# lujiarui/Str2Str

Hardware: AMD Instinct MI355X
Metric: sampled conformations/sec (whole node), 256-res chain, 100 denoise steps (higher is better)
Workload: dtype f32 (matrix products on 2-way f16 split MFMA 'f16x3': 3 products per block, fp32 accumulate, fp32-equivalent); 1 GPU; configs[1]: single 256-residue synthetic chain, 128 replicas per GPU x 100 denoise steps (+1 self-conditioning forward), probability-flow ODE, seeded synthetic weights; n_res=256, replicas_per_gpu=128, denoise_steps=100, parallelism=replica-shard x1, arith=f16x3, rng=device

## Files before the change

include/str2str_hip.h:

```cpp
#ifndef STR2STR_HIP_H
#define STR2STR_HIP_H

#ifdef __cplusplus
extern "C" {
#endif

int s2s_abi_version(void);



int s2s_edge_transition(const float* edge, const float* node_ab, const float* node_p, const float* w1_packed,
                        const float* w2_packed, const float* wf_packed, const float* b2, const float* bf,
                        const float* ln_gamma, const float* ln_beta, const float* mask, float* out, int n_samples,
                        int n_res, float ln_eps, const float* proj_w_packed, const float* proj_bias_cat64,
                        float* proj_attn_bias, float* proj_pair_z, void* stream);

int s2s_edge_transition_f16x3(const float* edge, const float* node_ab, const float* node_p, const void* weight_stream,
                              const float* b2, const float* ln_gamma, const float* ln_beta,
                              const float* mask, float* out, int n_samples, int n_res, float ln_eps, int io_layout,
                              const float* proj_bias_cat64, float* proj_attn_bias, float* proj_pair_z, int prescale_exp,
                              int* range_words, void* stream);

int s2s_edge_embed(const float* node_a, const float* node_b, const float* rel_table, const float* bin_table,
                   const float* bin_lower, const long long* residue_idx, const float* ca_xyz, const float* w2_packed,
                   const float* w3_packed, const float* b2, const float* b3, const float* ln_gamma, const float* ln_beta,
                   const float* mask, float* out, int n_samples, int n_res, int rel_offset, int n_rel, int n_bins,
                   float ln_eps, const float* proj_w_packed, const float* proj_bias_cat64, float* proj_attn_bias,
                   float* proj_pair_z, void* stream);

int s2s_edge_embed_f16x3(const float* node_a, const float* node_b, const float* rel_table, const float* bin_table,
                         const float* bin_lower, const long long* residue_idx, const float* ca_xyz,
                         const void* weight_stream, const float* b2, const float* b3, const float* ln_gamma,
                         const float* ln_beta, const float* mask, float* out, int n_samples, int n_res, int rel_offset,
                         int n_rel, int n_bins, float ln_eps, int out_tiled, const float* proj_bias_cat64,
                         float* proj_attn_bias, float* proj_pair_z, int* range_words, void* stream);

int s2s_pair_project(const float* edge, const float* w_packed, const float* bias_cat64, float* attn_bias, float* pair_z,
                     int n_samples, int n_res, void* stream);


int s2s_ipa_prep_points(const float* rigids7, const float* q_pts_lin, const float* kv_pts_lin, float* q_pts, float* k_pts,
                        float* v_pts, long long n_frames, int n_heads, int n_qk_points, int n_v_points, int v_pts_stride,
                        void* stream);

int s2s_ipa_attention(const float* q, const float* kv, const float* q_pts, const float* k_pts, const float* v_pts64,
                      const float* attn_bias, float* logits_out, float* stats_out, const float* mask, const float* rigids7,
                      const float* head_w_scaled, float* out, int n_samples, int n_res, int n_heads, int c_hidden,
                      int n_qk_points, int n_v_points, int c_pair_z, float inf, float eps, void* stream);

int s2s_ipa_prep_points_f16(const float* rigids7, const float* q_pts_lin, const float* kv_pts_lin, const float* head_w_scaled,
                            void* qp_xp, void* kp_xp, void* vp_vf, float* q2, float* k2, int n_samples, int n_res, int n_heads,
                            int n_qk_points, int n_v_points, int c_hidden, const void* s_xp, void* k_shared, void* v_shared,
                            int* range_words, void* stream);
int s2s_ipa_attention_f16w(const void* q_xp, const void* k_xp, const void* v_vf, const void* qp_xp, const void* kp_xp,
                             const void* vp_vf, const float* q2, const float* k2, const float* attn_bias, float* logits_out,
                             float* stats_out, const float* mask, const float* rigids7, float* out, void* out_xp,
                             int out_xp_ksteps, int n_samples, int n_res, int n_heads, int c_hidden, int n_qk_points,
                             int n_v_points, int c_pair_z, float inf, float eps, int n_kv_heads, void* stream);

int s2s_ipa_opair(const float* logits, const float* stats, const float* pair_z, float* out, int n_samples, int n_res,
                  int n_heads, int c_pair_z, int out_row_stride, int out_col_offset, int logits_ld, void* stream);


int s2s_rigid_compose_update(const float* rigids7, const float* update6, const float* mask, float* out7,
                             long long n_frames, int update_ld, void* stream);

int s2s_torsion_head(const float* u, int u_ld, int normalize, const float* gt_sin_cos, long long gt_row_stride, const float* fixed_mask,
                     float eps, float* out2, long long n_rows, void* stream);

int s2s_rigid_scale_trans(const float* rigids7, float* out7, long long n_frames, float scale, int divide, void* stream);

int s2s_set_backbone_tables(const float* pos_21x5x3, const float* mask_21x5, const int* is_psi_group_21x5,
                            const float* default_frames_21x2x4x4);

int s2s_frames_to_backbone(const float* rigids7, const float* psi_sincos, const long long* aatype, float* atom14_bb5,
                           float* atom37, long long n_frames, void* stream);


int s2s_se3_step(const float* x0_7, const float* xt_7, const float* mask, const float* diffuse_mask,
                 const float* params8, const double* z_rot, const double* z_trans,
                 const double* rot_score_in, const double* trans_score_in, float* next7,
                 double* rot_score_out, double* trans_score_out, int n_samples, int n_res, double dt,
                 const double* dt_per_sample, double coordinate_scaling, int probability_flow, int center_trans,
                 double noise_scale, void* stream);

int s2s_embed_assemble(const float* t_img, long long t_img_rows, const float* node_const, long long node_const_rows, const float* fa, const float* fb,
                       long long n_rows, int n_res, void* h_xp, float* h_f32, float* node_a, float* node_b, int b_col_blocked,
                       int* range_words, void* stream);


int s2s_pack_planes(const float* x, long long n_rows, int ld, int col0, int n_cols, void* xp, int xp_ksteps, int xp_kstep0,
                    const float* row_scale, int* range_words, void* stream);

int s2s_node_linear(const void* xp, const void* w_packed, const float* bias, long long n_rows, int k_in, int n_out,
                    int tiles_per_block, const float* pre_scale, int relu, const float* pre_mask, const float* residual,
                    int residual_ld, const float* ln_gamma, const float* ln_beta, float ln_eps, const float* post_mask,
                    float* out_f32, int out_ld, int out_col0, void* out_xp, int out_xp_ksteps, int out_xp_kstep0,
                    int map_pad, int map_src, int* range_words, void* stream);

int s2s_node_linear_f32(const float* x, int x_ld, const float* w_packed, const float* bias, long long n_rows, int k_in, int n_out,
                        int tiles_per_block, const float* pre_scale, int relu, const float* pre_mask, const float* residual,
                        int residual_ld, const float* ln_gamma, const float* ln_beta, float ln_eps, const float* post_mask,
                        float* out_f32, int out_ld, int out_col0, void* stream);

int s2s_node_linear_vfrag(const void* xp, const void* w_packed, const float* bias, long long n_rows, int k_in, int n_out,
                          int tiles_per_head, void* out_vf, int map_pad, int map_src, int* range_words, void* stream);

typedef struct s2s_node_problem {
    const void* xp; const void* w_packed; const float* bias;
    long long n_rows; int k_in, n_out, tiles_per_block;
    int vfrag_tiles_per_head;
    float* out_f32; int out_ld, out_col0;
    void* out_xp; int out_xp_ksteps, out_xp_kstep0;
    void* out_vf;
    int map_pad, map_src, relu;
    const float* pre_scale;
} s2s_node_problem;
int s2s_node_linear_multi(const s2s_node_problem* problems, int n_problems, int* range_words, void* stream);

typedef struct s2s_chain_layer { const void* w_packed; const float* bias; int relu; } s2s_chain_layer;
int s2s_node_chain(const void* xp, const s2s_chain_layer* layers, int n_layers, long long n_rows, int width, int k_in0,
                   const float* mid_residual, int mid_residual_ld, float* mid_out_f32, int mid_out_ld, const float* mid_ln_gamma,
                   const float* mid_ln_beta, float mid_ln_eps, const float* pre_mask, const float* residual, int residual_ld, const float* ln_gamma, const float* ln_beta, float ln_eps,
                   const float* post_mask, float* out_f32, int out_ld, int out_col0, void* out_xp, int out_xp_ksteps,
                   int out_xp_kstep0, int* range_words, void* stream);

int s2s_row_layernorm(const float* x, int x_ld, long long n_rows, int n_cols, const float* ln_gamma, const float* ln_beta, float ln_eps,
                      const float* post_mask, float* out_f32, int out_ld, int out_col0, void* out_xp, int out_xp_ksteps,
                      int out_xp_kstep0, int* range_words, void* stream);

int s2s_encoder_attention(const float* qkv, const float* key_bias, float* out_f32, void* out_xp, int n_samples, int n_res,
                          int n_heads, int head_dim, int* range_words, void* stream);

int s2s_encoder_attention_f16x3(const float* qkv, const float* key_bias, float* out_f32, void* out_xp, int n_samples, int n_res,
                          int n_heads, int head_dim, int* range_words, void* stream);


int s2s_forward_marginal(const float* rigids0_4x4, const float* z_axis, const float* u01, const float* z_trans,
                         const double* cdf_rows, const int* cdf_row_of_sample, const float* omega_grid, int n_omega,
                         const float* params2, const float* diffuse_mask, float coordinate_scaling, float* rigids_t7,
                         int n_samples, int n_res, void* stream);


int s2s_ca_sample_stats(const float* ca, int n_samples, int n_res, float clash_bar, int k_exclusion, int* n_clash,
                        float* adjacent_max, double* radius_of_gyration, void* stream);

int s2s_ca_pairwise_distances(const float* ca, int n_samples, int n_res, int offset, float* out, void* stream);

int s2s_ca_pwd_js(const float* ref_ca, int n_ref, const float* pred_ca, int n_pred, int n_res, int offset, int n_bins,
                  double pseudo_count, double* js_per_channel, const double* ref_weights, const double* pred_weights, void* stream);


int s2s_ca_rmsd_matrix(const float* a, int n_a, const float* b, int n_b, int n_res, const float* weights, double* rmsd,
                       double* workspace, long long workspace_doubles, void* stream);

int s2s_ca_superpose(const float* mobile, int n_mobile, const float* target, int n_res, const float* weights, double* rmsd,
                     double* xform, void* stream);

int s2s_apply_xform(const float* points, const double* xform, int n_samples, long long n_points, float* out, void* stream);

#define S2S_TM_MAX_RES 800

int s2s_ca_tm_matrix(const float* a, int n_a, const float* b, int n_b, int n_res, double d0, double* tm, void* stream);

int s2s_ca_tm_superpose(const float* mobile, int n_mobile, const float* target, int n_res, double d0, double* tm, double* xform12,
                        void* stream);

#define S2S_LDDT_MAX_RES 1024
#define S2S_LDDT_LIST_SLOTS(n_res) (((long long)(n_res) * ((long long)(n_res) - 1) / 2 + 1) / 2 * 2)
#define S2S_LDDT_WORKSPACE_BYTES(n_a, n_res) ((long long)(n_a) * (12 * S2S_LDDT_LIST_SLOTS(n_res) + 8 + 4 * (long long)(n_res)))

int s2s_ca_lddt_matrix(const float* a, int n_a, const float* b, int n_b, int n_res, double cutoff, int min_seq_sep, double* lddt,
                       void* workspace, long long workspace_bytes, void* stream);

int s2s_ca_lddt_per_residue(const float* model, int n_model, const float* target, int n_res, double cutoff, int min_seq_sep,
                            double* per_res, double* total, void* workspace, long long workspace_bytes, void* stream);

#define S2S_VIOL_MAX_RES 1024

int s2s_backbone_violations(const float* atoms, int n, int n_res, const unsigned char* atom_exists, const int* aatype,
                            const int* residue_index, double tolerance_factor, double clash_tolerance, double* losses, double* fractions,
                            double* per_residue_loss, unsigned char* bond_mask, unsigned char* clash_atom_mask, int* n_clash_pairs,
                            void* stream);

#define S2S_SS_MAX_RES 704

int s2s_secondary_structure(const float* atoms, int n, int n_res, const int* aatype, const int* residue_index, unsigned char* ss,
                            int* n_hbonds, double* hb_energy, int* hb_partner, double* torsions, void* stream);

#define S2S_CLUSTER_MAX_N 65536

int s2s_cluster_adjacency(const double* values, int n_rows, int row0, int n, double cutoff, int at_least, unsigned long long* adj,
                          int* deg, void* stream);

int s2s_cluster_gromos(const unsigned long long* adj, int* deg, int n, int init, int n_rounds, int* labels, int* centres, int* sizes,
                       int* state, unsigned long long* live_ws, unsigned long long* members_ws, void* stream);

#define S2S_CONTACT_MAX_RES 1024
#define S2S_CONTACT_MAX_STRUCTURES 65535
#define S2S_CONTACT_LIST_SLOTS(n_res) ((long long)(n_res) > 1 ? (long long)(n_res) * ((long long)(n_res) - 1) / 2 : 1)

int s2s_ca_contact_map(const float* ca, int n, int n_res, double cutoff, int min_seq_sep, const double* weights, int* counts,
                       double* weighted, void* stream);

int s2s_ca_contact_stats(const float* ca, int n, int n_res, double cutoff, int min_seq_sep, int* n_contacts, long long* sep_sum,
                         void* stream);

int s2s_ca_native_contacts(const float* native, int n_res, double cutoff, int min_seq_sep, int* pairs, double* d0, int* n_pairs,
                           void* stream);

int s2s_ca_native_q(const float* ca, int n, int n_res, const int* pairs, const double* d0, int n_pairs, double beta, double lam,
                    double* q_soft, double* q_hard, int* hits, void* stream);

#define S2S_SASA_MAX_RES 512
#define S2S_SASA_MAX_POINTS 1024

int s2s_backbone_sasa(const float* atoms, int n, int n_res, const unsigned char* atom_exists, const double* radii, double probe,
                      const double* sphere, int n_points, int* counts, double* per_residue, double* total, void* stream);

#define S2S_SAXS_MAX_RES 1024
#define S2S_SAXS_MAX_Q 1024
#define S2S_SAXS_MAX_TYPES 64

int s2s_ca_scattering(const float* ca, int n, int n_res, const double* q, int n_q, const int* types, const double* table, int n_types,
                      double* intensity, double* inv_r_mean, void* stream);


long long s2s_format_pdb_models(const float* atom37, int n_models, int n_res, const long long* aatype,
                                const long long* residue_index, const long long* chain_index, const double* b_factors,
                                int first_model_number, int add_end, char* out, long long out_capacity);

long long s2s_write_pdb_models(const char* path, int append, const float* atom37, int n_models, int n_res,
                               const long long* aatype, const long long* residue_index, const long long* chain_index,
                               const double* b_factors, int first_model_number, int add_end);

long long s2s_merge_pdb_files(const char* const* paths, int n_paths, const char* out_path);

int s2s_mt19937_discard(unsigned long long* state624, int* left, unsigned long long* next, unsigned long long n_outputs);

#ifdef __cplusplus
}
#endif
#endif
```

str2str_amd/csrc/enc_attention.hip:

```cpp
#include <hip/hip_runtime.h>
#include <math.h>

#include "f16x3.h"
#include "range_flag.h"
#include "str2str_hip.h"

namespace {

__device__ __forceinline__ f32x16 mfma32(float a, float b, f32x16 c) { return __builtin_amdgcn_mfma_f32_32x32x2f32(a, b, c, 0, 0, 0); }

template <int DH>
__global__ void __launch_bounds__(256) enc_attention_kernel(const float* __restrict__ qkv, const float* __restrict__ key_bias,
                                                            float* __restrict__ out_f32, bf16x8* __restrict__ out_xp, int* range_flag, int B, int N,
                                                            int heads, float scale) {
    static_assert(DH == 80, "built for the reference configuration (d_model 320, 4 heads)");
    constexpr int KSd = DH + 4;
    constexpr int CT = (DH + 31) / 32;
    constexpr int HALF = DH / 2;
    __shared__ __attribute__((aligned(16))) float s_k[2][32 * KSd];
    __shared__ __attribute__((aligned(16))) float s_v[2][32 * 96];
    __shared__ float s_b[2][32];
    const int lane = threadIdx.x & 63, h = lane >> 5, c = lane & 31, wave = threadIdx.x >> 6;
    const int n_qb = (N + 127) / 128;
    int bid = blockIdx.x;
    const int qb = bid % n_qb; bid /= n_qb;
    const int head = bid % heads;
    const int b = bid / heads;
    const int D = heads * DH;
    const int i = qb * 128 + wave * 32 + c;
    const bool ivalid = i < N;
    const long long row_i = (long long)b * N + (ivalid ? i : N - 1);
    const float* base = qkv + (long long)b * N * 3 * D + head * DH;

    float4 st[5];
    auto tile_load = [&](int j0) {
#pragma unroll
        for (int k = 0; k < 5; ++k) {
            const int idx = threadIdx.x + 256 * k;
            const int which = idx / 640, rem = idx % 640, r = rem / 20, c4 = rem % 20;
            const int j = min(j0 + r, N - 1);
            st[k] = *reinterpret_cast<const float4*>(base + (long long)j * 3 * D + D * (1 + which) + 4 * c4);
        }
    };
    auto tile_store = [&](int par, int j0) {
#pragma unroll
        for (int k = 0; k < 5; ++k) {
            const int idx = threadIdx.x + 256 * k;
            const int which = idx / 640, rem = idx % 640, r = rem / 20, c4 = rem % 20;
            float* dst = which ? &s_v[par][r * 96 + 4 * c4] : &s_k[par][r * KSd + 4 * c4];
            *reinterpret_cast<float4*>(dst) = st[k];
        }
        if (threadIdx.x < 32) {
            const int j = j0 + threadIdx.x;
            s_b[par][threadIdx.x] = j < N ? (key_bias ? key_bias[(long long)b * N + j] : 0.f) : -INFINITY;
        }
    };
    for (int idx = threadIdx.x; idx < 2 * 32 * 16; idx += 256) s_v[idx / 512][((idx % 512) / 16) * 96 + 80 + idx % 16] = 0.f;

    tile_load(0);
    float qreg[HALF];
    {
        const float* qrow = qkv + row_i * 3 * D + head * DH + HALF * h;
#pragma unroll
        for (int s4 = 0; s4 < HALF / 4; ++s4) {
            const float4 v = *reinterpret_cast<const float4*>(qrow + 4 * s4);
            qreg[4 * s4 + 0] = v.x * scale; qreg[4 * s4 + 1] = v.y * scale; qreg[4 * s4 + 2] = v.z * scale; qreg[4 * s4 + 3] = v.w * scale;
        }
    }
    f32x16 O[CT];
#pragma unroll
    for (int t = 0; t < CT; ++t)
#pragma unroll
        for (int r = 0; r < 16; ++r) O[t][r] = 0.f;
    float m_run = -INFINITY, l_run = 0.f;
    tile_store(0, 0);
    __syncthreads();

    int cur = 0;
    for (int j0 = 0; j0 < N; j0 += 32, cur ^= 1) {
        const bool more = j0 + 32 < N;
        if (more) tile_load(j0 + 32);
        f32x16 S, S1;
#pragma unroll
        for (int r = 0; r < 16; ++r) S[r] = 0.f, S1[r] = 0.f;
        const float* krow = &s_k[cur][c * KSd + HALF * h];
#pragma unroll
        for (int s4 = 0; s4 < HALF / 4; ++s4) {
            const float4 kf = *reinterpret_cast<const float4*>(krow + 4 * s4);
            S = mfma32(kf.x, qreg[4 * s4 + 0], S);
            S1 = mfma32(kf.y, qreg[4 * s4 + 1], S1);
            S = mfma32(kf.z, qreg[4 * s4 + 2], S);
            S1 = mfma32(kf.w, qreg[4 * s4 + 3], S1);
        }
        float tmax = -INFINITY;
#pragma unroll
        for (int r = 0; r < 16; ++r) {
            const float s = (S[r] + S1[r]) + s_b[cur][rowmap(r, h)];
            S[r] = s;
            tmax = fmaxf(tmax, s);
        }
        tmax = fmaxf(tmax, __shfl_xor(tmax, 32, 64));
        const float m_new = fmaxf(m_run, tmax);
        const float m_use = m_new == -INFINITY ? 0.f : m_new;
        const float alpha = expf(m_run - m_use);
        m_run = m_new;
        float psum = 0.f;
#pragma unroll
        for (int r = 0; r < 16; ++r) {
            const float p = expf(S[r] - m_use);
            S[r] = p;
            psum += p;
        }
        l_run = l_run * alpha + psum;
#pragma unroll
        for (int t = 0; t < CT; ++t) {
            f32x16 o = O[t];
#pragma unroll
            for (int r = 0; r < 16; ++r) o[r] *= alpha;
            const float* vcol = &s_v[cur][32 * t + c + 4 * h * 96];
#pragma unroll
            for (int s = 0; s < 16; ++s) o = mfma32(vcol[((s & 3) + 8 * (s >> 2)) * 96], S[s], o);
            O[t] = o;
        }
        if (more) tile_store(cur ^ 1, j0 + 32);
        __syncthreads();
    }

    const float l_tot = l_run + __shfl_xor(l_run, 32, 64);
    const float inv = 1.0f / l_tot;
    if (!ivalid) return;
    const long long row = (long long)b * N + i;
    if (out_f32) {
        float* o = out_f32 + row * D + head * DH;
#pragma unroll
        for (int t = 0; t < CT; ++t)
#pragma unroll
            for (int rq = 0; rq < 4; ++rq) {
                const int c0 = 32 * t + 8 * rq + 4 * h;
                if (c0 < DH)
                    *reinterpret_cast<float4*>(o + c0) = make_float4(O[t][4 * rq] * inv, O[t][4 * rq + 1] * inv, O[t][4 * rq + 2] * inv, O[t][4 * rq + 3] * inv);
            }
    }
    if (out_xp) {
        const int KS = D / 16;
        bf16x8* o = out_xp + (((row >> 5) * KS + (DH / 16) * head) * 2) * 64 + 32 * h + (int)(row & 31);
        float amax = 0.f;
#pragma unroll
        for (int t = 0; t < CT; ++t)
#pragma unroll
            for (int u = 0; u < 2; ++u) {
                if (2 * t + u >= DH / 16) continue;
                f16x8 ph, pl;
#pragma unroll
                for (int j = 0; j < 8; ++j) {
                    float v = O[t][8 * u + j] * inv;
                    amax = s2s::range_max(amax, v);
                    asm volatile("" : "+v"(v));
                    const _Float16 a_ = (_Float16)v;
                    ph[j] = a_; pl[j] = (_Float16)(v - (float)a_);
                }
                bf16x8* q = o + ((2 * t + u) * 2) * 64;
                q[0] = __builtin_bit_cast(bf16x8, ph); q[64] = __builtin_bit_cast(bf16x8, pl);
            }
        s2s::range_report(range_flag, amax, s2s::kRangeEncoderAttention);
    }
}


__device__ __forceinline__ void enc_split8(float x0, float x1, float x2, float x3, float x4, float x5, float x6, float x7, f16x8& ph, f16x8& pl,
                                           float& amax) {
    unsigned h0, h1, h2, h3, l0, l1, l2, l3;
    split4_f16(x0, x1, x2, x3, h0, h1, l0, l1, amax);
    split4_f16(x4, x5, x6, x7, h2, h3, l2, l3, amax);
    ph = __builtin_bit_cast(f16x8, u32x4{h0, h1, h2, h3});
    pl = __builtin_bit_cast(f16x8, u32x4{l0, l1, l2, l3});
}

template <int DH>
__global__ void __launch_bounds__(256, 2) enc_attention_f16_kernel(const float* __restrict__ qkv, const float* __restrict__ key_bias,
                                                                float* __restrict__ out_f32, bf16x8* __restrict__ out_xp, int* range_flag, int B,
                                                                int N, int heads, float scale) {
    static_assert(DH == 80, "built for the reference configuration (d_model 320, 4 heads)");
    constexpr int KSQ = DH / 16;
    constexpr int CT = (DH + 31) / 32;
    constexpr float kPS = 1024.0f;
    __shared__ __attribute__((aligned(16))) f16x8 s_kf[2][KSQ * 2 * 64];
    __shared__ __attribute__((aligned(16))) f16x8 s_vf[2][CT * 2 * 2 * 64];
    __shared__ float s_b[2][32];
    const int lane = threadIdx.x & 63, h = lane >> 5, c = lane & 31, wave = threadIdx.x >> 6;
    const int n_qb = (N + 127) / 128;
    int bid = blockIdx.x;
    const int qb = bid % n_qb; bid /= n_qb;
    const int head = bid % heads;
    const int b = bid / heads;
    const int D = heads * DH;
    const int i = qb * 128 + wave * 32 + c;
    const bool ivalid = i < N;
    const long long row_i = (long long)b * N + (ivalid ? i : N - 1);
    const float* base = qkv + (long long)b * N * 3 * D + head * DH;
    float amax = 0.f;

    float4 st[5];
    auto tile_load = [&](int j0) {
#pragma unroll
        for (int k = 0; k < 5; ++k) {
            const int idx = threadIdx.x + 256 * k;
            const int which = idx / 640, rem = idx % 640, r = rem / 20, c4 = rem % 20;
            const int j = min(j0 + r, N - 1);
            st[k] = *reinterpret_cast<const float4*>(base + (long long)j * 3 * D + D * (1 + which) + 4 * c4);
        }
    };
    auto tile_store = [&](int par, int j0) {
#pragma unroll
        for (int k = 0; k < 5; ++k) {
            const int idx = threadIdx.x + 256 * k;
            const int which = idx / 640, rem = idx % 640, r = rem / 20, c4 = rem % 20;
            unsigned h0, h1, l0, l1;
            split4_f16(st[k].x, st[k].y, st[k].z, st[k].w, h0, h1, l0, l1, amax);
            if (!which) {
                const int ch = 4 * c4, ks = ch >> 4, hh = (ch >> 3) & 1, e = ch & 7;
                _Float16* ph = reinterpret_cast<_Float16*>(&s_kf[par][(ks * 2 + 0) * 64 + 32 * hh + r]) + e;
                _Float16* pl = reinterpret_cast<_Float16*>(&s_kf[par][(ks * 2 + 1) * 64 + 32 * hh + r]) + e;
                *reinterpret_cast<uint2*>(ph) = make_uint2(h0, h1);
                *reinterpret_cast<uint2*>(pl) = make_uint2(l0, l1);
            } else {
                const int u = r >> 4, hh = (r >> 2) & 1, e = (r & 3) + 4 * ((r >> 3) & 1);
                const unsigned hv[2] = {h0, h1}, lv[2] = {l0, l1};
#pragma unroll
                for (int q = 0; q < 4; ++q) {
                    const int ch = 4 * c4 + q, t = ch >> 5, cc = ch & 31;
                    const unsigned short hb = (unsigned short)(hv[q >> 1] >> (16 * (q & 1))), lb = (unsigned short)(lv[q >> 1] >> (16 * (q & 1)));
                    reinterpret_cast<unsigned short*>(&s_vf[par][((t * 2 + u) * 2 + 0) * 64 + 32 * hh + cc])[e] = hb;
                    reinterpret_cast<unsigned short*>(&s_vf[par][((t * 2 + u) * 2 + 1) * 64 + 32 * hh + cc])[e] = lb;
                }
            }
        }
        if (threadIdx.x < 32) {
            const int j = j0 + threadIdx.x;
            s_b[par][threadIdx.x] = j < N ? (key_bias ? key_bias[(long long)b * N + j] : 0.f) : -INFINITY;
        }
    };
    for (int idx = threadIdx.x; idx < 2 * 2 * 2 * 64; idx += 256) {
        const int par = idx >> 8, rest = idx & 255, ln = rest & 63;
        if ((ln & 31) >= DH - 32 * (CT - 1)) s_vf[par][((CT - 1) * 2 * 2) * 64 + rest] = f16x8{0, 0, 0, 0, 0, 0, 0, 0};
    }

    tile_load(0);
    f16x8 qh[KSQ], ql[KSQ];
    {
        const float* qrow = qkv + row_i * 3 * D + head * DH + 8 * h;
#pragma unroll
        for (int ks = 0; ks < KSQ; ++ks) {
            const float4 v0 = *reinterpret_cast<const float4*>(qrow + 16 * ks), v1 = *reinterpret_cast<const float4*>(qrow + 16 * ks + 4);
            enc_split8(v0.x * scale, v0.y * scale, v0.z * scale, v0.w * scale, v1.x * scale, v1.y * scale, v1.z * scale, v1.w * scale, qh[ks], ql[ks],
                       amax);
        }
    }
    f32x16 O[CT];
#pragma unroll
    for (int t = 0; t < CT; ++t)
#pragma unroll
        for (int r = 0; r < 16; ++r) O[t][r] = 0.f;
    float m_run = -INFINITY, l_run = 0.f;
    tile_store(0, 0);
    __syncthreads();

    int cur = 0;
    for (int j0 = 0; j0 < N; j0 += 32, cur ^= 1) {
        const bool more = j0 + 32 < N;
        if (more) tile_load(j0 + 32);
        f32x16 S, S1;
#pragma unroll
        for (int r = 0; r < 16; ++r) S[r] = 0.f, S1[r] = 0.f;
#pragma unroll
        for (int ks = 0; ks < KSQ; ++ks) {
            const f16x8 kh = s_kf[cur][(ks * 2 + 0) * 64 + lane], kl = s_kf[cur][(ks * 2 + 1) * 64 + lane];
            f32x16& acc = (ks & 1) ? S1 : S;
            acc = mfma_f16(kl, qh[ks], acc);
            acc = mfma_f16(kh, ql[ks], acc);
            acc = mfma_f16(kh, qh[ks], acc);
        }
        float tmax = -INFINITY;
#pragma unroll
        for (int r = 0; r < 16; ++r) {
            const float sv = (S[r] + S1[r]) + s_b[cur][rowmap(r, h)];
            S[r] = sv;
            tmax = fmaxf(tmax, sv);
        }
        tmax = fmaxf(tmax, __shfl_xor(tmax, 32, 64));
        const float m_new = fmaxf(m_run, tmax);
        const float m_use = m_new == -INFINITY ? 0.f : m_new;
        const float alpha = expf(m_run - m_use);
        m_run = m_new;
        float psum = 0.f;
#pragma unroll
        for (int r = 0; r < 16; ++r) {
            const float pv = expf(S[r] - m_use);
            S[r] = pv * kPS;
            psum += pv;
        }
        l_run = l_run * alpha + psum;
        f16x8 ph[2], pl[2];
        float pmax = 0.f;
#pragma unroll
        for (int u = 0; u < 2; ++u) {
            enc_split8(S[8 * u + 0], S[8 * u + 1], S[8 * u + 2], S[8 * u + 3], S[8 * u + 4], S[8 * u + 5], S[8 * u + 6], S[8 * u + 7], ph[u], pl[u], pmax);
        }
#pragma unroll
        for (int t = 0; t < CT; ++t) {
            f32x16 o = O[t];
#pragma unroll
            for (int r = 0; r < 16; ++r) o[r] *= alpha;
#pragma unroll
            for (int u = 0; u < 2; ++u) {
                const f16x8 vh = s_vf[cur][((t * 2 + u) * 2 + 0) * 64 + lane], vl = s_vf[cur][((t * 2 + u) * 2 + 1) * 64 + lane];
                o = mfma_f16(vl, ph[u], o);
                o = mfma_f16(vh, pl[u], o);
                o = mfma_f16(vh, ph[u], o);
            }
            O[t] = o;
        }
        if (more) tile_store(cur ^ 1, j0 + 32);
        __syncthreads();
    }

    const float l_tot = l_run + __shfl_xor(l_run, 32, 64);
    const float inv = 1.0f / (l_tot * kPS);
    if (ivalid) {
        const long long row = (long long)b * N + i;
        if (out_f32) {
            float* o = out_f32 + row * D + head * DH;
#pragma unroll
            for (int t = 0; t < CT; ++t)
#pragma unroll
                for (int rq = 0; rq < 4; ++rq) {
                    const int c0 = 32 * t + 8 * rq + 4 * h;
                    if (c0 < DH)
                        *reinterpret_cast<float4*>(o + c0) = make_float4(O[t][4 * rq] * inv, O[t][4 * rq + 1] * inv, O[t][4 * rq + 2] * inv, O[t][4 * rq + 3] * inv);
                }
        }
        if (out_xp) {
            const int KS = D / 16;
            bf16x8* o = out_xp + (((row >> 5) * KS + (DH / 16) * head) * 2) * 64 + 32 * h + (int)(row & 31);
#pragma unroll
            for (int t = 0; t < CT; ++t)
#pragma unroll
                for (int u = 0; u < 2; ++u) {
                    if (2 * t + u >= DH / 16) continue;
                    f16x8 oh, ol;
                    enc_split8(O[t][8 * u + 0] * inv, O[t][8 * u + 1] * inv, O[t][8 * u + 2] * inv, O[t][8 * u + 3] * inv, O[t][8 * u + 4] * inv,
                               O[t][8 * u + 5] * inv, O[t][8 * u + 6] * inv, O[t][8 * u + 7] * inv, oh, ol, amax);
                    bf16x8* q = o + ((2 * t + u) * 2) * 64;
                    q[0] = __builtin_bit_cast(bf16x8, oh); q[64] = __builtin_bit_cast(bf16x8, ol);
                }
        }
    }
    s2s::range_report(range_flag, amax, s2s::kRangeEncoderAttention);
}

}

extern "C" int s2s_encoder_attention_f16x3(const float* qkv, const float* key_bias, float* out_f32, void* out_xp, int n_samples, int n_res,
                                           int n_heads, int head_dim, int* range_words, void* stream) {
    if (n_samples <= 0 || n_res <= 0) return 0;
    if (!qkv || (!out_f32 && !out_xp) || head_dim != 80 || n_heads < 1 || (n_heads * head_dim) % 32) return (int)hipErrorInvalidValue;
    const long long blocks = (long long)n_samples * n_heads * ((n_res + 127) / 128);
    hipLaunchKernelGGL((enc_attention_f16_kernel<80>), dim3((unsigned)blocks), dim3(256), 0, (hipStream_t)stream, qkv, key_bias, out_f32,
                       (bf16x8*)out_xp, range_words, n_samples, n_res, n_heads, 1.0f / sqrtf((float)head_dim));
    return (int)hipGetLastError();
}

extern "C" int s2s_encoder_attention(const float* qkv, const float* key_bias, float* out_f32, void* out_xp, int n_samples, int n_res,
                                     int n_heads, int head_dim, int* range_words, void* stream) {
    if (n_samples <= 0 || n_res <= 0) return 0;
    if (!qkv || (!out_f32 && !out_xp) || head_dim != 80 || n_heads < 1 || (n_heads * head_dim) % 32) return (int)hipErrorInvalidValue;
    const long long blocks = (long long)n_samples * n_heads * ((n_res + 127) / 128);
    hipLaunchKernelGGL((enc_attention_kernel<80>), dim3((unsigned)blocks), dim3(256), 0, (hipStream_t)stream, qkv, key_bias, out_f32,
                       (bf16x8*)out_xp, range_words, n_samples, n_res, n_heads, 1.0f / sqrtf((float)head_dim));
    return (int)hipGetLastError();
}
```

str2str_amd/csrc/node_gemm.hip:

```cpp
#include <hip/hip_runtime.h>

#include <cstdlib>

#include "f16x3.h"
#include "range_flag.h"
#include "str2str_hip.h"

namespace {

using s2s::range_max;

__device__ __forceinline__ void split8_f16(const float* v, f16x8& ph, f16x8& pl, float& amax) {
    unsigned h0, h1, h2, h3, l0, l1, l2, l3;
    split4_f16(v[0], v[1], v[2], v[3], h0, h1, l0, l1, amax);
    split4_f16(v[4], v[5], v[6], v[7], h2, h3, l2, l3, amax);
    ph = __builtin_bit_cast(f16x8, u32x4{h0, h1, h2, h3});
    pl = __builtin_bit_cast(f16x8, u32x4{l0, l1, l2, l3});
}
__device__ __forceinline__ void store_planes(f16x8* q, const float* v, float& amax) {
    f16x8 ph, pl;
    split8_f16(v, ph, pl, amax);
    q[0] = ph; q[64] = pl;
}

struct GemmArgs {
    const f16x8* xp;
    const char* wpk;
    const float* bias;
    const float* pre_scale;
    const float* pre_mask;
    const float* residual;
    const float* ln_gamma;
    const float* ln_beta;
    const float* post_mask;
    float* out_f32;
    f16x8* out_xp;
    f16x8* out_vf;
    int vf_tiles_per_head;
    long long M;
    int KS;
    int n_col_blocks;
    int res_ld, out_ld, out_col0, xp_KS, xp_ks0;
    int relu;
    float ln_eps;
    int x_ld;
    int* range_flag;
    int map_pad, map_src;
};

__device__ float s2s_zero[512];

template <int TG>
__device__ __forceinline__ void node_epilogue(f32x16 (&acc)[TG], const GemmArgs& a, long long rt, long long n_rt, int lane, int cb,
                                              float ps) {
    const int h = lane >> 5;
    const long long row = rt * 32 + (lane & 31);
    const bool valid = rt < n_rt && row < a.M;
    const long long rowc = valid ? row : a.M - 1;
    const float pm = a.pre_mask ? a.pre_mask[rowc] : 1.0f;
    const int col_base = cb * TG * 32;
    const float* bias_p = a.bias ? a.bias + col_base + 4 * h : s2s_zero + 4 * h;
    const float* res_p = a.residual ? a.residual + rowc * a.res_ld + col_base + 4 * h : s2s_zero + 4 * h;
    float4 qb[2][4], qr[2][4];
    auto fetch4 = [&](const float* p, int t, float4 (&q)[4]) {
#pragma unroll
        for (int rq = 0; rq < 4; ++rq) q[rq] = *reinterpret_cast<const float4*>(p + 32 * t + 8 * rq);
    };
    fetch4(bias_p, 0, qb[0]);
    fetch4(res_p, 0, qr[0]);
    const bool relu = a.relu != 0;
#pragma unroll
    for (int t = 0; t < TG; ++t) {
        if (t + 1 < TG) {
            fetch4(bias_p, t + 1, qb[(t + 1) & 1]);
            fetch4(res_p, t + 1, qr[(t + 1) & 1]);
        }
#pragma unroll
        for (int rq = 0; rq < 4; ++rq) {
            const float4 b = qb[t & 1][rq], rr = qr[t & 1][rq];
            float v[4] = {acc[t][4 * rq + 0] * ps + b.x, acc[t][4 * rq + 1] * ps + b.y, acc[t][4 * rq + 2] * ps + b.z,
                          acc[t][4 * rq + 3] * ps + b.w};
#pragma unroll
            for (int e = 0; e < 4; ++e) v[e] = relu ? fmaxf(v[e], 0.f) : v[e];
            acc[t][4 * rq + 0] = v[0] * pm + rr.x; acc[t][4 * rq + 1] = v[1] * pm + rr.y;
            acc[t][4 * rq + 2] = v[2] * pm + rr.z; acc[t][4 * rq + 3] = v[3] * pm + rr.w;
        }
    }
    if (a.ln_gamma) {
        float sum = 0.f;
#pragma unroll
        for (int t = 0; t < TG; ++t)
#pragma unroll
            for (int r = 0; r < 16; ++r) sum += acc[t][r];
        const float m0 = xhalf_sum(sum) * (1.0f / (TG * 32));
        float var = 0.f, dev = 0.f;
#pragma unroll
        for (int t = 0; t < TG; ++t)
#pragma unroll
            for (int r = 0; r < 16; ++r) {
                const float d = acc[t][r] - m0;
                dev += d;
                var += d * d;
            }
        const float dm = xhalf_sum(dev) * (1.0f / (TG * 32));
        const float mean = m0 + dm;
        const float rstd = 1.0f / sqrtf(xhalf_sum(var) * (1.0f / (TG * 32)) - dm * dm + a.ln_eps);
        fetch4(a.ln_gamma + col_base + 4 * h, 0, qb[0]);
        fetch4(a.ln_beta + col_base + 4 * h, 0, qr[0]);
#pragma unroll
        for (int t = 0; t < TG; ++t) {
            if (t + 1 < TG) {
                fetch4(a.ln_gamma + col_base + 4 * h, t + 1, qb[(t + 1) & 1]);
                fetch4(a.ln_beta + col_base + 4 * h, t + 1, qr[(t + 1) & 1]);
            }
#pragma unroll
            for (int rq = 0; rq < 4; ++rq) {
                const float4 g = qb[t & 1][rq], be = qr[t & 1][rq];
                acc[t][4 * rq + 0] = (acc[t][4 * rq + 0] - mean) * rstd * g.x + be.x;
                acc[t][4 * rq + 1] = (acc[t][4 * rq + 1] - mean) * rstd * g.y + be.y;
                acc[t][4 * rq + 2] = (acc[t][4 * rq + 2] - mean) * rstd * g.z + be.z;
                acc[t][4 * rq + 3] = (acc[t][4 * rq + 3] - mean) * rstd * g.w + be.w;
            }
        }
    }
    if (a.post_mask) {
        const float q = a.post_mask[rowc];
#pragma unroll
        for (int t = 0; t < TG; ++t)
#pragma unroll
            for (int r = 0; r < 16; ++r) acc[t][r] *= q;
    }
    if (a.out_f32 && valid) {
        float* o = a.out_f32 + row * a.out_ld + a.out_col0 + col_base;
#pragma unroll
        for (int t = 0; t < TG; ++t)
#pragma unroll
            for (int rq = 0; rq < 4; ++rq)
                *reinterpret_cast<float4*>(o + 32 * t + 8 * rq + 4 * h) =
                    make_float4(acc[t][4 * rq + 0], acc[t][4 * rq + 1], acc[t][4 * rq + 2], acc[t][4 * rq + 3]);
    }
    if (a.out_xp && rt < n_rt) {
        float amax = 0.f;
        f16x8* o = a.out_xp + ((rt * a.xp_KS + a.xp_ks0 + 2 * (cb * TG)) * 2) * 64 + lane;
#pragma unroll
        for (int t = 0; t < TG; ++t)
#pragma unroll
            for (int u = 0; u < 2; ++u) {
                float v[8];
#pragma unroll
                for (int j = 0; j < 8; ++j) v[j] = valid ? acc[t][8 * u + j] : 0.f;
                store_planes(o + ((2 * t + u) * 2) * 64, v, amax);
            }
        s2s::range_report(a.range_flag, amax, s2s::kRangeNodeGemm);
    }
}

template <int TG, int WAVES, bool VF>
__device__ __forceinline__ void node_gemm_body(const GemmArgs& a, const int bx, const int by) {
    constexpr int kStage = 2 * TG * 1024;
    constexpr int kFrags = 2 * TG;
    constexpr int kPieces = (kFrags + WAVES - 1) / WAVES;
    extern __shared__ __attribute__((aligned(16))) char s_w[];
    const int lane = threadIdx.x & 63, h = lane >> 5;
    const int wave = __builtin_amdgcn_readfirstlane(threadIdx.x >> 6);
    const long long rt = (long long)bx * WAVES + wave;
    const long long n_rt = (a.M + 31) / 32;
    const long long rtc = rt < n_rt ? rt : n_rt - 1;
    const int KS = a.KS;

    typedef __attribute__((address_space(3))) char lds_char;
    typedef __attribute__((address_space(3))) f32x4 lds_f4;
    typedef __attribute__((address_space(3))) f16x8 lds_frag;

    f32x4 wst[kPieces];
    const char* wsrc = a.wpk + (long long)by * KS * kStage + lane * 16;
    auto w_load = [&](int ks) {
        ks = ks < KS ? ks : KS - 1;
        const char* src = wsrc + (long long)ks * kStage;
#pragma unroll
        for (int k = 0; k < kPieces; ++k) {
            if (WAVES * k + WAVES - 1 < kFrags || WAVES * k + wave < kFrags)
                wst[k] = *reinterpret_cast<const f32x4*>(src + (WAVES * k + wave) * 1024);
        }
    };
    auto w_store = [&](int par) {
        lds_char* dst = (lds_char*)s_w + par * kStage + lane * 16;
#pragma unroll
        for (int k = 0; k < kPieces; ++k) {
            if (WAVES * k + WAVES - 1 < kFrags || WAVES * k + wave < kFrags) *(lds_f4*)(dst + (WAVES * k + wave) * 1024) = wst[k];
        }
    };
    const f16x8* xsrc = a.xp + (rtc * KS) * 2 * 64 + lane;
    if (a.map_pad > 0) {
        const long long orow = rtc * 32 + (lane & 31);
        const long long smp = orow / a.map_pad;
        const int n = (int)(orow - smp * a.map_pad);
        const long long srow = smp * a.map_src + (n < a.map_src ? n : a.map_src - 1);
        xsrc = a.xp + ((srow >> 5) * KS) * 2 * 64 + ((int)(srow & 31) + 32 * h);
    }
    f16x8 xa[2], xb[2];
    auto x_load = [&](int ks, f16x8 (&x)[2]) {
        ks = ks < KS ? ks : KS - 1;
        const f16x8* p = xsrc + (long long)ks * 2 * 64;
        x[0] = p[0]; x[1] = p[64];
    };

    f32x16 acc[TG];

    w_load(0);
    x_load(0, xa);
    w_store(0);
    w_load(1);
    __syncthreads();

    auto compute = [&](int par, const f16x8 (&x)[2]) {
        const lds_frag* wl = (const lds_frag*)((lds_char*)s_w + par * kStage) + lane;
        auto mm = [&](const f16x8& wf, const f16x8& xf, f32x16 c) { return VF ? mfma_f16(xf, wf, c) : mfma_f16(wf, xf, c); };
        f16x8 fl[TG], fh[TG];
        __builtin_amdgcn_sched_barrier(0);
#pragma unroll
        for (int t = 0; t < TG; ++t) fl[t] = wl[t * 128 + 64];
#pragma unroll
        for (int t = 0; t < TG; ++t) fh[t] = wl[t * 128];
#pragma unroll
        for (int t = 0; t < TG; ++t) acc[t] = mm(fl[t], x[0], acc[t]);
#pragma unroll
        for (int t = 0; t < TG; ++t) acc[t] = mm(fh[t], x[1], acc[t]);
#pragma unroll
        for (int t = 0; t < TG; ++t) acc[t] = mm(fh[t], x[0], acc[t]);
        __builtin_amdgcn_sched_group_barrier(0x100, TG, 0);
#pragma unroll
        for (int t = 0; t < TG; ++t) {
            __builtin_amdgcn_sched_group_barrier(0x008, 1, 0);
            __builtin_amdgcn_sched_group_barrier(0x100, 1, 0);
        }
        __builtin_amdgcn_sched_group_barrier(0x008, 2 * TG, 0);
        __builtin_amdgcn_sched_barrier(0);
    };

    const long long row = rt * 32 + (lane & 31);
    const long long rowc = (rt < n_rt && row < a.M) ? row : a.M - 1;
    const float ps = (a.pre_scale ? a.pre_scale[rowc] : 1.0f) * kInvWS;

    const int cb = by;
#pragma unroll
    for (int t = 0; t < TG; ++t)
#pragma unroll
        for (int r = 0; r < 16; ++r) acc[t][r] = 0.f;
    for (int ks = 0; ks < KS; ks += 2) {
        x_load(ks + 1, xb);
        compute(0, xa);
        w_store(1);
        w_load(ks + 2);
        __syncthreads();
        x_load(ks + 2, xa);
        compute(1, xb);
        w_store(0);
        w_load(ks + 3);
        __syncthreads();
    }

    float amax = 0.f;
    if constexpr (VF) {
        if (rt < n_rt) {
            const float* bias_col = a.bias ? a.bias + (lane & 31) : s2s_zero;
            const int bias_step = a.bias ? 32 : 0;
            float bvs[TG];
#pragma unroll
            for (int t = 0; t < TG; ++t) bvs[t] = bias_col[bias_step * (cb * TG + t)];
#pragma unroll
            for (int t = 0; t < TG; ++t) {
                const int T = cb * TG + t;
                const float bv = bvs[t];
                f16x8* o = a.out_vf + ((((rt * (a.n_col_blocks * TG / a.vf_tiles_per_head) + T / a.vf_tiles_per_head) * a.vf_tiles_per_head +
                                         T % a.vf_tiles_per_head) * 2) * 2) * 64 + lane;
#pragma unroll
                for (int u = 0; u < 2; ++u) {
                    float v[8];
#pragma unroll
                    for (int j = 0; j < 8; ++j) {
                        const int r = 8 * u + j;
                        v[j] = (rt * 32 + (r & 3) + 8 * (r >> 2) + 4 * h < a.M) ? __builtin_fmaf(acc[t][r], kInvWS, bv) : 0.f;
                    }
                    store_planes(o + (u * 2) * 64, v, amax);
                }
            }
        }
        s2s::range_report(a.range_flag, amax, s2s::kRangeNodeGemm);
        return;
    }
    node_epilogue<TG>(acc, a, rt, n_rt, lane, cb, ps);
}

template <int TG, int WAVES, bool VF>
__global__ void __launch_bounds__(64 * WAVES, 2) node_gemm_kernel(GemmArgs a) {
    node_gemm_body<TG, WAVES, VF>(a, blockIdx.x, blockIdx.y);
}

constexpr int kMultiMax = 6;
struct MultiArgs {
    GemmArgs a[kMultiMax];
    int kind[kMultiMax];
    int nx[kMultiMax];
    int cum[kMultiMax + 1];
    int n;
};
__global__ void __launch_bounds__(256, 2) node_gemm_multi_kernel(MultiArgs ma) {
    int p = 0;
#pragma unroll
    for (int q = 1; q < kMultiMax; ++q)
        if (q < ma.n && (int)blockIdx.x >= ma.cum[q]) p = q;
    p = __builtin_amdgcn_readfirstlane(p);
    const int local = (int)blockIdx.x - ma.cum[p];
    const int bx = local % ma.nx[p], by = local / ma.nx[p];
    const GemmArgs& a = ma.a[p];
    switch (ma.kind[p]) {
        case 0: node_gemm_body<8, 4, false>(a, bx, by); break;
        case 1: node_gemm_body<8, 4, true>(a, bx, by); break;
        case 2: node_gemm_body<6, 4, false>(a, bx, by); break;
        case 3: node_gemm_body<5, 4, false>(a, bx, by); break;
        case 4: node_gemm_body<10, 4, false>(a, bx, by); break;
        case 5: node_gemm_body<4, 4, false>(a, bx, by); break;
        case 6: node_gemm_body<2, 4, false>(a, bx, by); break;
        default: node_gemm_body<1, 4, false>(a, bx, by); break;
    }
}

constexpr int kChainMax = 4;
struct ChainArgs {
    GemmArgs a;
    const char* w[kChainMax];
    const float* bias[kChainMax];
    int relu[kChainMax];
    int n_layers;
    const float* mid_residual; int mid_res_ld;
    float* mid_out; int mid_out_ld;
    const float* mid_ln_gamma; const float* mid_ln_beta; float mid_ln_eps;
};

template <int TG, int KS0>
__global__ void __launch_bounds__(256, 1) node_chain_kernel(ChainArgs c) {
    constexpr int KS = 2 * TG;
    constexpr int KSX = KS0 > KS ? KS0 : KS;
    constexpr int kStage = 2 * TG * 1024;
    constexpr int kFrags = 2 * TG, kPieces = (kFrags + 3) / 4;
    extern __shared__ __attribute__((aligned(16))) char s_w[];
    const int lane = threadIdx.x & 63;
    const int wave = __builtin_amdgcn_readfirstlane(threadIdx.x >> 6);
    const GemmArgs& a = c.a;
    const long long rt = (long long)blockIdx.x * 4 + wave;
    const long long n_rt = (a.M + 31) / 32;
    const long long rtc = rt < n_rt ? rt : n_rt - 1;
    typedef __attribute__((address_space(3))) char lds_char;
    typedef __attribute__((address_space(3))) f32x4 lds_f4;
    typedef __attribute__((address_space(3))) f16x8 lds_frag;

    f32x4 wst[kPieces];
    const char* wsrc = c.w[0] + lane * 16;
    auto w_load = [&](int ks) {
        const char* src = wsrc + (long long)ks * kStage;
#pragma unroll
        for (int k = 0; k < kPieces; ++k)
            if (4 * k + 3 < kFrags || 4 * k + wave < kFrags) wst[k] = *reinterpret_cast<const f32x4*>(src + (4 * k + wave) * 1024);
    };
    auto w_store = [&](int par) {
        lds_char* dst = (lds_char*)s_w + par * kStage + lane * 16;
#pragma unroll
        for (int k = 0; k < kPieces; ++k)
            if (4 * k + 3 < kFrags || 4 * k + wave < kFrags) *(lds_f4*)(dst + (4 * k + wave) * 1024) = wst[k];
    };
    f16x8 xr[KSX][2];
    {
        const f16x8* xsrc = a.xp + (rtc * KS0) * 2 * 64 + lane;
#pragma unroll
        for (int ks = 0; ks < KS0; ++ks) { xr[ks][0] = xsrc[(ks * 2) * 64]; xr[ks][1] = xsrc[(ks * 2 + 1) * 64]; }
    }
    f32x16 acc[TG];
    const long long row = rt * 32 + (lane & 31);
    const bool valid = rt < n_rt && row < a.M;
    const long long rowc = valid ? row : a.M - 1;
    auto compute = [&](int par, const f16x8 (&x)[2]) {
        const lds_frag* wl = (const lds_frag*)((lds_char*)s_w + par * kStage) + lane;
        f16x8 fl[TG], fh[TG];
        __builtin_amdgcn_sched_barrier(0);
#pragma unroll
        for (int t = 0; t < TG; ++t) fl[t] = wl[t * 128 + 64];
#pragma unroll
        for (int t = 0; t < TG; ++t) fh[t] = wl[t * 128];
#pragma unroll
        for (int t = 0; t < TG; ++t) acc[t] = mfma_f16(fl[t], x[0], acc[t]);
#pragma unroll
        for (int t = 0; t < TG; ++t) acc[t] = mfma_f16(fh[t], x[1], acc[t]);
#pragma unroll
        for (int t = 0; t < TG; ++t) acc[t] = mfma_f16(fh[t], x[0], acc[t]);
        __builtin_amdgcn_sched_group_barrier(0x100, TG, 0);
#pragma unroll
        for (int t = 0; t < TG; ++t) {
            __builtin_amdgcn_sched_group_barrier(0x008, 1, 0);
            __builtin_amdgcn_sched_group_barrier(0x100, 1, 0);
        }
        __builtin_amdgcn_sched_group_barrier(0x008, 2 * TG, 0);
        __builtin_amdgcn_sched_barrier(0);
    };
    float amax = 0.f;
    w_load(0);
    w_store(0);
    w_load(1);
    __syncthreads();
    auto run_layer = [&](auto nkc, int l, bool last) {
        constexpr int NK = decltype(nkc)::value;
#pragma unroll
        for (int t = 0; t < TG; ++t)
#pragma unroll
            for (int r = 0; r < 16; ++r) acc[t][r] = 0.f;
        static_for<0, NK>([&](auto kc) {
            constexpr int ks = decltype(kc)::value, par = ks & 1;
            compute(par, xr[ks]);
            if constexpr (ks + 1 < NK) {
                w_store(par ^ 1);
                if constexpr (ks + 2 < NK) w_load(ks + 2);
                else if (!last) { wsrc = c.w[l + 1] + lane * 16; w_load(0); }
                __syncthreads();
            } else if (!last) {
                __syncthreads();
                w_store(0);
                w_load(1);
                __syncthreads();
            }
        });
    };
    auto inner_epilogue = [&](int l) {
        GemmArgs inner = a;
        inner.bias = c.bias[l]; inner.relu = c.relu[l];
        inner.pre_scale = nullptr; inner.pre_mask = nullptr; inner.residual = nullptr; inner.ln_gamma = nullptr; inner.ln_beta = nullptr;
        inner.post_mask = nullptr; inner.out_f32 = nullptr; inner.out_xp = nullptr;
        if (l == 0) {
            inner.residual = c.mid_residual; inner.res_ld = c.mid_res_ld;
            inner.out_f32 = c.mid_out; inner.out_ld = c.mid_out_ld; inner.out_col0 = 0;
            inner.ln_gamma = c.mid_ln_gamma; inner.ln_beta = c.mid_ln_beta; inner.ln_eps = c.mid_ln_eps;
        }
        node_epilogue<TG>(acc, inner, rt, n_rt, lane, 0, kInvWS);
        if (l == 0 && c.mid_out) asm volatile("s_waitcnt vmcnt(0)" ::: "memory");
#pragma unroll
        for (int t = 0; t < TG; ++t)
#pragma unroll
            for (int u = 0; u < 2; ++u) {
                float v[8];
#pragma unroll
                for (int j = 0; j < 8; ++j) v[j] = valid ? acc[t][8 * u + j] : 0.f;
                split8_f16(v, xr[2 * t + u][0], xr[2 * t + u][1], amax);
            }
    };
    run_layer(IC<KS0>{}, 0, c.n_layers == 1);
    for (int l = 1; l < c.n_layers; ++l) {
        inner_epilogue(l - 1);
        run_layer(IC<KS>{}, l, l == c.n_layers - 1);
    }
    s2s::range_report(a.range_flag, amax, s2s::kRangeNodeGemm);
    GemmArgs fin = a;
    fin.bias = c.bias[c.n_layers - 1]; fin.relu = c.relu[c.n_layers - 1];
    const float ps = (a.pre_scale ? a.pre_scale[rowc] : 1.0f) * kInvWS;
    node_epilogue<TG>(acc, fin, rt, n_rt, lane, 0, ps);
}

template <int TG>
__global__ void __launch_bounds__(256) node_ln_kernel(GemmArgs a, const float* __restrict__ x, int x_ld) {
    const int lane = threadIdx.x & 63, h = lane >> 5, wave = threadIdx.x >> 6;
    const long long rt = (long long)blockIdx.x * 4 + wave;
    const long long n_rt = (a.M + 31) / 32;
    const long long row = rt * 32 + (lane & 31);
    const long long rowc = (rt < n_rt && row < a.M) ? row : a.M - 1;
    f32x16 acc[TG];
    const float* p = x + rowc * x_ld + 4 * h;
#pragma unroll
    for (int t = 0; t < TG; ++t)
#pragma unroll
        for (int rq = 0; rq < 4; ++rq) {
            const float4 v = *reinterpret_cast<const float4*>(p + 32 * t + 8 * rq);
            acc[t][4 * rq + 0] = v.x; acc[t][4 * rq + 1] = v.y; acc[t][4 * rq + 2] = v.z; acc[t][4 * rq + 3] = v.w;
        }
    node_epilogue<TG>(acc, a, rt, n_rt, lane, 0, 1.0f);
}

__global__ void __launch_bounds__(256) pack_planes_kernel(const float* __restrict__ x, long long M, int ld, int col0, int KS,
                                                          f16x8* __restrict__ xp, int xp_KS, int ks0, const float* __restrict__ row_scale,
                                                          int* range_flag) {
    const int lane = threadIdx.x & 63, g = lane >> 5;
    const long long unit = (long long)blockIdx.x * 4 + (threadIdx.x >> 6);
    const long long n_rt = (M + 31) / 32;
    if (unit >= n_rt * KS) return;
    const long long rt = unit / KS;
    const int ks = (int)(unit - rt * KS);
    const long long row = rt * 32 + (lane & 31);
    float v[8] = {0.f, 0.f, 0.f, 0.f, 0.f, 0.f, 0.f, 0.f};
    if (row < M) {
        const float* p = x + row * ld + col0 + 32 * (ks >> 1) + 16 * (ks & 1) + 4 * g;
        const float4 lo = *reinterpret_cast<const float4*>(p), hi = *reinterpret_cast<const float4*>(p + 8);
        const float sc = row_scale ? row_scale[row] : 1.0f;
        v[0] = lo.x * sc; v[1] = lo.y * sc; v[2] = lo.z * sc; v[3] = lo.w * sc;
        v[4] = hi.x * sc; v[5] = hi.y * sc; v[6] = hi.z * sc; v[7] = hi.w * sc;
    }
    float amax = 0.f;
    store_planes(xp + ((rt * xp_KS + ks0 + ks) * 2) * 64 + lane, v, amax);
    s2s::range_report(range_flag, amax, s2s::kRangePackPlanes);
}

template <int TG>
__global__ void __launch_bounds__(256) node_gemm_f32_kernel(GemmArgs a) {
    const int lane = threadIdx.x & 63, h = lane >> 5;
    const int wave = __builtin_amdgcn_readfirstlane(threadIdx.x >> 6);
    const long long rt = (long long)blockIdx.x * 4 + wave;
    const long long n_rt = (a.M + 31) / 32;
    const int cb = blockIdx.y;
    const long long row = rt * 32 + (lane & 31);
    const long long rowc = (rt < n_rt && row < a.M) ? row : a.M - 1;
    const int S4 = a.KS;
    const float* xr = reinterpret_cast<const float*>(a.xp) + rowc * a.x_ld + 4 * h;
    const float4* w = reinterpret_cast<const float4*>(a.wpk) + ((long long)cb * S4 * TG) * 64 + lane;
    f32x16 acc[TG];
#pragma unroll
    for (int t = 0; t < TG; ++t)
#pragma unroll
        for (int r = 0; r < 16; ++r) acc[t][r] = 0.f;
    float4 xv = *reinterpret_cast<const float4*>(xr);
    for (int j = 0; j < S4; ++j) {
        const float4 xn = *reinterpret_cast<const float4*>(xr + 8 * (j + 1 < S4 ? j + 1 : j));
        const float4* wj = w + (long long)j * TG * 64;
#pragma unroll
        for (int t = 0; t < TG; ++t) {
            const float4 wv = wj[t * 64];
            acc[t] = __builtin_amdgcn_mfma_f32_32x32x2f32(wv.x, xv.x, acc[t], 0, 0, 0);
            acc[t] = __builtin_amdgcn_mfma_f32_32x32x2f32(wv.y, xv.y, acc[t], 0, 0, 0);
            acc[t] = __builtin_amdgcn_mfma_f32_32x32x2f32(wv.z, xv.z, acc[t], 0, 0, 0);
            acc[t] = __builtin_amdgcn_mfma_f32_32x32x2f32(wv.w, xv.w, acc[t], 0, 0, 0);
        }
        xv = xn;
    }
    const float ps = a.pre_scale ? a.pre_scale[rowc] : 1.0f;
    node_epilogue<TG>(acc, a, rt, n_rt, lane, cb, ps);
}

template <int TG>
int launch_gemm_f32(const GemmArgs& a, hipStream_t stream) {
    const long long n_rt = (a.M + 31) / 32;
    hipLaunchKernelGGL((node_gemm_f32_kernel<TG>), dim3((unsigned)((n_rt + 3) / 4), (unsigned)a.n_col_blocks), dim3(256), 0, stream, a);
    return (int)hipGetLastError();
}

template <int TG, int WAVES, bool VF = false>
int launch_gemm_w(const GemmArgs& a, hipStream_t stream) {
    constexpr int lds = 2 * 2 * TG * 1024;
    const long long n_rt = (a.M + 31) / 32;
    const long long row_blocks = (n_rt + WAVES - 1) / WAVES;
    hipLaunchKernelGGL((node_gemm_kernel<TG, WAVES, VF>), dim3((unsigned)row_blocks, (unsigned)a.n_col_blocks), dim3(64 * WAVES), lds, stream, a);
    return (int)hipGetLastError();
}

template <int TG>
int launch_gemm(const GemmArgs& a, hipStream_t stream) {
    return launch_gemm_w<TG, 4>(a, stream);
}

}

__global__ void __launch_bounds__(256) embed_assemble_kernel(const float* __restrict__ t_img_all, int t_img_stride, const float* __restrict__ node_const,
                                                             long long nc_rows, const float* __restrict__ fa, const float* __restrict__ fb,
                                                             long long M, int L, f16x8* __restrict__ h_xp, float* __restrict__ h_f32,
                                                             float* __restrict__ node_a, float* __restrict__ node_b, int b_col_blocked,
                                                             unsigned nh, unsigned na, int* range_flag) {
    const unsigned bid = blockIdx.x;
    if (bid < nh) {
        const int lane = threadIdx.x & 63, g = lane >> 5;
        const long long n_rt = (M + 31) / 32;
        if (h_xp) {
            const long long unit = (long long)bid * 4 + (threadIdx.x >> 6);
            if (unit >= n_rt * 16) return;
            const long long rt = unit / 16;
            const int ks = (int)(unit - rt * 16);
            const long long row = rt * 32 + (lane & 31);
            float v[8] = {0.f, 0.f, 0.f, 0.f, 0.f, 0.f, 0.f, 0.f};
            if (row < M) {
                const int c0 = 32 * (ks >> 1) + 16 * (ks & 1) + 4 * g;
                const float* p = node_const + (row % nc_rows) * 256 + c0;
                const float* t_img = t_img_all + (row / L) * t_img_stride;
                const float4 lo = *reinterpret_cast<const float4*>(p), hi = *reinterpret_cast<const float4*>(p + 8);
                const float4 tl = *reinterpret_cast<const float4*>(t_img + c0), th = *reinterpret_cast<const float4*>(t_img + c0 + 8);
                v[0] = fmaxf(tl.x + lo.x, 0.f); v[1] = fmaxf(tl.y + lo.y, 0.f); v[2] = fmaxf(tl.z + lo.z, 0.f); v[3] = fmaxf(tl.w + lo.w, 0.f);
                v[4] = fmaxf(th.x + hi.x, 0.f); v[5] = fmaxf(th.y + hi.y, 0.f); v[6] = fmaxf(th.z + hi.z, 0.f); v[7] = fmaxf(th.w + hi.w, 0.f);
            }
            float amax = 0.f;
            store_planes(h_xp + ((rt * 16 + ks) * 2) * 64 + lane, v, amax);
            s2s::range_report(range_flag, amax, s2s::kRangePackPlanes);
        } else {
            const long long i = (long long)bid * 256 + threadIdx.x;
            if (i < M * 64) {
                const long long row = i >> 6;
                const int c = (int)(i & 63) * 4;
                const float4 x = *reinterpret_cast<const float4*>(node_const + (row % nc_rows) * 256 + c);
                const float4 t = *reinterpret_cast<const float4*>(t_img_all + (row / L) * t_img_stride + c);
                *reinterpret_cast<float4*>(h_f32 + i * 4) = make_float4(fmaxf(t.x + x.x, 0.f), fmaxf(t.y + x.y, 0.f), fmaxf(t.z + x.z, 0.f), fmaxf(t.w + x.w, 0.f));
            }
        }
        return;
    }
    const bool is_a = bid < nh + na;
    const long long i = (long long)(bid - nh - (is_a ? 0u : na)) * 256 + threadIdx.x;
    if (i >= M * 32) return;
    int c;
    if (is_a || !b_col_blocked) c = (int)(i & 31) * 4;
    else c = (int)((i / L) & 31) * 4;
    const float* src = is_a ? fa : fb;
    const float4 x = *reinterpret_cast<const float4*>(src + i * 4);
    const float* t_img = t_img_all + (i / (32ll * L)) * t_img_stride;
    const float4 t = *reinterpret_cast<const float4*>(t_img + (is_a ? 256 : 384) + c);
    *reinterpret_cast<float4*>((is_a ? node_a : node_b) + i * 4) = make_float4(t.x + x.x, t.y + x.y, t.z + x.z, t.w + x.w);
}

extern "C" int s2s_embed_assemble(const float* t_img, long long t_img_rows, const float* node_const, long long node_const_rows, const float* fa, const float* fb,
                                  long long n_rows, int n_res, void* h_xp, float* h_f32, float* node_a, float* node_b, int b_col_blocked,
                                  int* range_words, void* stream) {
    if (n_rows <= 0) return 0;
    if (!t_img || !node_const || !fa || !fb || !node_a || !node_b || (!h_xp == !h_f32) || n_res <= 0 || node_const_rows <= 0 ||
        n_rows % n_res || (node_const_rows != n_rows && node_const_rows != n_res) || (t_img_rows != 1 && t_img_rows != n_rows / n_res))
        return (int)hipErrorInvalidValue;
    const long long nh = h_xp ? (((n_rows + 31) / 32) * 16 + 3) / 4 : (n_rows * 64 + 255) / 256;
    const long long na = (n_rows * 32 + 255) / 256;
    if (nh + 2 * na >= (1ll << 31)) return (int)hipErrorInvalidValue;
    hipLaunchKernelGGL(embed_assemble_kernel, dim3((unsigned)(nh + 2 * na)), dim3(256), 0, (hipStream_t)stream, t_img, t_img_rows == 1 ? 0 : 512, node_const,
                       node_const_rows, fa, fb, n_rows, n_res, (f16x8*)h_xp, h_f32, node_a, node_b, b_col_blocked, (unsigned)nh, (unsigned)na,
                       range_words);
    return (int)hipGetLastError();
}

extern "C" int s2s_pack_planes(const float* x, long long n_rows, int ld, int col0, int n_cols, void* xp, int xp_ksteps,
                               int xp_kstep0, const float* row_scale, int* range_words, void* stream) {
    if (n_rows <= 0) return 0;
    if (!x || !xp || n_cols <= 0 || n_cols % 32 || ld % 4 || col0 % 4 || xp_kstep0 < 0 || xp_kstep0 + n_cols / 16 > xp_ksteps)
        return (int)hipErrorInvalidValue;
    const int KS = n_cols / 16;
    const long long units = ((n_rows + 31) / 32) * KS;
    hipLaunchKernelGGL(pack_planes_kernel, dim3((unsigned)((units + 3) / 4)), dim3(256), 0, (hipStream_t)stream, x, n_rows, ld, col0, KS,
                       (f16x8*)xp, xp_ksteps, xp_kstep0, row_scale, range_words);
    return (int)hipGetLastError();
}

static int check_epilogue(int n_out, int TG, const float* ln_gamma, const float* ln_beta, const float* out_f32, int out_ld, int out_col0,
                          const float* residual, int residual_ld) {
    if (n_out <= 0 || TG <= 0 || n_out % (32 * TG)) return 1;
    if ((ln_gamma != nullptr) != (ln_beta != nullptr) || (ln_gamma && n_out != 32 * TG)) return 1;
    if (out_f32 && (out_ld % 4 || out_col0 % 4)) return 1;
    if (residual && residual_ld % 4) return 1;
    return 0;
}

extern "C" int s2s_node_linear(const void* xp, const void* w_packed, const float* bias, long long n_rows, int k_in, int n_out,
                               int tiles_per_block, const float* pre_scale, int relu, const float* pre_mask, const float* residual,
                               int residual_ld, const float* ln_gamma, const float* ln_beta, float ln_eps, const float* post_mask,
                               float* out_f32, int out_ld, int out_col0, void* out_xp, int out_xp_ksteps, int out_xp_kstep0,
                               int map_pad, int map_src, int* range_words, void* stream) {
    if (n_rows <= 0) return 0;
    if (map_pad < 0 || (map_pad > 0 && (map_src <= 0 || map_src > map_pad || map_pad % 32 || n_rows % map_pad || pre_scale || pre_mask ||
                                        residual || post_mask)))
        return (int)hipErrorInvalidValue;
    const int TG = tiles_per_block;
    if (!xp || !w_packed || k_in <= 0 || k_in % 32 || (!out_f32 && !out_xp) ||
        check_epilogue(n_out, TG, ln_gamma, ln_beta, out_f32, out_ld, out_col0, residual, residual_ld))
        return (int)hipErrorInvalidValue;
    const int ncb = n_out / (32 * TG);
    if (out_xp && (out_xp_kstep0 < 0 || out_xp_kstep0 % 2 || out_xp_kstep0 + n_out / 16 > out_xp_ksteps)) return (int)hipErrorInvalidValue;
    GemmArgs a{(const f16x8*)xp, (const char*)w_packed, bias, pre_scale, pre_mask, residual, ln_gamma, ln_beta, post_mask, out_f32,
               (f16x8*)out_xp, nullptr, 0, n_rows, k_in / 16, ncb, residual_ld, out_ld, out_col0, out_xp_ksteps, out_xp_kstep0, relu, ln_eps,
               0, range_words, map_pad, map_src};
    hipStream_t st = (hipStream_t)stream;
    switch (TG) {
        case 1: return launch_gemm<1>(a, st);
        case 2: return launch_gemm<2>(a, st);
        case 4: return launch_gemm<4>(a, st);
        case 5: return launch_gemm<5>(a, st);
        case 6: return launch_gemm<6>(a, st);
        case 8: return launch_gemm<8>(a, st);
        case 10: return launch_gemm<10>(a, st);
        default: return (int)hipErrorInvalidValue;
    }
}

extern "C" int s2s_node_linear_f32(const float* x, int x_ld, const float* w_packed, const float* bias, long long n_rows, int k_in, int n_out,
                                   int tiles_per_block, const float* pre_scale, int relu, const float* pre_mask, const float* residual,
                                   int residual_ld, const float* ln_gamma, const float* ln_beta, float ln_eps, const float* post_mask,
                                   float* out_f32, int out_ld, int out_col0, void* stream) {
    if (n_rows <= 0) return 0;
    const int TG = tiles_per_block;
    if (!x || !w_packed || !out_f32 || k_in <= 0 || k_in % 8 || x_ld % 4 || x_ld < k_in ||
        check_epilogue(n_out, TG, ln_gamma, ln_beta, out_f32, out_ld, out_col0, residual, residual_ld))
        return (int)hipErrorInvalidValue;
    GemmArgs a{(const f16x8*)x, (const char*)w_packed, bias, pre_scale, pre_mask, residual, ln_gamma, ln_beta, post_mask, out_f32,
               nullptr, nullptr, 0, n_rows, k_in / 8, n_out / (32 * TG), residual_ld, out_ld, out_col0, 0, 0, relu, ln_eps, x_ld, nullptr, 0, 0};
    hipStream_t st = (hipStream_t)stream;
    switch (TG) {
        case 1: return launch_gemm_f32<1>(a, st);
        case 2: return launch_gemm_f32<2>(a, st);
        case 4: return launch_gemm_f32<4>(a, st);
        case 5: return launch_gemm_f32<5>(a, st);
        case 6: return launch_gemm_f32<6>(a, st);
        case 8: return launch_gemm_f32<8>(a, st);
        case 10: return launch_gemm_f32<10>(a, st);
        default: return (int)hipErrorInvalidValue;
    }
}

extern "C" int s2s_node_linear_vfrag(const void* xp, const void* w_packed, const float* bias, long long n_rows, int k_in, int n_out,
                                     int tiles_per_head, void* out_vf, int map_pad, int map_src, int* range_words, void* stream) {
    if (n_rows <= 0) return 0;
    constexpr int TG = 8;
    if (map_pad < 0 || (map_pad > 0 && (map_src <= 0 || map_src > map_pad || map_pad % 32 || n_rows % map_pad))) return (int)hipErrorInvalidValue;
    if (!xp || !w_packed || !out_vf || k_in <= 0 || k_in % 32 || n_out <= 0 || n_out % (32 * TG) || tiles_per_head <= 0 ||
        (n_out / 32) % tiles_per_head)
        return (int)hipErrorInvalidValue;
    GemmArgs a{(const f16x8*)xp, (const char*)w_packed, bias, nullptr, nullptr, nullptr, nullptr, nullptr, nullptr, nullptr, nullptr,
               (f16x8*)out_vf, tiles_per_head, n_rows, k_in / 16, n_out / (32 * TG), 0, 0, 0, 0, 0, 0, 0.f, 0, range_words, map_pad,
               map_src};
    return launch_gemm_w<TG, 4, true>(a, (hipStream_t)stream);
}


extern "C" int s2s_node_chain(const void* xp, const s2s_chain_layer* layers, int n_layers, long long n_rows, int width, int k_in0,
                              const float* mid_residual, int mid_residual_ld, float* mid_out_f32, int mid_out_ld,
                              const float* mid_ln_gamma, const float* mid_ln_beta, float mid_ln_eps,
                              const float* pre_mask, const float* residual, int residual_ld, const float* ln_gamma, const float* ln_beta,
                              float ln_eps, const float* post_mask, float* out_f32, int out_ld, int out_col0, void* out_xp,
                              int out_xp_ksteps, int out_xp_kstep0, int* range_words, void* stream) {
    if (n_rows <= 0) return 0;
    const int TG = width / 32;
    if (!xp || !layers || n_layers < 2 || n_layers > kChainMax || width % 32 || (TG != 8 && TG != 10) || (!out_f32 && !out_xp) ||
        check_epilogue(width, TG, ln_gamma, ln_beta, out_f32, out_ld, out_col0, residual, residual_ld) ||
        (out_xp && (out_xp_kstep0 < 0 || out_xp_kstep0 % 2 || out_xp_kstep0 + width / 16 > out_xp_ksteps)) ||
        (k_in0 != width && !(TG == 8 && k_in0 == 320)) || (mid_residual && mid_residual_ld % 4) || (mid_out_f32 && (mid_out_ld % 4 || mid_out_ld < width)) ||
        ((mid_ln_gamma != nullptr) != (mid_ln_beta != nullptr)))
        return (int)hipErrorInvalidValue;
    ChainArgs c{};
    c.a = GemmArgs{(const f16x8*)xp, nullptr, nullptr, nullptr, pre_mask, residual, ln_gamma, ln_beta, post_mask, out_f32, (f16x8*)out_xp,
                   nullptr, 0, n_rows, width / 16, 1, residual_ld, out_ld, out_col0, out_xp_ksteps, out_xp_kstep0, 0, ln_eps, 0,
                   range_words, 0, 0};
    c.n_layers = n_layers;
    c.mid_residual = mid_residual; c.mid_res_ld = mid_residual_ld; c.mid_out = mid_out_f32; c.mid_out_ld = mid_out_ld;
    c.mid_ln_gamma = mid_ln_gamma; c.mid_ln_beta = mid_ln_beta; c.mid_ln_eps = mid_ln_eps;
    for (int l = 0; l < n_layers; ++l) {
        if (!layers[l].w_packed) return (int)hipErrorInvalidValue;
        c.w[l] = (const char*)layers[l].w_packed; c.bias[l] = layers[l].bias; c.relu[l] = layers[l].relu;
    }
    const long long n_rt = (n_rows + 31) / 32;
    const unsigned grid = (unsigned)((n_rt + 3) / 4);
    hipStream_t st = (hipStream_t)stream;
    if (TG == 8 && k_in0 == 320) {
        constexpr int lds = 2 * 2 * 8 * 1024;
        hipLaunchKernelGGL((node_chain_kernel<8, 20>), dim3(grid), dim3(256), lds, st, c);
    } else if (TG == 8) {
        constexpr int lds = 2 * 2 * 8 * 1024;
        hipLaunchKernelGGL((node_chain_kernel<8, 16>), dim3(grid), dim3(256), lds, st, c);
    } else {
        constexpr int lds = 2 * 2 * 10 * 1024;
        hipLaunchKernelGGL((node_chain_kernel<10, 20>), dim3(grid), dim3(256), lds, st, c);
    }
    return (int)hipGetLastError();
}

extern "C" int s2s_node_linear_multi(const s2s_node_problem* pr, int n, int* range_words, void* stream) {
    if (n <= 0) return 0;
    if (!pr || n > kMultiMax) return (int)hipErrorInvalidValue;
    MultiArgs ma{};
    ma.n = n;
    long long total = 0;
    for (int i = 0; i < n; ++i) {
        const s2s_node_problem& q = pr[i];
        const bool vf = q.vfrag_tiles_per_head > 0;
        const int TG = vf ? 8 : q.tiles_per_block;
        if (q.n_rows <= 0 || !q.xp || !q.w_packed || q.k_in <= 0 || q.k_in % 32 || q.n_out <= 0 || TG <= 0 || q.n_out % (32 * TG) ||
            q.map_pad < 0 || (q.map_pad > 0 && (q.map_src <= 0 || q.map_src > q.map_pad || q.map_pad % 32 || q.n_rows % q.map_pad)))
            return (int)hipErrorInvalidValue;
        int kind;
        if (vf) {
            if (!q.out_vf || (q.n_out / 32) % q.vfrag_tiles_per_head) return (int)hipErrorInvalidValue;
            kind = 1;
        } else {
            if ((!q.out_f32 && !q.out_xp) || check_epilogue(q.n_out, TG, nullptr, nullptr, q.out_f32, q.out_ld, q.out_col0, nullptr, 0) ||
                (q.out_xp && (q.out_xp_kstep0 < 0 || q.out_xp_kstep0 % 2 || q.out_xp_kstep0 + q.n_out / 16 > q.out_xp_ksteps)))
                return (int)hipErrorInvalidValue;
            kind = TG == 8 ? 0 : (TG == 6 ? 2 : (TG == 5 ? 3 : (TG == 10 ? 4 : (TG == 4 ? 5 : (TG == 2 ? 6 : (TG == 1 ? 7 : -1))))));
            if (kind < 0) return (int)hipErrorInvalidValue;
        }
        const int ncb = q.n_out / (32 * TG);
        ma.a[i] = GemmArgs{(const f16x8*)q.xp, (const char*)q.w_packed, q.bias, q.pre_scale, nullptr, nullptr, nullptr, nullptr, nullptr,
                           vf ? nullptr : q.out_f32, vf ? nullptr : (f16x8*)q.out_xp, vf ? (f16x8*)q.out_vf : nullptr,
                           vf ? q.vfrag_tiles_per_head : 0, q.n_rows, q.k_in / 16, ncb, 0, q.out_ld, q.out_col0, q.out_xp_ksteps,
                           q.out_xp_kstep0, q.relu, 0.f, 0, range_words, q.map_pad, q.map_src};
        ma.kind[i] = kind;
        const long long n_rt = (q.n_rows + 31) / 32;
        ma.nx[i] = (int)((n_rt + 3) / 4);
        ma.cum[i] = (int)total;
        total += (long long)ma.nx[i] * ncb;
        if (total > (1ll << 30)) return (int)hipErrorInvalidValue;
    }
    for (int i = n; i <= kMultiMax; ++i) ma.cum[i] = (int)total;
    constexpr int lds = 2 * 2 * 10 * 1024;
    hipLaunchKernelGGL(node_gemm_multi_kernel, dim3((unsigned)total), dim3(256), lds, (hipStream_t)stream, ma);
    return (int)hipGetLastError();
}

extern "C" int s2s_row_layernorm(const float* x, int x_ld, long long n_rows, int n_cols, const float* ln_gamma, const float* ln_beta,
                                 float ln_eps, const float* post_mask, float* out_f32, int out_ld, int out_col0, void* out_xp,
                                 int out_xp_ksteps, int out_xp_kstep0, int* range_words, void* stream) {
    if (n_rows <= 0) return 0;
    const int TG = n_cols / 32;
    if (!x || x_ld % 4 || !ln_gamma || !ln_beta || (n_cols != 256 && n_cols != 320) || (!out_f32 && !out_xp) ||
        check_epilogue(n_cols, TG, ln_gamma, ln_beta, out_f32, out_ld, out_col0, nullptr, 0) ||
        (out_xp && (out_xp_kstep0 < 0 || out_xp_kstep0 % 2 || out_xp_kstep0 + n_cols / 16 > out_xp_ksteps)))
        return (int)hipErrorInvalidValue;
    GemmArgs a{nullptr, nullptr, nullptr, nullptr, nullptr, nullptr, ln_gamma, ln_beta, post_mask, out_f32, (f16x8*)out_xp, nullptr, 0, n_rows,
               0, 1, 0, out_ld, out_col0, out_xp_ksteps, out_xp_kstep0, 0, ln_eps, 0, range_words, 0, 0};
    const long long n_rt = (n_rows + 31) / 32;
    const dim3 grid((unsigned)((n_rt + 3) / 4));
    if (TG == 8) hipLaunchKernelGGL(node_ln_kernel<8>, grid, dim3(256), 0, (hipStream_t)stream, a, x, x_ld);
    else hipLaunchKernelGGL(node_ln_kernel<10>, grid, dim3(256), 0, (hipStream_t)stream, a, x, x_ld);
    return (int)hipGetLastError();
}
```

str2str_amd/models/net/ipa.py:

```python
from __future__ import annotations

import math
import os
from typing import Optional

import torch
import torch.nn as nn
import torch.nn.functional as F

from ... import ops
from ...arith import default_arith
from ...common.rigid_utils import Rigid, Rotation
from .layers import BackboneUpdate, DerivedCache, EdgeTransition, Linear, NodeTransition, TorsionAngleHead


class InvariantPointAttention(nn.Module):
    launch_switches = ("arith", "fold")

    def __init__(self, c_s: int, c_z: int, c_hidden: int, no_heads: int, no_qk_points: int, no_v_points: int,
                 inf: float = 1e5, eps: float = 1e-8):
        super().__init__()
        self.c_s, self.c_z, self.c_hidden = c_s, c_z, c_hidden
        self.no_heads, self.no_qk_points, self.no_v_points = no_heads, no_qk_points, no_v_points
        self.inf, self.eps = inf, eps
        hc = c_hidden * no_heads
        self.linear_q = Linear(c_s, hc)
        self.linear_kv = Linear(c_s, 2 * hc)
        self.linear_q_points = Linear(c_s, no_heads * no_qk_points * 3)
        self.linear_kv_points = Linear(c_s, no_heads * (no_qk_points + no_v_points) * 3)
        self.linear_b = Linear(c_z, no_heads)
        self.down_z = Linear(c_z, c_z // 4)
        self.head_weights = nn.Parameter(torch.full((no_heads,), 0.541324854612918))
        self.linear_out = Linear(no_heads * (c_z // 4 + c_hidden + no_v_points * 4), c_s, init="final")
        self.softmax = nn.Softmax(dim=-1)
        self.softplus = nn.Softplus()
        self.arith = default_arith()
        self.fold = os.environ.get("S2S_IPA_FOLD", "1") != "0"
        self._last_folded = False
        self._cache, self._packs = DerivedCache(), DerivedCache()

    def _derived(self):
        def build():
            wcat = torch.cat([self.linear_b.weight, self.down_z.weight], dim=0).float()
            bcat = torch.cat([self.linear_b.bias, self.down_z.bias]).float()
            b64 = bcat.new_zeros(64)
            b64[: bcat.numel()] = bcat
            hw = F.softplus(self.head_weights.float()) * math.sqrt(1.0 / (3 * (self.no_qk_points * 9.0 / 2)))
            wcat64 = wcat.new_zeros(64, wcat.shape[1])
            wcat64[: wcat.shape[0]] = wcat
            return ops.LazyDict({"wp": ops.pack_weight(wcat), "b64": b64.contiguous(), "hw": hw.contiguous()},
                                wp_f16x2=lambda d: ops.pack_f16x2_layer(wcat64, "chain").reshape(-1).view(torch.int16).contiguous())

        return self._cache.get([self.linear_b.weight, self.linear_b.bias, self.down_z.weight, self.down_z.bias,
                                self.head_weights], build)

    def node_packs(self):
        def build():
            H, C = self.no_heads, self.c_hidden
            pk = ops.pack_node_layer
            wkv = self.linear_kv.weight.view(H, 2, C, -1)
            bkv = self.linear_kv.bias.view(H, 2, C)
            d = {"q": pk(self.linear_q.weight, self.linear_q.bias), "kv": pk(self.linear_kv.weight, self.linear_kv.bias),
                 "k": pk(wkv[:, 0].reshape(H * C, -1), bkv[:, 0].reshape(-1)),
                 "v": pk(wkv[:, 1].reshape(H * C, -1), bkv[:, 1].reshape(-1)),
                 "qp": pk(self.linear_q_points.weight, self.linear_q_points.bias),
                 "kvp": pk(self.linear_kv_points.weight, self.linear_kv_points.bias),
                 "out": pk(self.linear_out.weight, self.linear_out.bias, True)}
            if self.c_s == C:
                d.update(self._folded_packs(wkv, bkv))
            return d

        return self._packs.get([p for lin in (self.linear_q, self.linear_kv, self.linear_q_points, self.linear_kv_points,
                                              self.linear_out) for p in (lin.weight, lin.bias)], build)

    def _folded_packs(self, wkv, bkv):
        H, C, cs = self.no_heads, self.c_hidden, self.c_s
        dev = self.linear_q.weight.device
        c64 = lambda t: t.detach().double().cpu()
        wq, bq = c64(self.linear_q.weight).view(H, C, cs), c64(self.linear_q.bias).view(H, C)
        wk, wv, bv = c64(wkv[:, 0]), c64(wkv[:, 1]), c64(bkv[:, 1])
        w_qf = torch.einsum("hca,hcb->hab", wk, wq).reshape(H * cs, cs).float().to(dev)
        b_qf = torch.einsum("hca,hc->ha", wk, bq).reshape(-1).float().to(dev)
        wo = c64(self.linear_out.weight)
        wo_o = wo[:, : H * C].view(-1, H, C)
        w_of = torch.cat([torch.einsum("ohc,hca->oha", wo_o, wv).reshape(-1, H * cs), wo[:, H * C:]], dim=1).float().to(dev)
        b_of = (c64(self.linear_out.bias) + torch.einsum("ohc,hc->o", wo_o, bv)).float().to(dev)
        return {"qf": ops.pack_node_layer(w_qf, b_qf), "outf": ops.pack_node_layer(w_of, b_of, True)}

    def use_f16(self, n_res: int, n_rows: int = 0) -> bool:
        if self.arith != "f16x3":
            return False
        shape_ok = (self.c_hidden == 256 and self.no_qk_points == 8 and self.no_v_points == 12 and self.c_z // 4 == 32
                    and self.no_heads == 8)
        rows_pad = (n_rows // max(n_res, 1)) * ops.padded_len(n_res)
        return shape_ok and rows_pad * 12288 < (1 << 32) and (n_res % 32 == 0 or n_rows * n_res * 32 < (1 << 31))

    def attention_f16(self, s_xp, B: int, N: int, r7, mask, pair_proj):
        w, d, M, H = self.node_packs(), self._derived(), B * N, self.no_heads
        if self.folded:
            return self._attention_f16_folded(s_xp, B, N, r7, mask, pair_proj, w, d)
        if w["v"]["tg"] != 8:
            raise ops.HipLibraryError("s2s_node_linear_vfrag is instantiated for 8 tiles per column block")
        NP = ops.padded_len(N)
        rmap, Mo = ((NP, N), B * NP) if NP != N else (None, M)
        K = torch.ops.str2str_amd
        names = ("q", "k", "v", "qp", "kvp")
        var = {n: (("w", w[n]["tg"]) if n == "v" else ops.small_rows_variant(w[n], M)) for n in names}
        dims = [x for n in names for x in (w[n]["k"], w[n]["n"], var[n][1])]
        q_xp, k_xp, v_vf, qp, kvp = K.ipa_projections(s_xp, *[[w[n][var[n][0]], w[n]["b"]] for n in names], dims, M, Mo, *(rmap or (0, 0)))
        pts = K.ipa_prep_points_f16(r7.view(B, N, 7), qp, kvp, d["hw"], H, self.no_qk_points, self.no_v_points, self.c_hidden)
        attn_bias, pair_z = pair_proj
        feats, feats_xp = K.ipa_attention_f16w(q_xp, k_xp, v_vf, *pts, attn_bias, pair_z, mask, r7, H, self.c_hidden,
                                               self.no_qk_points, self.no_v_points, self.c_z // 4, self.inf, self.eps, True)
        c0 = H * self.c_hidden
        f2 = feats.view(M, -1)
        K.pack_planes(f2, c0, f2.shape[1] - c0, feats_xp, f2.shape[1], c0)
        return feats_xp

    def _attention_f16_folded(self, s_xp, B, N, r7, mask, pair_proj, w, d):
        M, H = B * N, self.no_heads
        NP = ops.padded_len(N)
        rmap, Mo = ((NP, N), B * NP) if NP != N else (None, M)
        K = torch.ops.str2str_amd
        names = ("qf", "qp", "kvp")
        var = {n: ops.small_rows_variant(w[n], M) for n in names}
        dims = [x for n in ("qf", None, None, "qp", "kvp") for x in ((w[n]["k"], w[n]["n"], var[n][1]) if n else (0, 0, 0))]
        q_xp, _, _, qp, kvp = K.ipa_projections(s_xp, [w["qf"][var["qf"][0]], w["qf"]["b"]], [], [], [w["qp"][var["qp"][0]], w["qp"]["b"]],
                                                [w["kvp"][var["kvp"][0]], w["kvp"]["b"]], dims, M, Mo, *(rmap or (0, 0)))
        *pts, k_sh, v_sh = K.ipa_prep_points_shared_kv(r7.view(B, N, 7), qp, kvp, d["hw"], s_xp, H, self.no_qk_points, self.no_v_points,
                                                       self.c_hidden)
        attn_bias, pair_z = pair_proj
        feats, feats_xp = K.ipa_attention_f16w(q_xp, s_xp if k_sh is None else k_sh, v_sh, *pts, attn_bias, pair_z, mask, r7, H,
                                               self.c_hidden, self.no_qk_points, self.no_v_points, self.c_z // 4, self.inf, self.eps, True)
        c0 = H * self.c_hidden
        f2 = feats.view(M, -1)
        K.pack_planes(f2, c0, f2.shape[1] - c0, feats_xp, f2.shape[1], c0)
        return feats_xp

    @property
    def folded(self) -> bool:
        return self.fold and self.c_s == self.c_hidden and self.no_heads == 8

    def out_pack(self, feats_a) -> dict:
        w = self.node_packs()
        return w["outf"] if (self.folded and self._last_folded) else w["out"]

    def attention_f32(self, s_act, B: int, N: int, r7, mask, pair_proj):
        w, d, M, H = self.node_packs(), self._derived(), B * N, self.no_heads
        lin = lambda x: ops.node_apply(s_act, x, M)[0]
        q, kv, qp, kvp = lin(w["q"]), lin(w["kv"]), lin(w["qp"]), lin(w["kvp"])
        q_pts, k_pts, v_pts = torch.ops.str2str_amd.ipa_prep_points(r7.view(B, N, 7), qp.view(B, N, -1), kvp.view(B, N, -1), H,
                                                                    self.no_qk_points, self.no_v_points)
        attn_bias, pair_z = pair_proj
        feats = ops.ipa_attention(q.view(B, N, H, -1), kv.view(B, N, H, -1), q_pts, k_pts, v_pts, attn_bias, pair_z, mask, r7,
                                  d["hw"], H, self.c_hidden, self.no_qk_points, self.no_v_points, self.c_z // 4, self.inf,
                                  self.eps, logits_inplace=True)
        return ops.pack_planes(feats.view(M, -1)) if s_act.dtype == torch.int16 else feats.view(M, -1)

    def attention(self, s_act, B: int, N: int, r7, mask, pair_proj):
        self._last_folded = False
        if s_act.dtype == torch.int16 and self.use_f16(N, B * N):
            self._last_folded = self.folded
            return self.attention_f16(s_act, B, N, r7, mask, pair_proj)
        return self.attention_f32(s_act, B, N, r7, mask, pair_proj)

    def pair_proj_weights(self):
        return self._derived()

    def forward(self, s: torch.Tensor, z: torch.Tensor, r, mask: torch.Tensor, _rigids7: Optional[torch.Tensor] = None,
                _pair_proj=None):
        if not s.is_cuda:
            raise ops.HipLibraryError("InvariantPointAttention runs on the HIP device only (no CPU fallback)")
        if self.no_heads != 8 or self.c_z != 128:
            raise ops.HipLibraryError("IPA kernels are built for the reference configuration (H=8, c_z=128)")
        d = self._derived()
        r7 = (_rigids7 if _rigids7 is not None else r.to_tensor_7()).type(torch.float32).contiguous()
        mask = mask.type(torch.float32).contiguous()
        B, N = s.shape[:2]
        pp = _pair_proj if _pair_proj is not None else ops.pair_project(z.contiguous(), d["wp"], d["b64"])
        feats_a = self.attention(ops.to_act(s.reshape(B * N, -1).float().contiguous(), self.arith), B, N, r7, mask, pp)
        out, _ = ops.node_apply(feats_a, self.out_pack(feats_a), B * N)
        return out.view(B, N, -1)


class TranslationIPA(nn.Module):
    launch_switches = ("exact_padding", "fuse_pair_projection", "arith")

    def __init__(self, c_s: int, c_z: int, coordinate_scaling: float, no_ipa_blocks: int, skip_embed_size: int,
                 transformer_num_heads: int = 4, transformer_num_layers: int = 2, c_hidden: int = 256, no_heads: int = 8,
                 no_qk_points: int = 8, no_v_points: int = 12, dropout: float = 0.0):
        super().__init__()
        self.coordinate_scaling = coordinate_scaling
        self.scale_pos = lambda x: x * coordinate_scaling
        self.scale_rigids = lambda x: x.apply_trans_fn(self.scale_pos)
        self.unscale_pos = lambda x: x / coordinate_scaling
        self.unscale_rigids = lambda x: x.apply_trans_fn(self.unscale_pos)
        self.trunk = nn.ModuleDict()
        self.num_blocks = no_ipa_blocks
        for b in range(no_ipa_blocks):
            self.trunk[f"ipa_{b}"] = InvariantPointAttention(c_s=c_s, c_z=c_z, c_hidden=c_hidden, no_heads=no_heads,
                                                            no_qk_points=no_qk_points, no_v_points=no_v_points)
            self.trunk[f"ipa_ln_{b}"] = nn.LayerNorm(c_s)
            self.trunk[f"skip_embed_{b}"] = Linear(c_s, skip_embed_size, init="final")
            d = c_s + skip_embed_size
            layer = nn.TransformerEncoderLayer(d_model=d, nhead=transformer_num_heads, dim_feedforward=d)
            self.trunk[f"transformer_{b}"] = nn.TransformerEncoder(layer, transformer_num_layers, enable_nested_tensor=False)
            self.trunk[f"linear_{b}"] = Linear(d, c_s, init="final")
            self.trunk[f"node_transition_{b}"] = NodeTransition(c_s)
            self.trunk[f"bb_update_{b}"] = BackboneUpdate(c_s)
            if b < no_ipa_blocks - 1:
                self.trunk[f"edge_transition_{b}"] = EdgeTransition(node_embed_size=c_s, edge_embed_in=c_z,
                                                                    edge_embed_out=c_z)
        self.torsion_pred = TorsionAngleHead(c_s, 1)
        self._wcache, self._mask_cache = DerivedCache(), DerivedCache()
        self.exact_padding = False
        self.fuse_pair_projection = True
        self.arith = default_arith()

    def _node_weights(self):
        def build():
            T = self.trunk
            pk = lambda lin, whole=False: ops.pack_node_layer(lin.weight, lin.bias, whole)
            out = {}
            for b in range(self.num_blocks):
                d = {"skip": pk(T[f"skip_embed_{b}"]), "lin": pk(T[f"linear_{b}"]), "bb": pk(T[f"bb_update_{b}"].linear)}
                nt = T[f"node_transition_{b}"]
                d["nt1"], d["nt2"], d["nt3"] = pk(nt.linear_1), pk(nt.linear_2), pk(nt.linear_3, True)
                d["layers"] = []
                for layer in T[f"transformer_{b}"].layers:
                    att = layer.self_attn
                    d["layers"].append({"in": ops.pack_node_layer(att.in_proj_weight, att.in_proj_bias), "o": pk(att.out_proj, True),
                                        "l1": pk(layer.linear1), "l2": pk(layer.linear2, True)})
                out[b] = d
            tp = self.torsion_pred
            out["tor"] = {"l1": pk(tp.linear_1), "l2": pk(tp.linear_2), "fin": pk(tp.linear_final)}
            return out

        return self._wcache.get(list(self.parameters()), build)

    def _mask_terms(self, residue_mask: torch.Tensor, fixed_mask: torch.Tensor):
        def build():
            node_mask = residue_mask.type(torch.float).contiguous()
            fixed = fixed_mask.type(torch.float).contiguous()
            diffuse_mask = ((1 - fixed) * node_mask).contiguous()
            pad = 1.0 - node_mask
            key_bias = (torch.where(pad > 0, float("-inf"), 0.0) if self.exact_padding else pad).float().contiguous()
            return node_mask, diffuse_mask, key_bias, fixed.reshape(-1)

        return self._mask_cache.get([residue_mask, fixed_mask], build, bool(self.exact_padding))

    def forward(self, node_embed: torch.Tensor, edge_embed: torch.Tensor, batch: dict, _first_proj=None) -> dict:
        if not node_embed.is_cuda:
            raise ops.HipLibraryError("TranslationIPA runs on the HIP device only (no CPU fallback)")
        T, W = self.trunk, self._node_weights()
        f16 = self.arith == "f16x3"
        B, N, C = node_embed.shape
        M = B * N
        dev = node_embed.device
        node_mask, diffuse_mask, key_bias, fixed_flat = self._mask_terms(batch["residue_mask"], batch["fixed_mask"])
        nm, dm = node_mask.reshape(M), diffuse_mask.reshape(M)
        init7 = batch["rigids_t"].type(torch.float).contiguous()
        curr7 = torch.ops.str2str_amd.rigid_scale_trans(init7, self.coordinate_scaling, False)
        proj = _first_proj

        def lin(x, w, **kw):
            return ops.node_apply(x, w, M, **kw)

        s_f32 = node_embed.reshape(M, C).float().contiguous()
        init_a = batch.get("_node_embed_act")
        if init_a is None or (init_a.dtype == torch.int16) != f16:
            init_a = ops.to_act(s_f32, self.arith)
        s_a = init_a
        D = C + T["skip_embed_0"].out_features
        xbuf = []
        for b in range(self.num_blocks):
            xf = torch.empty(M, D, device=dev, dtype=torch.float32)
            xbuf.append((xf, ops.xp_alloc(M, D, dev) if f16 else xf))
        skip_done = None
        if f16 and 2 <= self.num_blocks <= 6:
            skip_done = ops.node_apply_multi(init_a, [(W[b]["skip"], dict(out_f32=xbuf[b][0], out_col0=C, out_xp=xbuf[b][1], out_xp_k=D, out_xp_k0=C))
                                                      for b in range(self.num_blocks)], M)
        for b in range(self.num_blocks):
            w, ipa = W[b], T[f"ipa_{b}"]
            if proj is None:
                d = ipa._derived()
                if isinstance(edge_embed, ops.PairTiled):
                    edge_embed = ops.pair_untiled(edge_embed)
                proj = torch.ops.str2str_amd.pair_project(edge_embed.contiguous(), d["wp"], d["b64"])
            feats_a = ipa.attention(s_a, B, N, curr7, node_mask, tuple(proj))
            proj = None
            ln = T[f"ipa_ln_{b}"]
            x_f32, x_a = xbuf[b]
            lin(feats_a, ipa.out_pack(feats_a), pre_mask=nm, residual=s_f32, ln=(ln.weight, ln.bias, ln.eps), out_f32=x_f32,
                out_xp=x_a, out_xp_k=D)
            if skip_done is None:
                lin(init_a, w["skip"], out_f32=x_f32, out_col0=C, out_xp=x_a, out_xp_k=D, out_xp_k0=C)
            xf, xx = x_f32, x_a
            for layer, lw in zip(T[f"transformer_{b}"].layers, w["layers"]):
                qkv, _ = lin(xx, lw["in"])
                sa_f32, sa_xp = torch.ops.str2str_amd.encoder_attention(qkv, key_bias, B, N, layer.self_attn.num_heads, not f16, f16, self.arith)
                x1 = torch.empty(M, D, device=dev, dtype=torch.float32)
                xf, xx = ops.node_apply_chain(sa_xp if f16 else sa_f32, [lw["o"], lw["l1"], lw["l2"]], M, (False, True, False),
                                              first_residual=xf, first_out_f32=x1, first_ln=(layer.norm1.weight, layer.norm1.bias, layer.norm1.eps),
                                              residual=x1, ln=(layer.norm2.weight, layer.norm2.bias, layer.norm2.eps), want_xp=True)
            nt = T[f"node_transition_{b}"]
            n_f32 = torch.empty(M, C, device=dev, dtype=torch.float32)
            s_f32, s_a = ops.node_apply_chain(xx, [w["lin"], w["nt1"], w["nt2"], w["nt3"]], M, (False, True, True, False),
                                              first_residual=x_f32, first_out_f32=n_f32, residual=n_f32,
                                              ln=(nt.ln.weight, nt.ln.bias, nt.ln.eps), post_mask=nm, want_xp=True)
            has_et = b < self.num_blocks - 1
            et = T[f"edge_transition_{b}"] if has_et else None
            specs = [(w["bb"], dict(pre_scale=dm))]
            if has_et:
                nl = et.node_layers()
                if et.arith == "f16x3":
                    node_ab16, ab_specs = et.ab16_specs(nl, True, M, s_a.device)
                    specs += [(nl["init"], {})] + ab_specs
                else:
                    specs += [(nl["init"], {}), (nl["ab_s"], {})]
            else:
                specs += [(W["tor"]["l1"], dict(relu=True, want_f32=False, want_xp=True))]
            outs = ops.node_apply_multi(s_a, specs, M)
            upd = outs[0][0]
            curr7 = torch.ops.str2str_amd.rigid_compose_update(curr7, upd, diffuse_mask)
            if has_et:
                n_p, node_ab = outs[1][0], (node_ab16 if et.arith == "f16x3" else outs[2][0])
                nxt = T[f"ipa_{b + 1}"].pair_proj_weights() if self.fuse_pair_projection else None
                et16 = et.arith == "f16x3"
                last = b == self.num_blocks - 2
                nxt16 = (not last) and T[f"edge_transition_{b + 1}"].arith == "f16x3"
                lay = "rowmajor" if not (et16 and nxt is not None) else ("none" if last else ("tiled" if nxt16 else "rowmajor"))
                if not et16 and isinstance(edge_embed, ops.PairTiled):
                    edge_embed = ops.pair_untiled(edge_embed)
                res = et.pair_mlp(edge_embed, node_ab.view(B, N, -1), n_p.view(B, N, -1), node_mask, nxt,
                                  **({"out_layout": lay} if lay != "rowmajor" else {}), **({"ab_kernel_form": True} if et16 else {}))
                if nxt is not None:
                    edge_embed, *proj = res
                else:
                    edge_embed = res
        wt = W["tor"]
        t1 = outs[1][1]
        _, t2 = lin(t1, wt["l2"], residual=s_f32, want_f32=False, want_xp=True)
        gt = batch.get("torsion_angles_sin_cos")
        blend = gt is not None and gt.is_cuda and gt.dtype == torch.float32 and gt.ndim == 4
        psi = torch.ops.str2str_amd.torsion_head(lin(t2, wt["fin"])[0], M, True, self.torsion_pred.eps,
                                                 gt[..., 2, :] if blend else None, fixed_flat if blend else None).view(B, N, 2)
        out7 = torch.ops.str2str_amd.rigid_scale_trans(curr7, self.coordinate_scaling, True)
        return {
            "psi_blended": blend,
            "in_rigids": Rigid.from_tensor_7(init7),
            "out_rigids": Rigid(Rotation(quats=out7[..., :4], normalize_quats=False), out7[..., 4:]),
            "out_rigids7": out7,
            "psi": psi,
        }
```

str2str_amd/ops/__init__.py:

```python
from .attention import encoder_attention, ipa_attention, ipa_attention_f16, ipa_prep_points, ipa_prep_points_f16
from .binding import ABI_VERSION, EXPORTS, LIB_PATH, HipLibraryError, KernelTimer, WeightRangeError, load_library
from .ensemble import (CLUSTER_MAX_N, CONTACT_MAX_RES, LDDT_MAX_RES, RMSD_LAUNCH_PAIRS, SASA_MAX_POINTS, SASA_MAX_RES, SAXS_MAX_Q, SAXS_MAX_RES,
                       SAXS_MAX_TYPES, SS_MAX_RES, TM_MAX_RES, VIOL_MAX_RES, apply_xform, backbone_sasa, backbone_violations, ca_contact_map, ca_contact_stats, ca_lddt_matrix, ca_native_contacts, ca_native_q, ca_lddt_per_residue, ca_pairwise_distances, ca_pwd_js, ca_rmsd_matrix,
                       ca_sample_stats, ca_scattering, ca_superpose, ca_tm_matrix, ca_tm_superpose, cluster_adjacency, cluster_gromos,
                       lddt_workspace_bytes, rmsd_row_chunk, secondary_structure, sphere_points)
from .geometry import forward_marginal, frames_to_backbone, rigid_compose_update, rigid_scale_trans, se3_step, torsion_head
from .hostio import (float64_normal_outputs, format_pdb_models, host_rng_can_discard, host_rng_discard_float64_normals,
                     host_rng_fast_forward_ok, merge_pdb_files, write_pdb_models)
from .node import (CHAIN_WIDTHS, NARROW_MAX_WORK, SMALL_ROWS, embed_assemble, ipa_projections, node_apply,
                   node_apply_chain, node_apply_multi, node_chain, node_linear, node_linear_f32, node_linear_multi, node_linear_vfrag,
                   pack_planes, row_layernorm, small_rows_variant, to_act)
from .packing import (NODE_TG, LazyDict, PairTiled, act_alloc, column_blocked, fragment_order, node_tiles, pack_f16x2_layer, pack_f16x3_embed_stream,
                      pack_f16x3_stream, pack_node_layer, pack_node_weight, pack_node_weight_f32, pack_weight, padded_len, pair_tiled,
                      pair_untiled, unpack_planes, vf_alloc, xp_alloc)
from .pair import edge_embed, edge_embed_f16x3, edge_transition, edge_transition_f16x3, pair_project
from .range_guard import (RANGE_BITS, RANGE_FAMILIES, range_families, range_flag, range_flag_names, range_flag_read, range_flag_reset,
                          range_headroom)
from .torch_ops import register_torch_ops

__all__ = [
    "ABI_VERSION", "EXPORTS", "LIB_PATH", "HipLibraryError", "KernelTimer", "WeightRangeError", "load_library",
    "RANGE_BITS", "RANGE_FAMILIES", "range_families", "range_flag", "range_flag_names", "range_flag_read", "range_flag_reset", "range_headroom",
    "NODE_TG", "LazyDict", "PairTiled", "act_alloc", "column_blocked", "fragment_order", "node_tiles", "pack_f16x2_layer", "pack_f16x3_embed_stream",
    "pack_f16x3_stream", "pack_node_layer", "pack_node_weight", "pack_node_weight_f32", "pack_weight", "padded_len", "pair_tiled", "pair_untiled",
    "unpack_planes", "vf_alloc", "xp_alloc",
    "edge_embed", "edge_embed_f16x3", "edge_transition", "edge_transition_f16x3", "pair_project",
    "encoder_attention", "ipa_attention", "ipa_attention_f16", "ipa_prep_points", "ipa_prep_points_f16",
    "CHAIN_WIDTHS", "NARROW_MAX_WORK", "SMALL_ROWS", "embed_assemble", "ipa_projections", "node_apply",
    "node_apply_chain", "node_apply_multi", "node_chain", "node_linear", "node_linear_f32", "node_linear_multi", "node_linear_vfrag", "pack_planes",
    "row_layernorm", "small_rows_variant", "to_act",
    "forward_marginal", "frames_to_backbone", "rigid_compose_update", "rigid_scale_trans", "se3_step", "torsion_head",
    "RMSD_LAUNCH_PAIRS", "apply_xform", "ca_pairwise_distances", "ca_pwd_js", "ca_rmsd_matrix", "ca_sample_stats", "ca_superpose", "rmsd_row_chunk",
    "TM_MAX_RES", "ca_tm_matrix", "ca_tm_superpose",
    "LDDT_MAX_RES", "ca_lddt_matrix", "ca_lddt_per_residue", "lddt_workspace_bytes",
    "VIOL_MAX_RES", "backbone_violations",
    "SS_MAX_RES", "secondary_structure",
    "SASA_MAX_POINTS", "SASA_MAX_RES", "backbone_sasa", "sphere_points",
    "SAXS_MAX_Q", "SAXS_MAX_RES", "SAXS_MAX_TYPES", "ca_scattering",
    "CONTACT_MAX_RES", "ca_contact_map", "ca_contact_stats", "ca_native_contacts", "ca_native_q",
    "CLUSTER_MAX_N", "cluster_adjacency", "cluster_gromos",
    "float64_normal_outputs", "format_pdb_models", "host_rng_can_discard", "host_rng_discard_float64_normals", "host_rng_fast_forward_ok",
    "merge_pdb_files", "write_pdb_models",
    "register_torch_ops",
]

register_torch_ops()
```

str2str_amd/ops/attention.py:

```python
from typing import Optional

import torch

from .binding import HipLibraryError, _check, _p, _req, _req_all, _req_opt, _stream, _timed, load_library
from .packing import padded_len, xp_alloc
from .range_guard import range_flag


def ipa_prep_points(rigids7, q_pts_lin, kv_pts_lin, n_heads=8, n_qk=8, n_v=12):
    lib = load_library()
    B, N = rigids7.shape[0], rigids7.shape[1]
    _req_all(rigids7=rigids7, q_pts_lin=q_pts_lin, kv_pts_lin=kv_pts_lin)
    dev = rigids7.device
    q_pts = torch.empty(B, N, n_heads, n_qk * 3, device=dev, dtype=torch.float32)
    k_pts = torch.empty(B, N, n_heads, n_qk * 3, device=dev, dtype=torch.float32)
    v_pts = torch.empty(B, N, n_heads, 64, device=dev, dtype=torch.float32)
    _check(lib.s2s_ipa_prep_points(_p(rigids7), _p(q_pts_lin), _p(kv_pts_lin), _p(q_pts), _p(k_pts), _p(v_pts), B * N,
                                   n_heads, n_qk, n_v, 64, _stream()), "s2s_ipa_prep_points")
    return q_pts, k_pts, v_pts


def ipa_attention(q, kv, q_pts, k_pts, v_pts, attn_bias, pair_z, mask, rigids7, head_w_scaled, n_heads=8, c_hidden=256,
                  n_qk=8, n_v=12, c_pz=32, inf=1e5, eps=1e-8, out=None, logits_inplace=False):
    lib = load_library()
    B, N = mask.shape
    _req_all(q=q, kv=kv, q_pts=q_pts, k_pts=k_pts, v_pts=v_pts, attn_bias=attn_bias, pair_z=pair_z, mask=mask, rigids7=rigids7, head_w=head_w_scaled)
    if attn_bias.shape != (B, n_heads, N, N) or pair_z.shape != (B, N, N, c_pz):
        raise HipLibraryError("ipa_attention: attn_bias must be [B,H,N,N] and pair_z [B,N,N,c_pz]")
    feat = n_heads * (c_hidden + 4 * n_v + c_pz)
    out = torch.empty(B, N, feat, device=q.device, dtype=torch.float32) if out is None else out
    logits = attn_bias if logits_inplace else torch.empty_like(attn_bias)
    stats = torch.empty(B, n_heads, N, 2, device=q.device, dtype=torch.float32)

    def launch():
        return (lib.s2s_ipa_attention(_p(q), _p(kv), _p(q_pts), _p(k_pts), _p(v_pts), _p(attn_bias), _p(logits), _p(stats), _p(mask),
                                      _p(rigids7), _p(head_w_scaled), _p(out), B, N, n_heads, c_hidden, n_qk, n_v, c_pz, inf, eps, _stream())
                or lib.s2s_ipa_opair(_p(logits), _p(stats), _p(pair_z), _p(out), B, N, n_heads, c_pz, feat, n_heads * (c_hidden + 4 * n_v), N, _stream()))

    _check(_timed("s2s_ipa_attention", launch), "s2s_ipa_attention/s2s_ipa_opair")
    return out


def ipa_prep_points_f16(rigids7, q_pts_lin, kv_pts_lin, head_w_scaled, n_heads=8, n_qk=8, n_v=12, c_hidden=256, s_xp=None):
    lib = load_library()
    _req_all(rigids7=rigids7, q_pts_lin=q_pts_lin, kv_pts_lin=kv_pts_lin, head_w=head_w_scaled)
    if rigids7.ndim != 3:
        raise HipLibraryError("ipa_prep_points_f16: rigids7 must be [B,N,7]")
    B, N = rigids7.shape[:2]
    dev, rt = rigids7.device, B * padded_len(N) // 32
    qp = torch.empty(rt * n_heads * 2 * 2 * 64 * 8, dtype=torch.int16, device=dev)
    kp = torch.empty_like(qp)
    vp = torch.empty(rt * n_heads * 4 * 2 * 64 * 8, dtype=torch.int16, device=dev)
    q2 = torch.empty(rt, n_heads, 32, dtype=torch.float32, device=dev)
    k2 = torch.empty_like(q2)
    k_sh = v_sh = None
    if s_xp is not None:
        _req(s_xp, torch.int16, "s_xp")
        if s_xp.numel() != ((B * N + 31) // 32) * 32 * 256 * 2:
            raise HipLibraryError("ipa_prep_points_f16: s_xp must hold the packed planes of a [B*N, 256] activation")
        v_sh = torch.empty(rt * 32 * 256 * 2, dtype=torch.int16, device=dev)
        k_sh = None if N % 32 == 0 else torch.empty_like(v_sh)
    _check(lib.s2s_ipa_prep_points_f16(_p(rigids7), _p(q_pts_lin), _p(kv_pts_lin), _p(head_w_scaled), _p(qp), _p(kp), _p(vp), _p(q2),
                                       _p(k2), B, N, n_heads, n_qk, n_v, c_hidden, _p(s_xp), _p(k_sh), _p(v_sh), _p(range_flag()),
                                       _stream()), "s2s_ipa_prep_points_f16")
    return (qp, kp, vp, q2, k2) if s_xp is None else (qp, kp, vp, q2, k2, k_sh, v_sh)


def ipa_attention_f16(q_xp, k_xp, v_vf, points, attn_bias, pair_z, mask, rigids7, n_heads=8, c_hidden=256, n_qk=8, n_v=12,
                      c_pz=32, inf=1e5, eps=1e-8, logits_inplace=False):
    lib = load_library()
    B, N = mask.shape
    qp, kp, vp, q2, k2 = points
    _req_all(attn_bias=attn_bias, pair_z=pair_z, mask=mask, rigids7=rigids7, q2=q2, k2=k2)
    _req_all(torch.int16, q_xp=q_xp, k_xp=k_xp, v_vf=v_vf, qp_xp=qp, kp_xp=kp, vp_vf=vp)
    NP = padded_len(N)
    if attn_bias.shape != (B, n_heads, N, N) or pair_z.shape != (B, N, N, c_pz):
        raise HipLibraryError("ipa_attention_f16: attn_bias must be [B,H,N,N] and pair_z [B,N,N,c_pz]")
    n_kv = 1 if (k_xp.numel() * n_heads == q_xp.numel() and n_heads > 1) else n_heads
    if (q_xp.numel() != B * NP * n_heads * c_hidden * 2 or v_vf.numel() != k_xp.numel() or q2.numel() != B * NP * n_heads
            or k_xp.numel() * (n_heads // n_kv) != q_xp.numel()):
        raise HipLibraryError("ipa_attention_f16: operand arrays do not hold padded_len(n_res) rows per sample")
    feat = n_heads * (c_hidden + 4 * n_v + c_pz)
    out = torch.empty(B, N, feat, device=mask.device, dtype=torch.float32)
    out_xp = xp_alloc(B * N, feat, mask.device)
    if NP != N:
        logits = torch.empty(B, n_heads, NP, NP, device=mask.device, dtype=torch.float32)
    else:
        logits = attn_bias if logits_inplace else torch.empty_like(attn_bias)
    stats = torch.empty(B, n_heads, N, 2, device=mask.device, dtype=torch.float32)

    def launch():
        return (lib.s2s_ipa_attention_f16w(_p(q_xp), _p(k_xp), _p(v_vf), _p(qp), _p(kp), _p(vp), _p(q2), _p(k2), _p(attn_bias), _p(logits),
                                           _p(stats), _p(mask), _p(rigids7), _p(out), _p(out_xp), feat // 16, B, N, n_heads, c_hidden,
                                           n_qk, n_v, c_pz, inf, eps, n_kv, _stream())
                or lib.s2s_ipa_opair(_p(logits), _p(stats), _p(pair_z), _p(out), B, N, n_heads, c_pz, feat, n_heads * (c_hidden + 4 * n_v), NP, _stream()))

    _check(_timed("s2s_ipa_attention", launch), "s2s_ipa_attention_f16w/s2s_ipa_opair")
    return out, out_xp


def encoder_attention(qkv: torch.Tensor, key_bias: Optional[torch.Tensor], n_samples: int, n_res: int, n_heads: int = 4,
                      want_f32: bool = False, want_xp: bool = True, arith: str = "f32"):
    lib = load_library()
    _req(qkv, name="qkv")
    M, D3 = qkv.shape
    D = D3 // 3
    if M != n_samples * n_res or D % n_heads:
        raise HipLibraryError("encoder_attention: bad shapes")
    _req_opt(key_bias=key_bias)
    out = torch.empty(M, D, device=qkv.device, dtype=torch.float32) if want_f32 else None
    oxp = xp_alloc(M, D, qkv.device) if want_xp else None
    if arith not in ("f32", "f16x3"):
        raise HipLibraryError(f"encoder_attention: arith {arith!r}")
    fn = lib.s2s_encoder_attention_f16x3 if arith == "f16x3" else lib.s2s_encoder_attention
    rw = _p(range_flag()) if want_xp or arith == "f16x3" else None
    _check(_timed("s2s_encoder_attention", lambda: fn(_p(qkv), _p(key_bias), _p(out), _p(oxp), n_samples, n_res, n_heads, D // n_heads,
                                                      rw, _stream())), "s2s_encoder_attention")
    return out, oxp
```

str2str_amd/ops/binding.py:

```python
import ctypes
import os
from typing import Optional

import torch

_PKG = os.path.dirname(os.path.dirname(os.path.abspath(__file__)))
LIB_PATH = os.environ.get("STR2STR_HIP_LIB") or os.path.join(_PKG, "libstr2str_hip.so")
ABI_VERSION = 40

_lib = None

_vp, _i, _f, _d, _ll = ctypes.c_void_p, ctypes.c_int, ctypes.c_float, ctypes.c_double, ctypes.c_longlong

_SIGNATURES = {
    "s2s_abi_version": [],
    "s2s_edge_transition": [_vp] * 12 + [_i, _i, _f, _vp, _vp, _vp, _vp, _vp],
    "s2s_edge_transition_f16x3": [_vp] * 9 + [_i, _i, _f, _i, _vp, _vp, _vp, _i, _vp, _vp],
    "s2s_edge_embed": [_vp] * 15 + [_i, _i, _i, _i, _i, _f, _vp, _vp, _vp, _vp, _vp],
    "s2s_edge_embed_f16x3": [_vp] * 14 + [_i, _i, _i, _i, _i, _f, _i, _vp, _vp, _vp, _vp, _vp],
    "s2s_pair_project": [_vp] * 5 + [_i, _i, _vp],
    "s2s_ipa_prep_points": [_vp] * 6 + [_ll, _i, _i, _i, _i, _vp],
    "s2s_ipa_attention": [_vp] * 12 + [_i, _i, _i, _i, _i, _i, _i, _f, _f, _vp],
    "s2s_ipa_opair": [_vp] * 4 + [_i, _i, _i, _i, _i, _i, _i, _vp],
    "s2s_ipa_prep_points_f16": [_vp] * 9 + [_i, _i, _i, _i, _i, _i, _vp, _vp, _vp, _vp, _vp],
    "s2s_ipa_attention_f16w": [_vp] * 15 + [_i] * 8 + [_f, _f, _i, _vp],
    "s2s_rigid_compose_update": [_vp] * 4 + [_ll, _i, _vp],
    "s2s_torsion_head": [_vp, _i, _i, _vp, _ll, _vp, _f, _vp, _ll, _vp],
    "s2s_rigid_scale_trans": [_vp, _vp, _ll, _f, _i, _vp],
    "s2s_set_backbone_tables": [_vp] * 4,
    "s2s_frames_to_backbone": [_vp] * 5 + [_ll, _vp],
    "s2s_se3_step": [_vp] * 12 + [_i, _i, _d, _vp, _d, _i, _i, _d, _vp],
    "s2s_forward_marginal": [_vp] * 7 + [_i, _vp, _vp, _f, _vp, _i, _i, _vp],
    "s2s_pack_planes": [_vp, _ll, _i, _i, _i, _vp, _i, _i, _vp, _vp, _vp],
    "s2s_node_linear": [_vp, _vp, _vp, _ll, _i, _i, _i, _vp, _i, _vp, _vp, _i, _vp, _vp, _f, _vp, _vp, _i, _i, _vp, _i, _i, _i, _i, _vp, _vp],
    "s2s_node_linear_f32": [_vp, _i, _vp, _vp, _ll, _i, _i, _i, _vp, _i, _vp, _vp, _i, _vp, _vp, _f, _vp, _vp, _i, _i, _vp],
    "s2s_node_linear_multi": [_vp, _i, _vp, _vp],
    "s2s_node_chain": [_vp, _vp, _i, _ll, _i, _i, _vp, _i, _vp, _i, _vp, _vp, _f, _vp, _vp, _i, _vp, _vp, _f, _vp, _vp, _i, _i, _vp, _i, _i, _vp, _vp],
    "s2s_embed_assemble": [_vp, _ll, _vp, _ll, _vp, _vp, _ll, _i, _vp, _vp, _vp, _vp, _i, _vp, _vp],
    "s2s_row_layernorm": [_vp, _i, _ll, _i, _vp, _vp, _f, _vp, _vp, _i, _i, _vp, _i, _i, _vp, _vp],
    "s2s_node_linear_vfrag": [_vp, _vp, _vp, _ll, _i, _i, _i, _vp, _i, _i, _vp, _vp],
    "s2s_encoder_attention": [_vp, _vp, _vp, _vp, _i, _i, _i, _i, _vp, _vp],
    "s2s_encoder_attention_f16x3": [_vp, _vp, _vp, _vp, _i, _i, _i, _i, _vp, _vp],
    "s2s_ca_sample_stats": [_vp, _i, _i, _f, _i, _vp, _vp, _vp, _vp],
    "s2s_ca_pairwise_distances": [_vp, _i, _i, _i, _vp, _vp],
    "s2s_ca_pwd_js": [_vp, _i, _vp, _i, _i, _i, _i, _d, _vp, _vp, _vp, _vp],
    "s2s_ca_rmsd_matrix": [_vp, _i, _vp, _i, _i, _vp, _vp, _vp, _ll, _vp],
    "s2s_ca_superpose": [_vp, _i, _vp, _i, _vp, _vp, _vp, _vp],
    "s2s_apply_xform": [_vp, _vp, _i, _ll, _vp, _vp],
    "s2s_ca_tm_matrix": [_vp, _i, _vp, _i, _i, _d, _vp, _vp],
    "s2s_ca_tm_superpose": [_vp, _i, _vp, _i, _d, _vp, _vp, _vp],
    "s2s_ca_lddt_matrix": [_vp, _i, _vp, _i, _i, _d, _i, _vp, _vp, _ll, _vp],
    "s2s_ca_lddt_per_residue": [_vp, _i, _vp, _i, _d, _i, _vp, _vp, _vp, _ll, _vp],
    "s2s_ca_contact_map": [_vp, _i, _i, _d, _i, _vp, _vp, _vp, _vp],
    "s2s_ca_contact_stats": [_vp, _i, _i, _d, _i, _vp, _vp, _vp],
    "s2s_ca_native_contacts": [_vp, _i, _d, _i, _vp, _vp, _vp, _vp],
    "s2s_ca_native_q": [_vp, _i, _i, _vp, _vp, _i, _d, _d, _vp, _vp, _vp, _vp],
    "s2s_backbone_violations": [_vp, _i, _i, _vp, _vp, _vp, _d, _d, _vp, _vp, _vp, _vp, _vp, _vp, _vp],
    "s2s_secondary_structure": [_vp, _i, _i, _vp, _vp, _vp, _vp, _vp, _vp, _vp, _vp],
    "s2s_backbone_sasa": [_vp, _i, _i, _vp, _vp, _d, _vp, _i, _vp, _vp, _vp, _vp],
    "s2s_ca_scattering": [_vp, _i, _i, _vp, _i, _vp, _vp, _i, _vp, _vp, _vp],
    "s2s_cluster_adjacency": [_vp, _i, _i, _i, _d, _i, _vp, _vp, _vp],
    "s2s_cluster_gromos": [_vp, _vp, _i, _i, _i, _vp, _vp, _vp, _vp, _vp, _vp, _vp],
    "s2s_format_pdb_models": [_vp, _i, _i, _vp, _vp, _vp, _vp, _i, _i, _vp, _ll],
    "s2s_write_pdb_models": [ctypes.c_char_p, _i, _vp, _i, _i, _vp, _vp, _vp, _vp, _i, _i],
    "s2s_merge_pdb_files": [_vp, _i, ctypes.c_char_p],
    "s2s_mt19937_discard": [_vp, _vp, _vp, ctypes.c_ulonglong],
}
_LL_RETURN = ("s2s_format_pdb_models", "s2s_write_pdb_models", "s2s_merge_pdb_files")
EXPORTS = tuple(_SIGNATURES)


class HipLibraryError(RuntimeError):
    pass


class WeightRangeError(HipLibraryError):
    """A weight does not fit the f16x3 packing (|32 w| >= 65504)."""


class KernelTimer:

    active = None

    def __init__(self, *names):
        self.names = set(names)
        self.events = {n: [] for n in names}
        self.work = {n: [0, 0] for n in names}

    def __enter__(self):
        KernelTimer.active = self if self.names else None
        return self

    def __exit__(self, *exc):
        KernelTimer.active = None

    def total_ms(self, name):
        torch.cuda.synchronize()
        ev = self.events[name]
        return sum(a.elapsed_time(b) for a, b in ev), len(ev)

    def mean_ms(self, name):
        total, n = self.total_ms(name)
        return (total / n if n else float("nan")), n


def _timed(name, launch, flops=0, nbytes=0):
    kt = KernelTimer.active
    if kt is None or name not in kt.names:
        return launch()
    kt.work[name][0] += int(flops)
    kt.work[name][1] += int(nbytes)
    a, b = torch.cuda.Event(enable_timing=True), torch.cuda.Event(enable_timing=True)
    a.record()
    rc = launch()
    b.record()
    kt.events[name].append((a, b))
    return rc


def load_library(path: Optional[str] = None):
    global _lib
    if _lib is not None and path is None:
        return _lib
    p = path or LIB_PATH
    if not os.path.exists(p):
        raise HipLibraryError(f"{p} not found: the HIP kernels are not built. Run `python -m str2str_amd.build` "
                              "(hipcc --offload-arch=gfx950). There is no CPU fallback for the sampling path.")
    lib = ctypes.CDLL(p)
    for name, args in _SIGNATURES.items():
        fn = getattr(lib, name)
        fn.argtypes = args
        fn.restype = ctypes.c_longlong if name in _LL_RETURN else ctypes.c_int
    v = lib.s2s_abi_version()
    if v != ABI_VERSION:
        raise HipLibraryError(f"libstr2str_hip.so ABI {v} != expected {ABI_VERSION}; rebuild")
    if path is None:
        _lib = lib
    return lib


def _check(rc: int, what: str):
    if rc != 0:
        raise HipLibraryError(f"{what} failed with hipError_t {rc}")


def _p(t: Optional[torch.Tensor]):
    return None if t is None else ctypes.c_void_p(t.data_ptr())


def _stream():
    return ctypes.c_void_p(torch.cuda.current_stream().cuda_stream)


def _req(t: torch.Tensor, dtype=torch.float32, name="tensor") -> torch.Tensor:
    if not isinstance(t, torch.Tensor) or not t.is_cuda:
        raise HipLibraryError(f"{name}: expected a tensor on the HIP device (no CPU fallback), got "
                              f"{getattr(t, 'device', type(t))}")
    if t.dtype != dtype:
        raise HipLibraryError(f"{name}: expected dtype {dtype}, got {t.dtype}")
    if not t.is_contiguous():
        raise HipLibraryError(f"{name}: expected a contiguous tensor")
    return t


def _req_all(dtype=torch.float32, /, **tensors):
    for name, t in tensors.items():
        _req(t, dtype, name)


def _req_opt(dtype=torch.float32, /, **tensors):
    _req_all(dtype, **{name: t for name, t in tensors.items() if t is not None})


def _int_arg(v: Optional[int]) -> int:
    return -1 if v is None else v


def _opt_int(v: Optional[int]) -> Optional[int]:
    return None if v is None or v < 0 else v
```

str2str_amd/ops/node.py:

```python
import ctypes
from typing import Optional

import torch

from .binding import HipLibraryError, _check, _int_arg, _p, _req, _req_all, _req_opt, _stream, _timed, load_library
from .packing import vf_alloc, xp_alloc
from .range_guard import range_flag

SMALL_ROWS = 8192
NARROW_MAX_WORK = 24 << 20
CHAIN_WIDTHS = (256, 320)


def _ln_args(ln, name=None):
    if ln is None:
        return None, None, 0.0
    g, b, eps = ln
    if name:
        _req(g, name=name + ".gamma"); _req(b, name=name + ".beta")
    return g, b, float(eps)


def _node_outputs(n_rows: int, n_out: int, dev, out_f32, want_f32, out_xp, out_xp_k, want_xp):
    if out_f32 is None and want_f32:
        out_f32 = torch.empty(n_rows, n_out, device=dev, dtype=torch.float32)
    if out_xp_k is None and (out_xp is not None or want_xp):
        out_xp_k = n_out
    if out_xp is None and want_xp:
        out_xp = xp_alloc(n_rows, out_xp_k, dev)
    return out_f32, out_xp, out_xp_k


def pack_planes(x2d: torch.Tensor, col0: int = 0, n_cols: Optional[int] = None, out=None, out_k: Optional[int] = None, k0: int = 0, row_scale=None):
    lib = load_library()
    _req(x2d, name="x")
    M, ld = x2d.shape
    n_cols = ld - col0 if n_cols is None else n_cols
    out_k = n_cols if out_k is None else out_k
    out = xp_alloc(M, out_k, x2d.device) if out is None else out
    _req_opt(row_scale=row_scale)
    _check(lib.s2s_pack_planes(_p(x2d), M, ld, col0, n_cols, _p(out), out_k // 16, k0 // 16, _p(row_scale), _p(range_flag()), _stream()), "s2s_pack_planes")
    return out


def to_act(x2d: torch.Tensor, arith: str) -> torch.Tensor:
    return pack_planes(x2d) if arith == "f16x3" else _req(x2d, name="x")


def node_linear(xp, wpk, bias, n_rows: int, k_in: int, n_out: int, tiles: int, *, pre_scale=None, relu=False, pre_mask=None,
                residual=None, ln=None, post_mask=None, out_f32=None, out_col0: int = 0, want_f32=True, out_xp=None,
                out_xp_k: Optional[int] = None, out_xp_k0: int = 0, want_xp=False, row_map: Optional[tuple] = None):
    lib = load_library()
    _req(xp, torch.int16, "xp"); _req(wpk, torch.int16, "w_packed")
    map_pad, map_src = row_map if row_map is not None else (0, 0)
    in_rows = n_rows // map_pad * map_src if map_pad else n_rows
    _req_opt(bias=bias, pre_scale=pre_scale, pre_mask=pre_mask, residual=residual, post_mask=post_mask)
    if xp.numel() != ((in_rows + 31) // 32) * (k_in // 16) * 1024 or wpk.numel() != n_out * k_in * 2:
        raise HipLibraryError(f"node_linear: operand sizes do not match M={in_rows} K={k_in} N={n_out}")
    out_f32, out_xp, out_xp_k = _node_outputs(n_rows, n_out, xp.device, out_f32, want_f32, out_xp, out_xp_k, want_xp)
    _req_opt(out_f32=out_f32)
    _req_opt(torch.int16, out_xp=out_xp)
    g, b, eps = _ln_args(ln, "ln")
    _check(_timed("s2s_node_linear", lambda: lib.s2s_node_linear(
        _p(xp), _p(wpk), _p(bias), n_rows, k_in, n_out, tiles, _p(pre_scale), int(bool(relu)), _p(pre_mask), _p(residual),
        residual.shape[-1] if residual is not None else 0, _p(g), _p(b), eps, _p(post_mask), _p(out_f32),
        out_f32.shape[-1] if out_f32 is not None else 0, out_col0, _p(out_xp), (out_xp_k or 0) // 16, out_xp_k0 // 16,
        map_pad, map_src, _p(range_flag()), _stream()), flops=2 * n_rows * k_in * n_out), "s2s_node_linear")
    return out_f32, out_xp


def node_linear_f32(x, wpk32, bias, n_rows: int, k_in: int, n_out: int, tiles: int, *, pre_scale=None, relu=False, pre_mask=None,
                    residual=None, ln=None, post_mask=None, out=None, out_col0: int = 0):
    lib = load_library()
    _req(x, name="x"); _req(wpk32, name="w_packed_f32")
    if x.ndim != 2 or x.shape[0] != n_rows or x.shape[1] < k_in or wpk32.numel() != n_out * k_in:
        raise HipLibraryError(f"node_linear_f32: operand sizes do not match M={n_rows} K={k_in} N={n_out}")
    _req_opt(bias=bias, pre_scale=pre_scale, pre_mask=pre_mask, residual=residual, post_mask=post_mask)
    out = torch.empty(n_rows, n_out, device=x.device, dtype=torch.float32) if out is None else out
    _req(out, name="out")
    g, b, eps = _ln_args(ln, "ln")
    _check(_timed("s2s_node_linear", lambda: lib.s2s_node_linear_f32(
        _p(x), x.shape[1], _p(wpk32), _p(bias), n_rows, k_in, n_out, tiles, _p(pre_scale), int(bool(relu)), _p(pre_mask), _p(residual),
        residual.shape[-1] if residual is not None else 0, _p(g), _p(b), eps, _p(post_mask), _p(out), out.shape[-1], out_col0,
        _stream()), flops=2 * n_rows * k_in * n_out), "s2s_node_linear_f32")
    return out


def small_rows_variant(layer: dict, n_rows: int):
    if n_rows * layer["n"] <= NARROW_MAX_WORK and layer.get("tg_s", layer["tg"]) != layer["tg"]:
        return "w_s", layer["tg_s"]
    return "w", layer["tg"]


def embed_assemble(t_img, node_const, fa, fb, n_samples: int, n_res: int, planes: bool, b_col_blocked: bool):
    lib = load_library()
    _req_all(t_img=t_img, node_const=node_const, fa=fa, fb=fb)
    M, dev = n_samples * n_res, t_img.device
    if (t_img.numel() not in (512, 512 * n_samples) or node_const.numel() not in (M * 256, n_res * 256) or fa.numel() != M * 128
            or fb.numel() != M * 128):
        raise HipLibraryError("embed_assemble: bad shapes")
    h = xp_alloc(M, 256, dev) if planes else torch.empty(M, 256, device=dev, dtype=torch.float32)
    node_a, node_b = torch.empty(n_samples, n_res, 128, device=dev, dtype=torch.float32), torch.empty_like(fb)
    _check(lib.s2s_embed_assemble(_p(t_img), t_img.numel() // 512 if t_img.numel() != 512 else 1, _p(node_const), node_const.numel() // 256,
                                  _p(fa), _p(fb), M, n_res, _p(h) if planes else None, None if planes else _p(h), _p(node_a), _p(node_b),
                                  int(b_col_blocked), _p(range_flag()), _stream()), "s2s_embed_assemble")
    return h, node_a, node_b


def row_layernorm(x, n_rows: int, n_cols: int, gamma, beta, eps: float, post_mask=None, out_f32=None, out_col0: int = 0, want_f32=True,
                  out_xp=None, out_xp_k: Optional[int] = None, out_xp_k0: int = 0, want_xp=False):
    lib = load_library()
    _req(x, name="x"); _req(gamma, name="ln.gamma"); _req(beta, name="ln.beta")
    _req_opt(post_mask=post_mask)
    out_f32, out_xp, out_xp_k = _node_outputs(n_rows, n_cols, x.device, out_f32, want_f32, out_xp, out_xp_k, want_xp)
    _check(_timed("s2s_node_linear", lambda: lib.s2s_row_layernorm(
        _p(x), x.shape[-1], n_rows, n_cols, _p(gamma), _p(beta), float(eps), _p(post_mask), _p(out_f32),
        out_f32.shape[-1] if out_f32 is not None else 0, out_col0, _p(out_xp), (out_xp_k or 0) // 16, out_xp_k0 // 16, _p(range_flag()),
        _stream())), "s2s_row_layernorm")
    return out_f32, out_xp


def node_apply(x, layer: dict, n_rows: int, *, out_f32=None, out_col0: int = 0, want_f32=True, out_xp=None, out_xp_k=None,
               out_xp_k0: int = 0, want_xp=False, **epilogue):
    T = torch.ops.str2str_amd
    ep = dict(epilogue)
    g, b, eps = _ln_args(ep.pop("ln", None))
    row_map = ep.pop("row_map", None)
    flat = (ep.pop("pre_scale", None), bool(ep.pop("relu", False)), ep.pop("pre_mask", None), ep.pop("residual", None), g, b, eps,
            ep.pop("post_mask", None))
    outs = (out_f32, out_col0, want_f32, out_xp, _int_arg(out_xp_k), out_xp_k0, want_xp)
    if ep:
        raise TypeError(f"node_apply: unexpected arguments {sorted(ep)}")
    if x.dtype == torch.int16 and g is not None and n_rows <= SMALL_ROWS and layer["k"] >= 1024 and layer["n"] in (256, 320) and row_map is None:
        pre = torch.empty(n_rows, layer["n"], device=x.device, dtype=torch.float32)
        T.node_linear(x, layer["w_n"], layer["b"], n_rows, layer["k"], layer["n"], 2, *flat[:4], None, None, 0.0, None, pre)
        return T.row_layernorm(pre, n_rows, layer["n"], g, b, eps, flat[7], *outs)
    if x.dtype == torch.int16:
        mp, ms = row_map if row_map is not None else (0, 0)
        wk, tg = small_rows_variant(layer, n_rows)
        return T.node_linear(x, layer[wk], layer["b"], n_rows, layer["k"], layer["n"], tg, *flat, *outs, mp, ms)
    if row_map is not None:
        raise HipLibraryError("node_apply: the row map belongs to the f16 attention operands")
    if out_f32 is not None and out_xp is not None and out_xp is not out_f32:
        raise HipLibraryError("node_apply (fp32): one output buffer")
    out, col0 = (out_f32, out_col0) if out_f32 is not None else (out_xp, out_xp_k0)
    y = T.node_linear_f32(x, layer["w32"], layer["b"], n_rows, layer["k"], layer["n"], layer["tg"], *flat, out, col0)
    return y, y


def node_linear_vfrag(xp, wpk, bias, n_rows: int, k_in: int, n_out: int, tiles_per_head: int = 8, out=None, row_map: Optional[tuple] = None):
    lib = load_library()
    _req(xp, torch.int16, "xp"); _req(wpk, torch.int16, "w_packed")
    _req_opt(bias=bias)
    out = _req(vf_alloc(n_rows, n_out, xp.device) if out is None else out, torch.int16, "out_vf")
    map_pad, map_src = row_map if row_map is not None else (0, 0)
    _check(_timed("s2s_node_linear", lambda: lib.s2s_node_linear_vfrag(_p(xp), _p(wpk), _p(bias), n_rows, k_in, n_out, tiles_per_head,
                                                                       _p(out), map_pad, map_src, _p(range_flag()), _stream()),
                  flops=2 * n_rows * k_in * n_out), "s2s_node_linear_vfrag")
    return out


class _NodeProblem(ctypes.Structure):
    _fields_ = [("xp", ctypes.c_void_p), ("w_packed", ctypes.c_void_p), ("bias", ctypes.c_void_p), ("n_rows", ctypes.c_longlong),
                ("k_in", ctypes.c_int), ("n_out", ctypes.c_int), ("tiles_per_block", ctypes.c_int), ("vfrag_tiles_per_head", ctypes.c_int),
                ("out_f32", ctypes.c_void_p), ("out_ld", ctypes.c_int), ("out_col0", ctypes.c_int), ("out_xp", ctypes.c_void_p),
                ("out_xp_ksteps", ctypes.c_int), ("out_xp_kstep0", ctypes.c_int), ("out_vf", ctypes.c_void_p), ("map_pad", ctypes.c_int),
                ("map_src", ctypes.c_int), ("relu", ctypes.c_int), ("pre_scale", ctypes.c_void_p)]


def _fill_problem(p, xp, w, bias, n_rows, k_in, n_out, tiles, **fields):
    p.xp, p.w_packed, p.bias = xp.data_ptr(), w.data_ptr(), bias.data_ptr()
    p.n_rows, p.k_in, p.n_out, p.tiles_per_block = n_rows, k_in, n_out, tiles
    for name, val in fields.items():
        setattr(p, name, val)


def _launch_problems(lib, arr, n):
    _check(_timed("s2s_node_linear", lambda: lib.s2s_node_linear_multi(ctypes.byref(arr), n, _p(range_flag()), _stream()),
                  flops=sum(2 * arr[i].n_rows * arr[i].k_in * arr[i].n_out for i in range(n))), "s2s_node_linear_multi")


def node_linear_multi(xp, w, bias, pre_scale, dims, out_f32, out_xp):
    lib = load_library()
    _req(xp, torch.int16, "xp")
    n = len(w)
    if not (1 <= n <= 6) or any(len(x) != n for x in (bias, pre_scale, out_f32, out_xp)) or len(dims) != 9 * n:
        raise HipLibraryError("node_linear_multi: 1 .. 6 layers, one entry per layer in every list, nine ints per layer")
    arr = (_NodeProblem * n)()
    for i in range(n):
        rows, k, nn, tg, ld, c0, xk, xk0, relu = (int(v) for v in dims[9 * i:9 * i + 9])
        fields = {"relu": relu}
        if pre_scale[i].numel():
            fields.update(pre_scale=_req(pre_scale[i], name="pre_scale").data_ptr())
        if out_f32[i].numel():
            fields.update(out_f32=_req(out_f32[i], name="out_f32").data_ptr(), out_ld=ld, out_col0=c0)
        if out_xp[i].numel():
            fields.update(out_xp=_req(out_xp[i], torch.int16, "out_xp").data_ptr(), out_xp_ksteps=xk // 16, out_xp_kstep0=xk0 // 16)
        _fill_problem(arr[i], xp, _req(w[i], torch.int16, "w"), _req(bias[i], name="bias"), rows, k, nn, tg, **fields)
    _launch_problems(lib, arr, n)


def ipa_projections(s_xp, q, k, v, qp, kvp, n_rows: int, n_rows_padded: int, row_map: Optional[tuple] = None, tiles_per_head: int = 8):
    lib = load_library()
    _req(s_xp, torch.int16, "xp")
    dev = s_xp.device
    mp, ms = row_map if row_map is not None else (0, 0)
    q_xp = xp_alloc(n_rows_padded, q["n"], dev)
    k_xp = xp_alloc(n_rows_padded, k["n"], dev) if k is not None else None
    v_vf = vf_alloc(n_rows_padded, v["n"], dev) if v is not None else None
    qp_o = torch.empty(n_rows, qp["n"], device=dev, dtype=torch.float32)
    kvp_o = torch.empty(n_rows, kvp["n"], device=dev, dtype=torch.float32)
    problems = [(q, n_rows_padded, dict(out_xp=q_xp.data_ptr(), out_xp_ksteps=q["n"] // 16, map_pad=mp, map_src=ms))]
    if k is not None:
        problems.append((k, n_rows_padded, dict(out_xp=k_xp.data_ptr(), out_xp_ksteps=k["n"] // 16, map_pad=mp, map_src=ms)))
    if v is not None:
        problems.append((v, n_rows_padded, dict(vfrag_tiles_per_head=tiles_per_head, out_vf=v_vf.data_ptr(), map_pad=mp, map_src=ms)))
    problems += [(qp, n_rows, dict(out_f32=qp_o.data_ptr(), out_ld=qp["n"])), (kvp, n_rows, dict(out_f32=kvp_o.data_ptr(), out_ld=kvp["n"]))]
    arr = (_NodeProblem * len(problems))()
    for p, (layer, rows, fields) in zip(arr, problems):
        _fill_problem(p, s_xp, layer["w"], layer["b"], rows, layer["k"], layer["n"], layer["tg"], **fields)
    _launch_problems(lib, arr, len(problems))
    return q_xp, k_xp, v_vf, qp_o, kvp_o


class _ChainLayer(ctypes.Structure):
    _fields_ = [("w_packed", ctypes.c_void_p), ("bias", ctypes.c_void_p), ("relu", ctypes.c_int)]


def node_chain(xp, w_row, bias, relu, n_rows: int, width: int, pre_mask=None, residual=None, ln_gamma=None, ln_beta=None, ln_eps: float = 0.0,
               post_mask=None, out_f32=None, out_col0: int = 0, want_f32=True, out_xp=None, out_xp_k: Optional[int] = None,
               out_xp_k0: int = 0, want_xp=False, k_in0: Optional[int] = None, mid_residual=None, mid_out_f32=None, mid_ln=None):
    lib = load_library()
    _req(xp, torch.int16, "xp")
    n = len(w_row)
    mg, mb, meps = _ln_args(mid_ln, "mid_ln")
    k0 = width if k_in0 is None else int(k_in0)
    if n not in (2, 3, 4) or len(bias) != n or len(relu) != n or width not in CHAIN_WIDTHS or (k0 != width and (width, k0) != (256, 320)):
        raise HipLibraryError("node_chain: 2 .. 4 layers of width 256 or 320 (first layer: 320 -> 256 allowed)")
    arr = (_ChainLayer * n)()
    for i in range(n):
        _req(w_row[i], torch.int16, "w_row"); _req(bias[i], name="bias")
        if w_row[i].numel() != width * (k0 if i == 0 else width) * 2 or bias[i].numel() < width:
            raise HipLibraryError("node_chain: weights must be packed with one column block of the layer's width")
        arr[i].w_packed, arr[i].bias, arr[i].relu = w_row[i].data_ptr(), bias[i].data_ptr(), int(bool(relu[i]))
    _req_opt(pre_mask=pre_mask, residual=residual, ln_gamma=ln_gamma, ln_beta=ln_beta, post_mask=post_mask, mid_residual=mid_residual,
             mid_out_f32=mid_out_f32)
    out_f32, out_xp, out_xp_k = _node_outputs(n_rows, width, xp.device, out_f32, want_f32, out_xp, out_xp_k, want_xp)
    _check(_timed("s2s_node_linear", lambda: lib.s2s_node_chain(
        _p(xp), ctypes.byref(arr), n, n_rows, width, k0, _p(mid_residual), mid_residual.shape[-1] if mid_residual is not None else 0,
        _p(mid_out_f32), mid_out_f32.shape[-1] if mid_out_f32 is not None else 0, _p(mg), _p(mb), meps, _p(pre_mask), _p(residual),
        residual.shape[-1] if residual is not None else 0, _p(ln_gamma), _p(ln_beta), float(ln_eps), _p(post_mask), _p(out_f32),
        out_f32.shape[-1] if out_f32 is not None else 0, out_col0, _p(out_xp), (out_xp_k or 0) // 16, out_xp_k0 // 16, _p(range_flag()),
        _stream()), flops=2 * n_rows * width * (k0 + (n - 1) * width)), "s2s_node_chain")
    return out_f32, out_xp


def node_apply_chain(x, layers, n_rows: int, relu, **kw):
    width = layers[0]["n"]
    first_res, first_out, first_ln = kw.pop("first_residual", None), kw.pop("first_out_f32", None), kw.pop("first_ln", None)
    k0 = layers[0]["k"]
    ok = (x.dtype == torch.int16 and len(layers) in (2, 3, 4) and width in CHAIN_WIDTHS and (k0 == width or (width, k0) == (256, 320))
          and all(L["n"] == width for L in layers) and all(L["k"] == width for L in layers[1:])
          and "pre_scale" not in kw and "row_map" not in kw)
    if ok and width == 320 and not (64 <= (n_rows + 127) // 128 <= 384):
        ok = False
    if not ok:
        act = x
        for i, L in enumerate(layers[:-1]):
            fk = dict(residual=first_res, out_f32=first_out, want_f32=first_out is not None, ln=first_ln) if i == 0 else dict(want_f32=False)
            _, act = node_apply(act, L, n_rows, relu=relu[i], want_xp=True, **fk)
        return node_apply(act, layers[-1], n_rows, relu=relu[-1], **kw)
    return torch.ops.str2str_amd.node_chain(x, [L["w_row"] for L in layers], [L["b"] for L in layers], [bool(r) for r in relu], n_rows, width,
                                            kw.get("pre_mask"), kw.get("residual"), *_ln_args(kw.get("ln")), kw.get("post_mask"),
                                            kw.get("out_f32"), kw.get("out_col0", 0), kw.get("want_f32", True), kw.get("out_xp"),
                                            _int_arg(kw.get("out_xp_k")), kw.get("out_xp_k0", 0), kw.get("want_xp", False), k0, first_res,
                                            first_out, *_ln_args(first_ln))


def node_apply_multi(x, specs, n_rows: int):
    if x.dtype != torch.int16 or len(specs) > 6 or len(specs) < 2:
        return [node_apply(x, layer, n_rows, **kw) for layer, kw in specs]
    dev = x.device
    empty_f, empty_i = torch.empty(0, device=dev), torch.empty(0, dtype=torch.int16, device=dev)
    w, bias, ps, dims, of, ox, res = [], [], [], [], [], [], []
    for layer, kw in specs:
        if set(kw) - {"relu", "pre_scale", "out_f32", "out_col0", "want_f32", "out_xp", "out_xp_k", "out_xp_k0", "want_xp"}:
            raise HipLibraryError(f"node_apply_multi: unsupported epilogue option in {sorted(kw)}")
        key, tg = small_rows_variant(layer, n_rows)
        o32, oxp, xk = _node_outputs(n_rows, layer["n"], dev, kw.get("out_f32"), kw.get("want_f32", True), kw.get("out_xp"),
                                     kw.get("out_xp_k"), kw.get("want_xp", False))
        w.append(layer[key]); bias.append(layer["b"]); ps.append(kw["pre_scale"] if kw.get("pre_scale") is not None else empty_f)
        dims += [n_rows, layer["k"], layer["n"], tg, o32.shape[-1] if o32 is not None else 0, kw.get("out_col0", 0), xk or 0,
                 kw.get("out_xp_k0", 0), int(bool(kw.get("relu", False)))]
        of.append(o32 if o32 is not None else empty_f); ox.append(oxp if oxp is not None else empty_i)
        res.append((o32, oxp))
    torch.ops.str2str_amd.node_linear_multi(x, w, bias, ps, dims, of, ox)
    return res
```

str2str_amd/ops/packing.py:

```python
from typing import Optional

import torch

from .binding import HipLibraryError, WeightRangeError


def _pad_rows32(w: torch.Tensor) -> torch.Tensor:
    pad = (-w.shape[0]) % 32
    return torch.cat([w, w.new_zeros(pad, w.shape[1])], dim=0) if pad else w


def pack_weight(w: torch.Tensor, tile_major: bool = False) -> torch.Tensor:
    k = w.shape[1]
    if k % 8:
        raise ValueError("K must be a multiple of 8")
    w = _pad_rows32(w)
    t, s4 = w.shape[0] // 32, k // 8
    perm = (0, 2, 3, 1, 4) if tile_major else (2, 0, 3, 1, 4)
    return w.reshape(t, 32, s4, 2, 4).permute(*perm).contiguous().reshape(-1)


def fragment_order(w: torch.Tensor, kind: str) -> torch.Tensor:
    mout, k = w.shape
    if mout % 32 or k % 32:
        raise ValueError("Mout and K must be multiples of 32")
    T, KS = mout // 32, k // 16
    ks = torch.arange(KS)[:, None, None]
    g = torch.arange(2)[None, :, None]
    j = torch.arange(8)[None, None, :]
    if kind == "row":
        lab = 16 * ks + 8 * g + j
    elif kind == "chain":
        r = 8 * (ks & 1) + j
        lab = 32 * (ks >> 1) + (r & 3) + 8 * (r >> 2) + 4 * g
    else:
        raise ValueError(kind)
    wg = w.float()[:, lab.to(w.device)]
    return wg.reshape(T, 32, KS, 2, 8).permute(2, 0, 3, 1, 4).reshape(KS, T, 64, 8).contiguous()


def pack_f16x2_layer(w: torch.Tensor, kind: str = "chain") -> torch.Tensor:
    wmax = float(w.detach().abs().max()) if w.numel() else 0.0
    if not (32.0 * wmax < 65504.0):
        raise WeightRangeError(f"|w| up to {wmax:.4g}: 32 w does not fit f16 (f16x3 weight packing)")
    planes = fragment_order(w, kind) * 32.0
    h = planes.to(torch.float16)
    ls = (planes - h.float()).to(torch.float16)
    return torch.stack([h, ls], dim=2).contiguous()


def pack_f16x3_stream(w1_edge: torch.Tensor, w2: torch.Tensor, wf: torch.Tensor) -> torch.Tensor:
    l1, l2, lf = pack_f16x2_layer(w1_edge), pack_f16x2_layer(w2), pack_f16x2_layer(wf)
    A = lambda t: l1[:, t]
    B = lambda t: l2[2 * t:2 * t + 2]
    pieces = [A(0), A(1)]
    for t in range(10):
        pieces += [B(t), A(t + 2)]
    b11 = B(11)
    pieces += [B(10), b11.reshape(2, 6, 2, *b11.shape[2:]).transpose(0, 1), lf]
    blob = torch.cat([x.contiguous().reshape(-1) for x in pieces]).view(torch.int16).contiguous()
    assert blob.numel() * 2 == 30 * 32 * 1024, blob.numel()
    return blob


class PairTiled:
    __slots__ = ("buf", "B", "N")

    def __init__(self, B: int, N: int, device=None, buf: Optional[torch.Tensor] = None):
        self.B, self.N = int(B), int(N)
        n = -(-(self.B * self.N * self.N) // 32) * 32 * 128
        self.buf = torch.empty(n, device=device, dtype=torch.float32) if buf is None else buf
        if self.buf.numel() != n or self.buf.dtype != torch.float32 or not self.buf.is_contiguous():
            raise HipLibraryError("PairTiled: buffer must be a contiguous fp32 tensor of whole 32-pair blocks")

    shape = property(lambda self: (self.B, self.N, self.N, 128))
    device = property(lambda self: self.buf.device)
    is_cuda = property(lambda self: self.buf.is_cuda)

    def data_ptr(self):
        return self.buf.data_ptr()

    def contiguous(self):
        return self


def pair_tiled(z: torch.Tensor) -> PairTiled:
    B, N = z.shape[0], z.shape[1]
    M = B * N * N
    t = PairTiled(B, N, z.device)
    zp = torch.zeros(t.buf.numel() // 128, 128, device=z.device, dtype=torch.float32)
    zp[:M] = z.reshape(M, 128)
    t.buf.copy_(zp.view(-1, 32, 16, 2, 4).permute(0, 2, 3, 1, 4).reshape(-1))
    return t


def pair_untiled(t: PairTiled) -> torch.Tensor:
    M = t.B * t.N * t.N
    return t.buf.view(-1, 16, 2, 32, 4).permute(0, 3, 1, 2, 4).reshape(-1, 128)[:M].reshape(t.B, t.N, t.N, 128).contiguous()


def column_blocked(t: torch.Tensor) -> torch.Tensor:
    *lead, rows, ch = t.shape
    return t.reshape(*lead, rows, ch // 4, 4).transpose(-3, -2).contiguous()


def pack_f16x3_embed_stream(w2: torch.Tensor, w3: torch.Tensor) -> torch.Tensor:
    blob = torch.cat([pack_f16x2_layer(w2, "chain").reshape(-1), pack_f16x2_layer(w3, "chain").reshape(-1)])
    blob = blob.view(torch.int16).contiguous()
    assert blob.numel() * 2 == 4 * 32 * 1024
    return blob


def padded_len(n_res: int) -> int:
    return (n_res + 31) // 32 * 32


NODE_TG = (10, 8, 6, 5, 4, 2, 1)


def node_tiles(n_out: int, whole_row: bool = False) -> int:
    if n_out % 32:
        raise ValueError("n_out must be a multiple of 32 (pad the weight)")
    t = n_out // 32
    if whole_row:
        if t not in NODE_TG:
            raise HipLibraryError(f"no node_linear instantiation holds a whole row of {n_out} columns")
        return t
    return next(g for g in NODE_TG if t % g == 0)


def pack_node_weight(w: torch.Tensor, tiles_per_block: int) -> torch.Tensor:
    w, k = _pad_rows32(w), w.shape[1]
    if k % 32 or (w.shape[0] // 32) % tiles_per_block:
        raise ValueError("k_in must be a multiple of 32 and n_out/32 of tiles_per_block")
    fr = pack_f16x2_layer(w.float(), "chain")
    KS, T = fr.shape[:2]
    fr = fr.reshape(KS, T // tiles_per_block, tiles_per_block, 2, 64, 8).permute(1, 0, 2, 3, 4, 5)
    return fr.contiguous().view(torch.int16).reshape(-1)


def pack_node_weight_f32(w: torch.Tensor, tiles_per_block: int) -> torch.Tensor:
    w, k = _pad_rows32(w), w.shape[1]
    if k % 8 or (w.shape[0] // 32) % tiles_per_block:
        raise ValueError("k_in must be a multiple of 8 and n_out/32 of tiles_per_block")
    T, S4 = w.shape[0] // 32, k // 8
    fr = w.float().reshape(T // tiles_per_block, tiles_per_block, 32, S4, 2, 4).permute(0, 3, 1, 4, 2, 5)
    return fr.contiguous().reshape(-1)


def pack_node_layer(w: torch.Tensor, bias, whole_row: bool = False) -> dict:
    n_out, k = w.shape
    n_pad = -(-n_out // 32) * 32
    tg = node_tiles(n_pad, whole_row=whole_row)
    b = w.new_zeros(n_pad, dtype=torch.float32)
    if bias is not None:
        b[:n_out] = bias.detach().float()
    t = n_pad // 32
    tg_s = tg if whole_row else (2 if t % 2 == 0 else tg)
    w = w.detach()

    def blocks(d, tiles):
        return d["w"] if tiles == tg else pack_node_weight(w.float(), tiles)

    return LazyDict({"b": b.contiguous(), "n": n_pad, "k": k, "tg": tg, "tg_s": tg_s}, w=lambda d: pack_node_weight(w.float(), tg),
                    w_s=lambda d: blocks(d, tg_s), w_row=lambda d: blocks(d, t), w_n=lambda d: blocks(d, 2),
                    w32=lambda d: pack_node_weight_f32(w.float(), tg))


class LazyDict(dict):

    def __init__(self, eager: dict, **lazy):
        super().__init__(eager)
        self._lazy = lazy

    def __missing__(self, key):
        if key not in self._lazy:
            raise KeyError(key)
        self[key] = self._lazy[key](self)
        return self[key]


def xp_alloc(n_rows: int, k: int, device) -> torch.Tensor:
    return torch.empty(((n_rows + 31) // 32) * (k // 16) * 2 * 64 * 8, dtype=torch.int16, device=device)


def vf_alloc(n_rows: int, n_out: int, device) -> torch.Tensor:
    return torch.empty(((n_rows + 31) // 32) * (n_out // 32) * 2 * 2 * 64 * 8, dtype=torch.int16, device=device)


def act_alloc(n_rows: int, k: int, device, arith: str) -> torch.Tensor:
    return xp_alloc(n_rows, k, device) if arith == "f16x3" else torch.empty(n_rows, k, device=device, dtype=torch.float32)


def unpack_planes(xp: torch.Tensor, n_rows: int, k: int) -> torch.Tensor:
    KS = k // 16
    fr = xp.view(torch.float16).reshape(-1, KS, 2, 2, 32, 8).float().sum(2)
    ks = torch.arange(KS)[:, None, None]
    g = torch.arange(2)[None, :, None]
    j = torch.arange(8)[None, None, :]
    r = 8 * (ks & 1) + j
    chan = (32 * (ks >> 1) + (r & 3) + 8 * (r >> 2) + 4 * g).to(xp.device)
    out = torch.zeros(fr.shape[0], 32, k, device=xp.device)
    out[:, :, chan.reshape(-1)] = fr.permute(0, 3, 1, 2, 4).reshape(fr.shape[0], 32, -1)
    return out.reshape(-1, k)[:n_rows]
```

str2str_amd/ops/torch_ops.py:

```python
import torch

from .attention import encoder_attention, ipa_attention, ipa_attention_f16, ipa_prep_points, ipa_prep_points_f16
from .binding import _opt_int
from .geometry import forward_marginal, frames_to_backbone, rigid_compose_update, rigid_scale_trans, se3_step, torsion_head
from .node import (embed_assemble, ipa_projections, node_chain, node_linear, node_linear_f32, node_linear_multi, node_linear_vfrag, pack_planes,
                   row_layernorm)
from .packing import PairTiled
from .pair import edge_embed, edge_embed_f16x3, edge_transition, edge_transition_f16x3, pair_project

_registered = False


def _ln3(g, b, eps):
    return None if g is None else (g, b, eps)


def _op_node_linear(xp, wpk, bias, n_rows, k_in, n_out, tiles, pre_scale=None, relu=False, pre_mask=None, residual=None, ln_gamma=None,
                    ln_beta=None, ln_eps=0.0, post_mask=None, out_f32=None, out_col0=0, want_f32=True, out_xp=None, out_xp_k=-1,
                    out_xp_k0=0, want_xp=False, map_pad=0, map_src=0):
    return node_linear(xp, wpk, bias, n_rows, k_in, n_out, tiles, pre_scale=pre_scale, relu=relu, pre_mask=pre_mask, residual=residual,
                       ln=_ln3(ln_gamma, ln_beta, ln_eps), post_mask=post_mask, out_f32=out_f32, out_col0=out_col0, want_f32=want_f32,
                       out_xp=out_xp, out_xp_k=_opt_int(out_xp_k), out_xp_k0=out_xp_k0, want_xp=want_xp,
                       row_map=(map_pad, map_src) if map_pad else None)


def _op_node_linear_f32(x, wpk32, bias, n_rows, k_in, n_out, tiles, pre_scale=None, relu=False, pre_mask=None, residual=None, ln_gamma=None,
                        ln_beta=None, ln_eps=0.0, post_mask=None, out=None, out_col0=0):
    return node_linear_f32(x, wpk32, bias, n_rows, k_in, n_out, tiles, pre_scale=pre_scale, relu=relu, pre_mask=pre_mask,
                           residual=residual, ln=_ln3(ln_gamma, ln_beta, ln_eps), post_mask=post_mask, out=out, out_col0=out_col0)


def _op_edge_transition_f16x3_chain(edge, in_tiled, B, N, node_ab, node_p, wstream, b2, gamma, beta, mask, ln_eps, proj_bias64,
                                    out_layout, prescale_exp=0, ab_kernel_form=False):
    e = PairTiled(B, N, buf=edge) if in_tiled else edge
    r = edge_transition_f16x3(e, node_ab, node_p, wstream, b2, gamma, beta, mask, ln_eps,
                              proj=None if proj_bias64 is None else (wstream, proj_bias64), out_layout=out_layout, prescale_exp=prescale_exp,
                              ab_kernel_form=ab_kernel_form)
    z, bias, pz = r if proj_bias64 is not None else (r, None, None)
    return (z.buf if isinstance(z, PairTiled) else z), bias, pz


_TORCH_OPS = {
    "edge_transition(Tensor edge, Tensor node_ab, Tensor node_p, Tensor w1p, Tensor w2p, Tensor wfp, Tensor b2, "
    "Tensor bf, Tensor gamma, Tensor beta, Tensor? mask, float ln_eps) -> Tensor": lambda *a: edge_transition(*a),
    "edge_transition_f16x3(Tensor edge, Tensor node_ab, Tensor node_p, Tensor wstream, Tensor b2, "
    "Tensor gamma, Tensor beta, Tensor? mask, float ln_eps, int prescale_exp=0) -> Tensor":
        lambda e, nab, np_, ws, b2, g, b, m, eps, pe=0: edge_transition_f16x3(e, nab, np_, ws, b2, g, b, m, eps, prescale_exp=pe),
    "edge_transition_f16x3_chain(Tensor edge, bool in_tiled, int B, int N, Tensor node_ab, Tensor node_p, Tensor wstream, Tensor b2, "
    "Tensor gamma, Tensor beta, Tensor? mask, float ln_eps, Tensor? proj_bias64, str out_layout, int prescale_exp=0, "
    "bool ab_kernel_form=False) -> (Tensor?, Tensor?, Tensor?)": _op_edge_transition_f16x3_chain,
    "edge_embed(Tensor node_a, Tensor node_b, Tensor rel_table, Tensor bin_table, Tensor bin_lower, Tensor residue_idx, Tensor ca, "
    "Tensor w2p, Tensor w3p, Tensor b2, Tensor b3, Tensor gamma, Tensor beta, Tensor? mask, int rel_offset, float ln_eps) -> Tensor":
        lambda *a: edge_embed(*a),
    "edge_embed_f16x3(Tensor node_a, Tensor node_b, Tensor rel_table, Tensor bin_table, Tensor bin_lower, Tensor residue_idx, Tensor ca, "
    "Tensor wstream, Tensor b2, Tensor b3, Tensor gamma, Tensor beta, Tensor? mask, int rel_offset, float ln_eps) -> Tensor":
        lambda *a: edge_embed_f16x3(*a),
    "pair_project(Tensor edge, Tensor wp, Tensor bias64) -> (Tensor, Tensor)": lambda *a: pair_project(*a),
    "ipa_prep_points(Tensor rigids7, Tensor q_pts_lin, Tensor kv_pts_lin, int n_heads=8, int n_qk=8, int n_v=12) -> (Tensor, Tensor, Tensor)":
        lambda *a: ipa_prep_points(*a),
    "ipa_attention(Tensor q, Tensor kv, Tensor q_pts, Tensor k_pts, Tensor v_pts, Tensor attn_bias, Tensor pair_z, "
    "Tensor mask, Tensor rigids7, Tensor head_w) -> Tensor": lambda *a: ipa_attention(*a),
    "ipa_prep_points_f16(Tensor rigids7, Tensor q_pts_lin, Tensor kv_pts_lin, Tensor head_w, int n_heads=8, int n_qk=8, int n_v=12, "
    "int c_hidden=256) -> (Tensor, Tensor, Tensor, Tensor, Tensor)": lambda *a: ipa_prep_points_f16(*a),
    "ipa_prep_points_shared_kv(Tensor rigids7, Tensor q_pts_lin, Tensor kv_pts_lin, Tensor head_w, Tensor s_xp, int n_heads=8, int n_qk=8, "
    "int n_v=12, int c_hidden=256) -> (Tensor, Tensor, Tensor, Tensor, Tensor, Tensor?, Tensor)":
        lambda r7, qp, kvp, hw, s_xp, h=8, nq=8, nv=12, c=256: ipa_prep_points_f16(r7, qp, kvp, hw, h, nq, nv, c, s_xp),
    "ipa_attention_f16w(Tensor q_xp, Tensor k_xp, Tensor v_vf, Tensor qp_xp, Tensor kp_xp, Tensor vp_vf, Tensor q2, Tensor k2, "
    "Tensor(a!) attn_bias, Tensor pair_z, Tensor mask, Tensor rigids7, int n_heads=8, int c_hidden=256, int n_qk=8, int n_v=12, int c_pz=32, "
    "float inf=1e5, float eps=1e-8, bool logits_inplace=False) -> (Tensor, Tensor)":
        lambda q, k, v, qp, kp, vp, q2, k2, ab, pz, m, r7, *rest: ipa_attention_f16(q, k, v, (qp, kp, vp, q2, k2), ab, pz, m, r7, *rest),
    "encoder_attention(Tensor qkv, Tensor? key_bias, int n_samples, int n_res, int n_heads=4, bool want_f32=False, bool want_xp=True, "
    "str arith='f32') -> (Tensor?, Tensor?)": lambda *a: encoder_attention(*a),
    "node_linear(Tensor xp, Tensor wpk, Tensor? bias, int n_rows, int k_in, int n_out, int tiles, Tensor? pre_scale=None, bool relu=False, "
    "Tensor? pre_mask=None, Tensor? residual=None, Tensor? ln_gamma=None, Tensor? ln_beta=None, float ln_eps=0.0, Tensor? post_mask=None, "
    "Tensor(a!)? out_f32=None, int out_col0=0, bool want_f32=True, Tensor(b!)? out_xp=None, int out_xp_k=-1, int out_xp_k0=0, "
    "bool want_xp=False, int map_pad=0, int map_src=0) -> (Tensor?, Tensor?)": _op_node_linear,
    "node_linear_f32(Tensor x, Tensor wpk32, Tensor? bias, int n_rows, int k_in, int n_out, int tiles, Tensor? pre_scale=None, "
    "bool relu=False, Tensor? pre_mask=None, Tensor? residual=None, Tensor? ln_gamma=None, Tensor? ln_beta=None, float ln_eps=0.0, "
    "Tensor? post_mask=None, Tensor(a!)? out=None, int out_col0=0) -> Tensor": _op_node_linear_f32,
    "node_linear_vfrag(Tensor xp, Tensor wpk, Tensor? bias, int n_rows, int k_in, int n_out, int tiles_per_head=8, int map_pad=0, "
    "int map_src=0) -> Tensor":
        lambda xp, w, b, m, k, n, tph=8, mp=0, ms=0: node_linear_vfrag(xp, w, b, m, k, n, tph, row_map=(mp, ms) if mp else None),
    "ipa_projections(Tensor s_xp, Tensor[] q, Tensor[] k, Tensor[] v, Tensor[] qp, Tensor[] kvp, int[] dims, int n_rows, int n_rows_padded, "
    "int map_pad=0, int map_src=0) -> (Tensor, Tensor?, Tensor?, Tensor, Tensor)":
        lambda s_xp, q, k, v, qp, kvp, dims, m, mo, mp=0, ms=0: ipa_projections(
            s_xp, *[({"w": t[0], "b": t[1], "k": dims[3 * i], "n": dims[3 * i + 1], "tg": dims[3 * i + 2]} if len(t) else None)
                    for i, t in enumerate((q, k, v, qp, kvp))],
            m, mo, (mp, ms) if mp else None),
    "embed_assemble(Tensor t_img, Tensor node_const, Tensor fa, Tensor fb, int n_samples, int n_res, bool planes, bool b_col_blocked) "
    "-> (Tensor, Tensor, Tensor)": lambda *a: embed_assemble(*a),
    "node_linear_multi(Tensor xp, Tensor[] w, Tensor[] bias, Tensor[] pre_scale, int[] dims, Tensor(a!)[] out_f32, Tensor(b!)[] out_xp) -> ()":
        lambda *a: node_linear_multi(*a),
    "node_chain(Tensor xp, Tensor[] w_row, Tensor[] bias, bool[] relu, int n_rows, int width, Tensor? pre_mask=None, Tensor? residual=None, "
    "Tensor? ln_gamma=None, Tensor? ln_beta=None, float ln_eps=0.0, Tensor? post_mask=None, Tensor(a!)? out_f32=None, int out_col0=0, "
    "bool want_f32=True, Tensor(b!)? out_xp=None, int out_xp_k=-1, int out_xp_k0=0, bool want_xp=False, int k_in0=-1, "
    "Tensor? mid_residual=None, Tensor(c!)? mid_out_f32=None, Tensor? mid_ln_gamma=None, Tensor? mid_ln_beta=None, float mid_ln_eps=0.0) "
    "-> (Tensor?, Tensor?)":
        lambda xp, w, b, r, m, wd, pm=None, res=None, g=None, be=None, eps=0.0, pom=None, of=None, oc=0, wf=True, ox=None, ok=-1, ok0=0, wx=False,
        k0=-1, mr=None, mo=None, mg=None, mb=None, me=0.0: node_chain(
            xp, w, b, r, m, wd, pm, res, g, be, eps, pom, of, oc, wf, ox, _opt_int(ok), ok0, wx, _opt_int(k0), mr, mo, _ln3(mg, mb, me)),
    "row_layernorm(Tensor x, int n_rows, int n_cols, Tensor gamma, Tensor beta, float eps, Tensor? post_mask=None, Tensor(a!)? out_f32=None, "
    "int out_col0=0, bool want_f32=True, Tensor(b!)? out_xp=None, int out_xp_k=-1, int out_xp_k0=0, bool want_xp=False) -> (Tensor?, Tensor?)":
        lambda x, m, n, g, b, eps, pm=None, of=None, oc=0, wf=True, ox=None, ok=-1, ok0=0, wx=False: row_layernorm(
            x, m, n, g, b, eps, pm, of, oc, wf, ox, _opt_int(ok), ok0, wx),
    "pack_planes(Tensor x, int col0=0, int n_cols=-1, Tensor(a!)? out=None, int out_k=-1, int k0=0, Tensor? row_scale=None) -> Tensor":
        lambda x, c0=0, nc=-1, out=None, ok=-1, k0=0, rs=None: pack_planes(x, c0, _opt_int(nc), out, _opt_int(ok), k0, rs),
    "se3_step(Tensor x0_7, Tensor xt_7, Tensor mask, Tensor diffuse_mask, Tensor params8, float dt) -> Tensor":
        lambda x0, xt, m, dm, p8, dt: se3_step(x0, xt, m, dm, p8, dt)[0],
    "forward_marginal(Tensor? rigids0_4x4, Tensor z_axis, Tensor u01, Tensor z_trans, Tensor cdf_rows, Tensor row_of_sample, "
    "Tensor omega_grid, Tensor? params2, Tensor? diffuse_mask=None, float coordinate_scaling=0.1) -> Tensor":
        lambda *a: forward_marginal(*a),
    "rigid_compose_update(Tensor rigids7, Tensor update6, Tensor mask) -> Tensor": lambda *a: rigid_compose_update(*a),
    "rigid_scale_trans(Tensor rigids7, float scale, bool divide=False) -> Tensor": lambda *a: rigid_scale_trans(*a),
    "torsion_head(Tensor u, int n_rows, bool normalize=True, float eps=1e-8, Tensor? gt_sin_cos=None, Tensor? fixed_mask=None) -> Tensor":
        lambda *a: torsion_head(*a),
    "frames_to_backbone(Tensor rigids7, Tensor psi, Tensor? aatype) -> Tensor": lambda r, p, a: frames_to_backbone(r, p, a)[0],
}


def register_torch_ops():
    global _registered
    if _registered:
        return
    lib = torch.library.Library("str2str_amd", "DEF")
    impl = torch.library.Library("str2str_amd", "IMPL", "CUDA")
    for schema, fn in _TORCH_OPS.items():
        lib.define(schema)
        impl.impl(schema.split("(")[0], fn)
    register_torch_ops._libs = (lib, impl)
    _registered = True
```

str2str_amd/sampler.py:

```python
from __future__ import annotations

import contextlib
import logging
import os
from typing import Optional, Tuple

import numpy as np
import torch

from . import ops
from .arith import FAMILIES, net_arith, use_arith
from .common.all_atom import compute_backbone
from .common.rigid_utils import Rigid

_REPEAT_KEYS = ("aatype", "residue_mask", "fixed_mask", "residue_idx", "torsion_angles_sin_cos")
_log = logging.getLogger("str2str_amd.sampler")
_GRAPH_MAX_PAIRS = 1 << 16
_GRAPH_MIN_STEPS = 16


class _GraphedNet:

    def __init__(self, net, feats):
        self.feats = dict(feats)
        self.static = tuple(k for k in ("rigids_t", "sc_ca_t", "t_img") if k in feats)
        for k in self.static:
            self.feats[k] = feats[k].clone()
        side = torch.cuda.Stream()
        side.wait_stream(torch.cuda.current_stream())
        with torch.cuda.stream(side):
            for _ in range(2):
                _net_eval(net, self.feats, True)
        torch.cuda.current_stream().wait_stream(side)
        self.graph = torch.cuda.CUDAGraph()
        with torch.cuda.graph(self.graph):
            self.out = _net_eval(net, self.feats, True)
        self._pinned = _graph_read_tensors(net)

    def __call__(self, feats):
        for k in self.static:
            self.feats[k].copy_(feats[k])
        self.graph.replay()
        return self.out


def _graph_read_tensors(net):
    from .models.net.layers import DerivedCache

    def tensors(x, out):
        if torch.is_tensor(x):
            out.append(x)
        elif isinstance(x, dict):
            for v in x.values():
                tensors(v, out)
        elif isinstance(x, (list, tuple)):
            for v in x:
                tensors(v, out)
        return out

    keep = []
    for m in net.modules():
        for v in vars(m).values():
            if isinstance(v, DerivedCache):
                tensors(v.held(), keep)
    return keep


def _net_eval(net, feats, defer_psi: bool):
    if defer_psi and hasattr(net, "blend_psi"):
        return net(feats, as_tensor_7=False, defer_psi_blend=True)
    return net(feats, as_tensor_7=False)


_GRAPH_CACHE = {}
_GRAPH_CACHE_MAX = 4


def _graph_key(net, feats, b, N):
    import hashlib

    h = hashlib.sha1()
    for k in sorted(feats):
        v = feats[k]
        if k in ("rigids_t", "sc_ca_t", "t_img", "t") or not torch.is_tensor(v):
            continue
        h.update(k.encode()); h.update(str(tuple(v.shape)).encode()); h.update(v.detach().cpu().numpy().tobytes())
    modes = tuple((type(m).__name__, a, getattr(m, a)) for m in net.modules() for a in getattr(type(m), "launch_switches", ()))
    return (id(net), sum(p._version for p in net.parameters()), b, N, modes, h.hexdigest())


def _maybe_graph(net, feats, b, N, trace, n_steps):
    mode = os.environ.get("S2S_HIP_GRAPH", "auto")
    if mode == "0" or trace is not None or ops.KernelTimer.active is not None:
        return None
    if mode != "1" and (b * N * N > _GRAPH_MAX_PAIRS or n_steps < _GRAPH_MIN_STEPS):
        return None
    key = _graph_key(net, feats, b, N)
    hit = _GRAPH_CACHE.get(key)
    if hit is not None:
        return hit
    try:
        g = _GraphedNet(net, feats)
    except ops.HipLibraryError:
        raise
    except RuntimeError as e:
        _log.warning("HIP graph capture failed (%s); continuing with eager launches", repr(e)[:200])
        torch.cuda.synchronize()
        return None
    if len(_GRAPH_CACHE) >= _GRAPH_CACHE_MAX:
        _GRAPH_CACHE.pop(next(iter(_GRAPH_CACHE)))
    _GRAPH_CACHE[key] = g
    return g


def schedule(t_delta: float, num_timesteps: int, min_t: float):
    T = t_delta if t_delta > 0 else 1.0
    n = int(float(num_timesteps) * T)
    return T, n, 1.0 / n, np.linspace(min_t, T, n)[::-1]


def shard_range(total: int, rank: int, world: int) -> Tuple[int, int]:
    per = -(-total // world)
    lo = min(total, rank * per)
    return lo, min(total, lo + per)


def rank_chunk_slices(n_replica: int, replica_per_batch: int, rank: int, world: int):
    my_lo, my_hi = shard_range(n_replica, rank, world)
    sizes = [replica_per_batch] * (n_replica // replica_per_batch)
    if n_replica % replica_per_batch > 0:
        sizes.append(n_replica % replica_per_batch)
    out, c0 = [], 0
    for bsz in sizes:
        lo, hi = max(my_lo, c0) - c0, min(my_hi, c0 + bsz) - c0
        out.append((bsz, lo, hi) if hi > lo else (bsz, 0, 0))
        c0 += bsz
    return out


@torch.no_grad()
def denoise_loop(net, diffuser, feats: dict, rigids_t: torch.Tensor, ts, dt: float, *, min_t: float,
                 noise_scale: float = 1.0, probability_flow: bool = True, self_conditioning: bool = True,
                 center_mode: int = 1, host_noise=None, trace: Optional[list] = None):
    if float(ts[-1]) != min_t:
        raise ValueError(f"the schedule ends at t = {float(ts[-1])}, not at min_t = {min_t}: its last evaluation is the sample")
    return _guarded_pass(net, diffuser, [dict(rigids_t=rigids_t, ts=ts, dt=dt, feats=feats)], noise_scale=noise_scale,
                         probability_flow=probability_flow, self_conditioning=self_conditioning, center_mode=center_mode,
                         host_noise=host_noise, trace=trace)[0]


def _guarded_pass(net, diffuser, groups, *, probability_flow: bool, host_noise, trace: Optional[list] = None, **kw):
    def run_pass():
        return _denoise_pass(net, diffuser, groups, probability_flow=probability_flow, host_noise=host_noise, trace=trace, **kw)

    return _range_guarded(net, run_pass, groups[0]["rigids_t"].device, host_draws=host_noise is not None,
                          device_draws=host_noise is None and not probability_flow, trace=trace)[0]


def _range_guarded(net, run_pass, device, *, host_draws: bool, device_draws: bool, trace: Optional[list] = None):
    if net_arith(net) == "f32":
        out = run_pass()
        _require_finite(out[1], "fp32")
        return out
    demoted = set(getattr(net, "range_fallback", None) or ())
    rng_state = torch.cuda.get_rng_state(device) if device_draws else None
    host_state = torch.get_rng_state() if host_draws else None
    while True:
        if host_state is not None:
            torch.set_rng_state(host_state)
        ops.range_flag_reset(device)
        try:
            with use_arith(net, "f32", families=tuple(demoted)):
                out = run_pass()
            finite = bool(torch.isfinite(out[1]).all())
            bits = ops.range_flag_read(device)
            if bits == 0 and finite:
                return out
            new = set(ops.range_families(bits)) - demoted
            why = f"an activation left f16's safe range in the split-f16 kernels ({ops.range_flag_names(bits)}{'' if finite else '; non-finite frames'})"
            if "edge_transition" in new:
                e_now = _raise_edge_prescale(net)
                if e_now:
                    new.discard("edge_transition")
                    _log.warning("range guard: %s; the edge transitions keep the split-f16 kernel with a block exponent of %d on their "
                                 "hidden activations (planes of 2^-%d x the value: exact, same speed; usable range 2^%d) -- re-running this chunk",
                                 why, e_now, e_now, 15 + e_now)
                    net.range_prescale = {"edge_transition": e_now}
                    if not new:
                        if trace is not None:
                            del trace[:]
                        if rng_state is not None:
                            torch.cuda.set_rng_state(rng_state, device)
                        continue
        except ops.WeightRangeError as e:
            new = set(FAMILIES) - demoted
            if not new:
                raise
            why = f"a weight does not fit the split-f16 packing ({e})"
        if not new:
            if len(demoted) == len(FAMILIES):
                _require_finite(out[1], "fp32 (range fallback)")
                return out
            new = set(FAMILIES) - demoted
        demoted |= new
        _log.warning("range guard: %s; re-running this chunk with the %s kernels on exact fp32 and keeping them there (now in fp32: %s; "
                     "S2S_ARITH=f32 starts everything in fp32)", why, " + ".join(sorted(new)), ", ".join(sorted(demoted)))
        net.range_fallback = frozenset(demoted)
        if trace is not None:
            del trace[:]
        if rng_state is not None:
            torch.cuda.set_rng_state(rng_state, device)


def _raise_edge_prescale(net, step: int = 5, top: int = 15) -> int:
    mods = [m for m in net.modules() if hasattr(m, "prescale_exp") and getattr(m, "arith", None) == "f16x3"]
    cur = max((int(m.prescale_exp) for m in mods), default=top)
    if not mods or cur >= top:
        return 0
    for m in mods:
        m.prescale_exp = min(cur + step, top)
    return min(cur + step, top)


def _require_finite(rigids7, what):
    if not bool(torch.isfinite(rigids7).all()):
        raise ops.HipLibraryError(f"non-finite frames at the end of the trajectory in the {what} arithmetic: the network itself "
                                  "overflows fp32 on this input (weights / checkpoint?)")


@contextlib.contextmanager
def _backbone_deferred(net):
    keep = getattr(net, "backbone_in_forward", None)
    if keep is not None:
        net.backbone_in_forward = False
    try:
        yield
    finally:
        if keep is not None:
            net.backbone_in_forward = keep


def _denoise_pass(net, diffuser, groups, *, noise_scale: float, probability_flow: bool, self_conditioning: bool, center_mode: int,
                  host_noise, trace: Optional[list]):
    device = groups[0]["rigids_t"].device
    N = groups[0]["rigids_t"].shape[1]
    emb = net.embedder
    order = sorted(range(len(groups)), key=lambda k: -len(groups[k]["ts"]))
    n_max = len(groups[order[0]]["ts"])
    per_sample = len(groups) > 1
    timg, p8s, base, o = [], [], {}, 0
    for k in order:
        t_all = torch.as_tensor(np.ascontiguousarray(groups[k]["ts"], dtype=np.float64)).float()
        p8s.append(diffuser.step_params(t_all).to(device))
        timg.append(emb.time_images(emb.time_embed(t_all).to(device)))
        base[k] = o
        o += len(t_all)
    TIMG, P8 = (torch.cat(timg).contiguous(), torch.cat(p8s).contiguous()) if per_sample else (timg[0], p8s[0])
    defer_psi = trace is None

    def eager(f):
        return _net_eval(net, f, defer_psi)

    with _backbone_deferred(net):
        rig = sc = idx = dtv = feats = mask = diffuse_mask = graphed = None
        members, run = [], eager
        for g in range(n_max):
            joining = [k for k in order if n_max - len(groups[k]["ts"]) == g]
            for k in joining:
                rk = groups[k]["rigids_t"]
                bk = rk.shape[0]
                fk = dict(groups[k]["feats"])
                for m in ("residue_mask", "fixed_mask"):
                    fk[m] = fk[m].to(device).float().contiguous()
                fk.update(rigids_t=rk, sc_ca_t=torch.zeros(bk, N, 3, device=device), t=torch.zeros(bk), t_img=TIMG[base[k]])
                if not per_sample:
                    graphed = _maybe_graph(net, fk, bk, N, trace, n_max)
                    run = graphed if graphed is not None else eager
                sck = fk["sc_ca_t"]
                if self_conditioning:
                    sck = run(fk)["rigids7"][..., 4:].clone()
                rig = rk if rig is None else torch.cat([rig, rk])
                sc = sck if sc is None else torch.cat([sc, sck])
                if per_sample:
                    ik = torch.full((bk,), base[k], dtype=torch.int64, device=device)
                    dk = torch.full((bk,), float(groups[k]["dt"]), dtype=torch.float64, device=device)
                    idx = ik if idx is None else torch.cat([idx, ik])
                    dtv = dk if dtv is None else torch.cat([dtv, dk])
                members.append((k, bk, fk))
            b = rig.shape[0]
            if joining:
                if len(members) == 1:
                    feats = members[0][2]
                else:
                    feats = {key: torch.cat([f[key].to(device) for _, _, f in members]) for key in _REPEAT_KEYS if key in members[0][2]}
                    feats["t"] = torch.zeros(b)
                mask = feats["residue_mask"]
                diffuse_mask = ((1 - feats["fixed_mask"]) * mask).contiguous()
            feats["rigids_t"], feats["sc_ca_t"] = rig, sc
            feats["t_img"] = TIMG.index_select(0, idx) if per_sample else TIMG[g]
            out = run(feats)
            x0_7 = out["rigids7"]
            t = float(groups[order[0]]["ts"][g])
            if g == n_max - 1:
                if trace is not None:
                    trace.append(dict(t=t, rigids_t=rig, sc_ca_t=sc, x0=x0_7, psi=out["psi"]))
                break
            sc_in = sc
            if self_conditioning:
                sc = x0_7[..., 4:].clone() if graphed is not None else x0_7[..., 4:]
            z = host_noise() if host_noise is not None else None
            z_rot, z_trans = z if z is not None else (None, None)
            if not probability_flow and z_rot is None:
                z_rot = torch.randn(b, N, 3, dtype=torch.float64, device=device)
                z_trans = torch.randn(b, N, 3, dtype=torch.float64, device=device)
            p8, dt = (P8.index_select(0, idx), dtv) if per_sample else (P8[g].expand(b, 8).contiguous(), groups[0]["dt"])
            nxt, rs, tsc = diffuser.step(x0_7, rig, p8, dt, mask, diffuse_mask, center_trans=center_mode, noise_scale=noise_scale,
                                         probability_flow=probability_flow, z_rot=z_rot, z_trans=z_trans, want_scores=trace is not None)
            if trace is not None:
                trace.append(dict(t=t, rigids_t=rig, sc_ca_t=sc_in, x0=x0_7, psi=out["psi"], rot_score=rs, trans_score=tsc, next7=nxt))
            rig = nxt
            if per_sample:
                idx = idx + 1
        psi = out["psi"]
        if out.get("psi_deferred"):
            psi = net.blend_psi(psi, feats["torsion_angles_sin_cos"], feats["fixed_mask"])
        atom37 = compute_backbone(out["rigids"], psi, aatype=feats.get("aatype"), _rigids7=x0_7)[0]
    samples, o = [None] * len(groups), 0
    for k, bk, _ in members:
        samples[k] = (atom37[o:o + bk], x0_7[o:o + bk], psi[o:o + bk])
        o += bk
    return samples, x0_7


def _require_hip_device(device, net) -> torch.device:
    device = torch.device(device) if device is not None else next(net.parameters()).device
    if device.type != "cuda":
        raise ops.HipLibraryError("the sampler needs the HIP device (MI355X); there is no CPU fallback")
    return device


def _start_frames(diffuser, batch: dict, rigids_0: Rigid, t_delta: float, lo: int, hi: int, rng: str, device):
    B_total, N = rigids_0.shape[0], rigids_0.shape[1]
    b = hi - lo
    if rng == "device":
        if b == 0:
            return None
        if t_delta > 0:
            dmask = batch["residue_mask"].to(device).float().reshape(1, N).expand(b, N).contiguous()
            return diffuser.forward_marginal_device(rigids_0[lo:hi].to_tensor_4x4().to(device), t_delta, dmask)
        return diffuser.forward_marginal_device(None, None, shape=(b, N))
    nt, keep = int(os.environ.get("S2S_HOST_FM_THREADS", "1")), torch.get_num_threads()
    if nt > 0 and nt != keep:
        torch.set_num_threads(nt)
    try:
        if t_delta > 0:
            rigids_t = diffuser.forward_marginal(rigids_0=rigids_0.to(device="cpu"), t=t_delta * torch.ones(B_total),
                                                 diffuse_mask=batch["residue_mask"].cpu().repeat(B_total, 1),
                                                 as_tensor_7=True)["rigids_t"]
        else:
            rigids_t = diffuser.sample_prior(shape=rigids_0.shape, device="cpu", as_tensor_7=True)["rigids_t"]
    finally:
        if nt > 0 and nt != keep:
            torch.set_num_threads(keep)
    if b == 0:
        return None
    return rigids_t[lo:hi].to(device).float().contiguous()


def _burn_step_draws(B_total: int, N: int, n_draw_steps: int):
    if ops.host_rng_discard_float64_normals(B_total * N * 3, 2 * n_draw_steps):
        return
    for _ in range(n_draw_steps):
        torch.randn(B_total, N, 3, dtype=torch.float64)
        torch.randn(B_total, N, 3, dtype=torch.float64)


def _skips_unused_draws(probability_flow: bool, B_total: int, N: int) -> bool:
    return probability_flow and ops.host_rng_can_discard(B_total * N * 3)


def _chunk_rigids(gt_frames_4x4: torch.Tensor, bsz: int) -> Rigid:
    return Rigid.from_tensor_4x4(gt_frames_4x4.repeat(bsz, *(1,) * (gt_frames_4x4.ndim - 1)))


def _expand_features(batch: dict, b: int, device) -> dict:
    return {k: batch[k].to(device).repeat(b, *(1,) * (batch[k].ndim - 1)) for k in _REPEAT_KEYS if k in batch}


def _draw_entries(diffuser, batch: dict, rig0, N: int, scheds, entries, *, rng: str, probability_flow: bool, device):
    n_max = max(scheds[i][1] for i, _, _, _ in entries)
# ... 241 lines not shown
```

Measured before the change: 29.29 conformations/s.

## Emit encoder Q/K/V directly in attention fragment layout from in-projection GEMM

Adds an encoder in-projection path that runs three GEMMs in one multi-problem launch. Q and K come out as f16 hi/lo planes in the order the attention kernel consumes, with the softmax scale folded into Q, and V comes out as padded per-head fragments. The attention kernel gains a FRAG variant that loads these pre-split tiles directly instead of reading the f32 qkv tensor and splitting it to f16 inside the kernel. The final encoder layer also skips its f32 output. The new path is on by default behind S2S_ENC_FRAG; it adds weight repacking and padded buffers, and changes rounding slightly because the scale is applied before the split.

```diff
diff --git a/include/str2str_hip.h b/include/str2str_hip.h
--- a/include/str2str_hip.h
+++ b/include/str2str_hip.h
@@ -135,6 +135,12 @@
 int s2s_encoder_attention_f16x3(const float* qkv, const float* key_bias, float* out_f32, void* out_xp, int n_samples, int n_res,
                           int n_heads, int head_dim, int* range_words, void* stream);
 
+int s2s_encoder_in_proj(const void* xp, const void* wq_packed, const float* bq, const void* wk_packed, const float* bk,
+                        const void* wv_packed, const float* bv, long long n_rows, int k_in, int n_heads, int head_dim, void* q_xp,
+                        void* k_xp, void* v_vf, int map_pad, int map_src, int* range_words, void* stream);
+int s2s_encoder_attention_frag(const void* q_xp, const void* k_xp, const void* v_vf, const float* key_bias, float* out_f32, void* out_xp,
+                               int n_samples, int n_res, int n_pad, int n_heads, int* range_words, void* stream);
+
 
 int s2s_forward_marginal(const float* rigids0_4x4, const float* z_axis, const float* u01, const float* z_trans,
                          const double* cdf_rows, const int* cdf_row_of_sample, const float* omega_grid, int n_omega,
diff --git a/str2str_amd/csrc/enc_attention.hip b/str2str_amd/csrc/enc_attention.hip
--- a/str2str_amd/csrc/enc_attention.hip
+++ b/str2str_amd/csrc/enc_attention.hip
@@ -176,10 +176,11 @@
     pl = __builtin_bit_cast(f16x8, u32x4{l0, l1, l2, l3});
 }
 
-template <int DH>
-__global__ void __launch_bounds__(256, 2) enc_attention_f16_kernel(const float* __restrict__ qkv, const float* __restrict__ key_bias,
-                                                                float* __restrict__ out_f32, bf16x8* __restrict__ out_xp, int* range_flag, int B,
-                                                                int N, int heads, float scale) {
+template <int DH, bool FRAG>
+__global__ void __launch_bounds__(256, 2) enc_attention_f16_kernel(const float* __restrict__ qkv, const f16x8* __restrict__ q_xp,
+                                                                const f16x8* __restrict__ k_xp, const f16x8* __restrict__ v_vf, int n_pad,
+                                                                const float* __restrict__ key_bias, float* __restrict__ out_f32,
+                                                                bf16x8* __restrict__ out_xp, int* range_flag, int B, int N, int heads, float scale) {
     static_assert(DH == 80, "built for the reference configuration (d_model 320, 4 heads)");
     constexpr int KSQ = DH / 16;
     constexpr int CT = (DH + 31) / 32;
@@ -197,13 +198,26 @@
     const int i = qb * 128 + wave * 32 + c;
     const bool ivalid = i < N;
     const long long row_i = (long long)b * N + (ivalid ? i : N - 1);
-    const float* base = qkv + (long long)b * N * 3 * D + head * DH;
+    const float* base = FRAG ? nullptr : qkv + (long long)b * N * 3 * D + head * DH;
     float amax = 0.f;
 
-    float4 st[5];
+    constexpr int kKF = KSQ * 2 * 64, kVF = CT * 2 * 2 * 64;
+    const long long rt0 = FRAG ? (long long)b * (n_pad >> 5) : 0;
+    const f16x8* kbase = FRAG ? k_xp + ((rt0 * (D / 16) + KSQ * head) * 2) * 64 : nullptr;
+    const f16x8* vbase = FRAG ? v_vf + (rt0 * heads + head) * kVF : nullptr;
+    float4 st[FRAG ? 1 : 5];
+    f16x8 stf[FRAG ? 6 : 1];
     auto tile_load = [&](int j0) {
-#pragma unroll
-        for (int k = 0; k < 5; ++k) {
+        const f16x8* kt = kbase + (long long)(j0 >> 5) * (D / 16) * 128;
+        const f16x8* vt = vbase + (long long)(j0 >> 5) * heads * kVF;
+#pragma unroll
+        for (int k = 0; k < (FRAG ? 6 : 0); ++k) {
+            const int idx = threadIdx.x + 256 * k;
+            if (idx < kKF) stf[k] = kt[idx];
+            else if (idx < kKF + kVF) stf[k] = vt[idx - kKF];
+        }
+#pragma unroll
+        for (int k = 0; k < (FRAG ? 0 : 5); ++k) {
             const int idx = threadIdx.x + 256 * k;
             const int which = idx / 640, rem = idx % 640, r = rem / 20, c4 = rem % 20;
             const int j = min(j0 + r, N - 1);
@@ -212,7 +226,13 @@
     };
     auto tile_store = [&](int par, int j0) {
 #pragma unroll
-        for (int k = 0; k < 5; ++k) {
+        for (int k = 0; k < (FRAG ? 6 : 0); ++k) {
+            const int idx = threadIdx.x + 256 * k;
+            if (idx < kKF) s_kf[par][idx] = stf[k];
+            else if (idx < kKF + kVF) s_vf[par][idx - kKF] = stf[k];
+        }
+#pragma unroll
+        for (int k = 0; k < (FRAG ? 0 : 5); ++k) {
             const int idx = threadIdx.x + 256 * k;
             const int which = idx / 640, rem = idx % 640, r = rem / 20, c4 = rem % 20;
             unsigned h0, h1, l0, l1;
@@ -240,14 +260,19 @@
             s_b[par][threadIdx.x] = j < N ? (key_bias ? key_bias[(long long)b * N + j] : 0.f) : -INFINITY;
         }
     };
-    for (int idx = threadIdx.x; idx < 2 * 2 * 2 * 64; idx += 256) {
+    for (int idx = threadIdx.x; idx < (FRAG ? 0 : 2 * 2 * 2 * 64); idx += 256) {
         const int par = idx >> 8, rest = idx & 255, ln = rest & 63;
         if ((ln & 31) >= DH - 32 * (CT - 1)) s_vf[par][((CT - 1) * 2 * 2) * 64 + rest] = f16x8{0, 0, 0, 0, 0, 0, 0, 0};
     }
 
     tile_load(0);
     f16x8 qh[KSQ], ql[KSQ];
-    {
+    if constexpr (FRAG) {
+        const int it = min(qb * 128 + wave * 32, n_pad - 32);
+        const f16x8* qp = q_xp + (((rt0 + (it >> 5)) * (D / 16) + KSQ * head) * 2) * 64 + lane;
+#pragma unroll
+        for (int ks = 0; ks < KSQ; ++ks) { qh[ks] = qp[(ks * 2) * 64]; ql[ks] = qp[(ks * 2 + 1) * 64]; }
+    } else {
         const float* qrow = qkv + row_i * 3 * D + head * DH + 8 * h;
 #pragma unroll
         for (int ks = 0; ks < KSQ; ++ks) {
@@ -365,8 +390,21 @@
     if (n_samples <= 0 || n_res <= 0) return 0;
     if (!qkv || (!out_f32 && !out_xp) || head_dim != 80 || n_heads < 1 || (n_heads * head_dim) % 32) return (int)hipErrorInvalidValue;
     const long long blocks = (long long)n_samples * n_heads * ((n_res + 127) / 128);
-    hipLaunchKernelGGL((enc_attention_f16_kernel<80>), dim3((unsigned)blocks), dim3(256), 0, (hipStream_t)stream, qkv, key_bias, out_f32,
-                       (bf16x8*)out_xp, range_words, n_samples, n_res, n_heads, 1.0f / sqrtf((float)head_dim));
+    hipLaunchKernelGGL((enc_attention_f16_kernel<80, false>), dim3((unsigned)blocks), dim3(256), 0, (hipStream_t)stream, qkv, nullptr, nullptr,
+                       nullptr, 0, key_bias, out_f32, (bf16x8*)out_xp, range_words, n_samples, n_res, n_heads, 1.0f / sqrtf((float)head_dim));
+    return (int)hipGetLastError();
+}
+
+extern "C" int s2s_encoder_attention_frag(const void* q_xp, const void* k_xp, const void* v_vf, const float* key_bias, float* out_f32,
+                                          void* out_xp, int n_samples, int n_res, int n_pad, int n_heads, int* range_words, void* stream) {
+    if (n_samples <= 0 || n_res <= 0) return 0;
+    if (!q_xp || !k_xp || !v_vf || (!out_f32 && !out_xp) || n_heads < 1 || (n_heads * 80) % 32 || n_pad % 32 || n_pad < n_res ||
+        n_pad - n_res >= 32)
+        return (int)hipErrorInvalidValue;
+    const long long blocks = (long long)n_samples * n_heads * ((n_res + 127) / 128);
+    hipLaunchKernelGGL((enc_attention_f16_kernel<80, true>), dim3((unsigned)blocks), dim3(256), 0, (hipStream_t)stream, nullptr,
+                       (const f16x8*)q_xp, (const f16x8*)k_xp, (const f16x8*)v_vf, n_pad, key_bias, out_f32, (bf16x8*)out_xp, range_words,
+                       n_samples, n_res, n_heads, 1.0f);
     return (int)hipGetLastError();
 }
 
diff --git a/str2str_amd/csrc/node_gemm.hip b/str2str_amd/csrc/node_gemm.hip
--- a/str2str_amd/csrc/node_gemm.hip
+++ b/str2str_amd/csrc/node_gemm.hip
@@ -46,6 +46,7 @@
     int x_ld;
     int* range_flag;
     int map_pad, map_src;
+    float out_scale = 1.0f;
 };
 
 __device__ float s2s_zero[512];
@@ -125,6 +126,13 @@
     }
     if (a.post_mask) {
         const float q = a.post_mask[rowc];
+#pragma unroll
+        for (int t = 0; t < TG; ++t)
+#pragma unroll
+            for (int r = 0; r < 16; ++r) acc[t][r] *= q;
+    }
+    if (a.out_scale != 1.0f) {
+        const float q = a.out_scale;
 #pragma unroll
         for (int t = 0; t < TG; ++t)
 #pragma unroll
@@ -322,6 +330,7 @@
         case 4: node_gemm_body<10, 4, false>(a, bx, by); break;
         case 5: node_gemm_body<4, 4, false>(a, bx, by); break;
         case 6: node_gemm_body<2, 4, false>(a, bx, by); break;
+        case 8: node_gemm_body<6, 4, true>(a, bx, by); break;
         default: node_gemm_body<1, 4, false>(a, bx, by); break;
     }
 }
@@ -764,7 +773,7 @@
     return (int)hipGetLastError();
 }
 
-extern "C" int s2s_node_linear_multi(const s2s_node_problem* pr, int n, int* range_words, void* stream) {
+static int launch_multi(const s2s_node_problem* pr, const float* out_scale, int vf_tiles, int n, int* range_words, void* stream) {
     if (n <= 0) return 0;
     if (!pr || n > kMultiMax) return (int)hipErrorInvalidValue;
     MultiArgs ma{};
@@ -773,14 +782,14 @@
     for (int i = 0; i < n; ++i) {
         const s2s_node_problem& q = pr[i];
         const bool vf = q.vfrag_tiles_per_head > 0;
-        const int TG = vf ? 8 : q.tiles_per_block;
+        const int TG = vf ? vf_tiles : q.tiles_per_block;
         if (q.n_rows <= 0 || !q.xp || !q.w_packed || q.k_in <= 0 || q.k_in % 32 || q.n_out <= 0 || TG <= 0 || q.n_out % (32 * TG) ||
             q.map_pad < 0 || (q.map_pad > 0 && (q.map_src <= 0 || q.map_src > q.map_pad || q.map_pad % 32 || q.n_rows % q.map_pad)))
             return (int)hipErrorInvalidValue;
         int kind;
         if (vf) {
             if (!q.out_vf || (q.n_out / 32) % q.vfrag_tiles_per_head) return (int)hipErrorInvalidValue;
-            kind = 1;
+            kind = TG == 8 ? 1 : 8;
         } else {
             if ((!q.out_f32 && !q.out_xp) || check_epilogue(q.n_out, TG, nullptr, nullptr, q.out_f32, q.out_ld, q.out_col0, nullptr, 0) ||
                 (q.out_xp && (q.out_xp_kstep0 < 0 || q.out_xp_kstep0 % 2 || q.out_xp_kstep0 + q.n_out / 16 > q.out_xp_ksteps)))
@@ -792,7 +801,7 @@
         ma.a[i] = GemmArgs{(const f16x8*)q.xp, (const char*)q.w_packed, q.bias, q.pre_scale, nullptr, nullptr, nullptr, nullptr, nullptr,
                            vf ? nullptr : q.out_f32, vf ? nullptr : (f16x8*)q.out_xp, vf ? (f16x8*)q.out_vf : nullptr,
                            vf ? q.vfrag_tiles_per_head : 0, q.n_rows, q.k_in / 16, ncb, 0, q.out_ld, q.out_col0, q.out_xp_ksteps,
-                           q.out_xp_kstep0, q.relu, 0.f, 0, range_words, q.map_pad, q.map_src};
+                           q.out_xp_kstep0, q.relu, 0.f, 0, range_words, q.map_pad, q.map_src, out_scale ? out_scale[i] : 1.0f};
         ma.kind[i] = kind;
         const long long n_rt = (q.n_rows + 31) / 32;
         ma.nx[i] = (int)((n_rt + 3) / 4);
@@ -804,6 +813,30 @@
     constexpr int lds = 2 * 2 * 10 * 1024;
     hipLaunchKernelGGL(node_gemm_multi_kernel, dim3((unsigned)total), dim3(256), lds, (hipStream_t)stream, ma);
     return (int)hipGetLastError();
+}
+
+extern "C" int s2s_node_linear_multi(const s2s_node_problem* pr, int n, int* range_words, void* stream) {
+    return launch_multi(pr, nullptr, 8, n, range_words, stream);
+}
+
+extern "C" int s2s_encoder_in_proj(const void* xp, const void* wq_packed, const float* bq, const void* wk_packed, const float* bk,
+                                   const void* wv_packed, const float* bv, long long n_rows, int k_in, int n_heads, int head_dim,
+                                   void* q_xp, void* k_xp, void* v_vf, int map_pad, int map_src, int* range_words, void* stream) {
+    if (n_rows <= 0) return 0;
+    const int D = n_heads * head_dim;
+    if (head_dim != 80 || n_heads < 2 || n_heads % 2 || D != 320 || !wq_packed || !wk_packed || !wv_packed || !bq || !bk || !bv || !q_xp ||
+        !k_xp || !v_vf)
+        return (int)hipErrorInvalidValue;
+    s2s_node_problem pr[3] = {};
+    for (int i = 0; i < 3; ++i) {
+        pr[i].xp = xp; pr[i].n_rows = n_rows; pr[i].k_in = k_in; pr[i].map_pad = map_pad; pr[i].map_src = map_src;
+    }
+    pr[0].w_packed = wq_packed; pr[0].bias = bq; pr[0].n_out = D; pr[0].tiles_per_block = D / 32; pr[0].out_xp = q_xp; pr[0].out_xp_ksteps = D / 16;
+    pr[1].w_packed = wk_packed; pr[1].bias = bk; pr[1].n_out = D; pr[1].tiles_per_block = D / 32; pr[1].out_xp = k_xp; pr[1].out_xp_ksteps = D / 16;
+    pr[2].w_packed = wv_packed; pr[2].bias = bv; pr[2].n_out = 96 * n_heads; pr[2].tiles_per_block = 6; pr[2].vfrag_tiles_per_head = 3;
+    pr[2].out_vf = v_vf;
+    const float scales[3] = {1.0f / sqrtf((float)head_dim), 1.0f, 1.0f};
+    return launch_multi(pr, scales, 6, 3, range_words, stream);
 }
 
 extern "C" int s2s_row_layernorm(const float* x, int x_ld, long long n_rows, int n_cols, const float* ln_gamma, const float* ln_beta,
diff --git a/str2str_amd/models/net/ipa.py b/str2str_amd/models/net/ipa.py
--- a/str2str_amd/models/net/ipa.py
+++ b/str2str_amd/models/net/ipa.py
@@ -185,6 +185,7 @@
 
 class TranslationIPA(nn.Module):
     launch_switches = ("exact_padding", "fuse_pair_projection", "arith")
+    ab_switches = ("enc_frag",)
 
     def __init__(self, c_s: int, c_z: int, coordinate_scaling: float, no_ipa_blocks: int, skip_embed_size: int,
                  transformer_num_heads: int = 4, transformer_num_layers: int = 2, c_hidden: int = 256, no_heads: int = 8,
@@ -216,6 +217,7 @@
         self.exact_padding = False
         self.fuse_pair_projection = True
         self.arith = default_arith()
+        self.enc_frag = os.environ.get("S2S_ENC_FRAG", "1") != "0"
 
     def _node_weights(self):
         def build():
@@ -229,7 +231,10 @@
                 d["layers"] = []
                 for layer in T[f"transformer_{b}"].layers:
                     att = layer.self_attn
-                    d["layers"].append({"in": ops.pack_node_layer(att.in_proj_weight, att.in_proj_bias), "o": pk(att.out_proj, True),
+                    d["layers"].append({"in": ops.pack_node_layer(att.in_proj_weight, att.in_proj_bias),
+                                        "fr": ops.LazyDict({}, pack=lambda _d, att=att: ops.pack_encoder_in_proj(
+                                            att.in_proj_weight, att.in_proj_bias, att.num_heads)),
+                                        "o": pk(att.out_proj, True),
                                         "l1": pk(layer.linear1), "l2": pk(layer.linear2, True)})
                 out[b] = d
             tp = self.torsion_pred
@@ -296,13 +301,22 @@
             if skip_done is None:
                 lin(init_a, w["skip"], out_f32=x_f32, out_col0=C, out_xp=x_a, out_xp_k=D, out_xp_k0=C)
             xf, xx = x_f32, x_a
-            for layer, lw in zip(T[f"transformer_{b}"].layers, w["layers"]):
-                qkv, _ = lin(xx, lw["in"])
-                sa_f32, sa_xp = torch.ops.str2str_amd.encoder_attention(qkv, key_bias, B, N, layer.self_attn.num_heads, not f16, f16, self.arith)
+            frag = f16 and self.enc_frag
+            n_enc = len(w["layers"])
+            for li, (layer, lw) in enumerate(zip(T[f"transformer_{b}"].layers, w["layers"])):
+                heads = layer.self_attn.num_heads
+                if frag:
+                    fp = lw["fr"]["pack"]
+                    q_xp, k_xp, v_vf = torch.ops.str2str_amd.encoder_in_proj(xx, [fp[k] for k in ("wq", "bq", "wk", "bk", "wv", "bv")], heads, B, N)
+                    sa_f32, sa_xp = torch.ops.str2str_amd.encoder_attention_frag(q_xp, k_xp, v_vf, key_bias, B, N, heads, False, True)
+                else:
+                    qkv, _ = lin(xx, lw["in"])
+                    sa_f32, sa_xp = torch.ops.str2str_amd.encoder_attention(qkv, key_bias, B, N, heads, not f16, f16, self.arith)
                 x1 = torch.empty(M, D, device=dev, dtype=torch.float32)
                 xf, xx = ops.node_apply_chain(sa_xp if f16 else sa_f32, [lw["o"], lw["l1"], lw["l2"]], M, (False, True, False),
                                               first_residual=xf, first_out_f32=x1, first_ln=(layer.norm1.weight, layer.norm1.bias, layer.norm1.eps),
-                                              residual=x1, ln=(layer.norm2.weight, layer.norm2.bias, layer.norm2.eps), want_xp=True)
+                                              residual=x1, ln=(layer.norm2.weight, layer.norm2.bias, layer.norm2.eps), want_xp=True,
+                                              want_f32=not (frag and li == n_enc - 1))
             nt = T[f"node_transition_{b}"]
             n_f32 = torch.empty(M, C, device=dev, dtype=torch.float32)
             s_f32, s_a = ops.node_apply_chain(xx, [w["lin"], w["nt1"], w["nt2"], w["nt3"]], M, (False, True, True, False),
diff --git a/str2str_amd/ops/__init__.py b/str2str_amd/ops/__init__.py
--- a/str2str_amd/ops/__init__.py
+++ b/str2str_amd/ops/__init__.py
@@ -1,4 +1,4 @@
-from .attention import encoder_attention, ipa_attention, ipa_attention_f16, ipa_prep_points, ipa_prep_points_f16
+from .attention import encoder_attention, encoder_attention_frag, ipa_attention, ipa_attention_f16, ipa_prep_points, ipa_prep_points_f16
 from .binding import ABI_VERSION, EXPORTS, LIB_PATH, HipLibraryError, KernelTimer, WeightRangeError, load_library
 from .ensemble import (CLUSTER_MAX_N, CONTACT_MAX_RES, LDDT_MAX_RES, RMSD_LAUNCH_PAIRS, SASA_MAX_POINTS, SASA_MAX_RES, SAXS_MAX_Q, SAXS_MAX_RES,
                        SAXS_MAX_TYPES, SS_MAX_RES, TM_MAX_RES, VIOL_MAX_RES, apply_xform, backbone_sasa, backbone_violations, ca_contact_map, ca_contact_stats, ca_lddt_matrix, ca_native_contacts, ca_native_q, ca_lddt_per_residue, ca_pairwise_distances, ca_pwd_js, ca_rmsd_matrix,
@@ -7,11 +7,11 @@
 from .geometry import forward_marginal, frames_to_backbone, rigid_compose_update, rigid_scale_trans, se3_step, torsion_head
 from .hostio import (float64_normal_outputs, format_pdb_models, host_rng_can_discard, host_rng_discard_float64_normals,
                      host_rng_fast_forward_ok, merge_pdb_files, write_pdb_models)
-from .node import (CHAIN_WIDTHS, NARROW_MAX_WORK, SMALL_ROWS, embed_assemble, ipa_projections, node_apply,
+from .node import (CHAIN_WIDTHS, NARROW_MAX_WORK, SMALL_ROWS, embed_assemble, encoder_in_proj, ipa_projections, node_apply,
                    node_apply_chain, node_apply_multi, node_chain, node_linear, node_linear_f32, node_linear_multi, node_linear_vfrag,
                    pack_planes, row_layernorm, small_rows_variant, to_act)
-from .packing import (NODE_TG, LazyDict, PairTiled, act_alloc, column_blocked, fragment_order, node_tiles, pack_f16x2_layer, pack_f16x3_embed_stream,
-                      pack_f16x3_stream, pack_node_layer, pack_node_weight, pack_node_weight_f32, pack_weight, padded_len, pair_tiled,
+from .packing import (NODE_TG, LazyDict, PairTiled, act_alloc, column_blocked, encoder_qk_order, fragment_order, node_tiles, pack_f16x2_layer, pack_f16x3_embed_stream,
+                      pack_encoder_in_proj, pack_f16x3_stream, pack_node_layer, pack_node_weight, pack_node_weight_f32, pack_weight, padded_len, pair_tiled,
                       pair_untiled, unpack_planes, vf_alloc, xp_alloc)
 from .pair import edge_embed, edge_embed_f16x3, edge_transition, edge_transition_f16x3, pair_project
 from .range_guard import (RANGE_BITS, RANGE_FAMILIES, range_families, range_flag, range_flag_names, range_flag_read, range_flag_reset,
@@ -25,7 +25,7 @@
     "pack_f16x3_stream", "pack_node_layer", "pack_node_weight", "pack_node_weight_f32", "pack_weight", "padded_len", "pair_tiled", "pair_untiled",
     "unpack_planes", "vf_alloc", "xp_alloc",
     "edge_embed", "edge_embed_f16x3", "edge_transition", "edge_transition_f16x3", "pair_project",
-    "encoder_attention", "ipa_attention", "ipa_attention_f16", "ipa_prep_points", "ipa_prep_points_f16",
+    "encoder_attention", "encoder_attention_frag", "encoder_in_proj", "encoder_qk_order", "pack_encoder_in_proj", "ipa_attention", "ipa_attention_f16", "ipa_prep_points", "ipa_prep_points_f16",
     "CHAIN_WIDTHS", "NARROW_MAX_WORK", "SMALL_ROWS", "embed_assemble", "ipa_projections", "node_apply",
     "node_apply_chain", "node_apply_multi", "node_chain", "node_linear", "node_linear_f32", "node_linear_multi", "node_linear_vfrag", "pack_planes",
     "row_layernorm", "small_rows_variant", "to_act",
diff --git a/str2str_amd/ops/attention.py b/str2str_amd/ops/attention.py
--- a/str2str_amd/ops/attention.py
+++ b/str2str_amd/ops/attention.py
@@ -117,3 +117,22 @@
     _check(_timed("s2s_encoder_attention", lambda: fn(_p(qkv), _p(key_bias), _p(out), _p(oxp), n_samples, n_res, n_heads, D // n_heads,
                                                       rw, _stream())), "s2s_encoder_attention")
     return out, oxp
+
+
+def encoder_attention_frag(q_xp, k_xp, v_vf, key_bias: Optional[torch.Tensor], n_samples: int, n_res: int, n_heads: int = 4,
+                           want_f32: bool = False, want_xp: bool = True):
+    lib = load_library()
+    _req_all(torch.int16, q_xp=q_xp, k_xp=k_xp, v_vf=v_vf)
+    _req_opt(key_bias=key_bias)
+    D, n_pad = 80 * n_heads, padded_len(n_res)
+    rows = n_samples * n_pad
+    if min(q_xp.numel(), k_xp.numel()) < rows * D * 2 or v_vf.numel() < rows * 96 * n_heads * 2 or (
+            key_bias is not None and key_bias.numel() != n_samples * n_res):
+        raise HipLibraryError("encoder_attention_frag: operands do not hold padded_len(n_res) rows per sample")
+    M = n_samples * n_res
+    out = torch.empty(M, D, device=q_xp.device, dtype=torch.float32) if want_f32 else None
+    oxp = xp_alloc(M, D, q_xp.device) if want_xp else None
+    _check(_timed("s2s_encoder_attention", lambda: lib.s2s_encoder_attention_frag(
+        _p(q_xp), _p(k_xp), _p(v_vf), _p(key_bias), _p(out), _p(oxp), n_samples, n_res, n_pad, n_heads, _p(range_flag()), _stream())),
+        "s2s_encoder_attention_frag")
+    return out, oxp
diff --git a/str2str_amd/ops/binding.py b/str2str_amd/ops/binding.py
--- a/str2str_amd/ops/binding.py
+++ b/str2str_amd/ops/binding.py
@@ -41,6 +41,8 @@
     "s2s_node_linear_vfrag": [_vp, _vp, _vp, _ll, _i, _i, _i, _vp, _i, _i, _vp, _vp],
     "s2s_encoder_attention": [_vp, _vp, _vp, _vp, _i, _i, _i, _i, _vp, _vp],
     "s2s_encoder_attention_f16x3": [_vp, _vp, _vp, _vp, _i, _i, _i, _i, _vp, _vp],
+    "s2s_encoder_in_proj": [_vp] * 7 + [_ll, _i, _i, _i, _vp, _vp, _vp, _i, _i, _vp, _vp],
+    "s2s_encoder_attention_frag": [_vp] * 6 + [_i, _i, _i, _i, _vp, _vp],
     "s2s_ca_sample_stats": [_vp, _i, _i, _f, _i, _vp, _vp, _vp, _vp],
     "s2s_ca_pairwise_distances": [_vp, _i, _i, _i, _vp, _vp],
     "s2s_ca_pwd_js": [_vp, _i, _vp, _i, _i, _i, _i, _d, _vp, _vp, _vp, _vp],
diff --git a/str2str_amd/ops/node.py b/str2str_amd/ops/node.py
--- a/str2str_amd/ops/node.py
+++ b/str2str_amd/ops/node.py
@@ -4,7 +4,7 @@
 import torch
 
 from .binding import HipLibraryError, _check, _int_arg, _p, _req, _req_all, _req_opt, _stream, _timed, load_library
-from .packing import vf_alloc, xp_alloc
+from .packing import ENC_HEAD_DIM, ENC_HEAD_PAD, padded_len, vf_alloc, xp_alloc
 from .range_guard import range_flag
 
 SMALL_ROWS = 8192
@@ -223,6 +223,30 @@
     return q_xp, k_xp, v_vf, qp_o, kvp_o
 
 
+def encoder_in_proj(xp, pack: dict, n_samples: int, n_res: int, out=None):
+    lib = load_library()
+    _req(xp, torch.int16, "xp")
+    D, heads = pack["k"], pack["heads"]
+    _req_all(torch.int16, wq=pack["wq"], wk=pack["wk"], wv=pack["wv"])
+    _req_all(bq=pack["bq"], bk=pack["bk"], bv=pack["bv"])
+    n_pad = padded_len(n_res)
+    rows = n_samples * n_pad
+    if xp.numel() != ((n_samples * n_res + 31) // 32) * (D // 16) * 1024:
+        raise HipLibraryError(f"encoder_in_proj: xp does not hold the planes of [{n_samples * n_res}, {D}]")
+    mp, ms = (n_pad, n_res) if n_pad != n_res else (0, 0)
+    if out is None:
+        out = xp_alloc(rows, D, xp.device), xp_alloc(rows, D, xp.device), vf_alloc(rows, ENC_HEAD_PAD * heads, xp.device)
+    q_xp, k_xp, v_vf = out
+    _req_all(torch.int16, q_xp=q_xp, k_xp=k_xp, v_vf=v_vf)
+    if min(q_xp.numel(), k_xp.numel()) < rows * D * 2 or v_vf.numel() < rows * ENC_HEAD_PAD * heads * 2:
+        raise HipLibraryError("encoder_in_proj: an output buffer is smaller than padded_len(n_res) rows per sample")
+    _check(_timed("s2s_node_linear", lambda: lib.s2s_encoder_in_proj(
+        _p(xp), _p(pack["wq"]), _p(pack["bq"]), _p(pack["wk"]), _p(pack["bk"]), _p(pack["wv"]), _p(pack["bv"]), rows, D, heads,
+        ENC_HEAD_DIM, _p(q_xp), _p(k_xp), _p(v_vf), mp, ms, _p(range_flag()), _stream()),
+        flops=2 * rows * D * (2 * D + ENC_HEAD_PAD * heads)), "s2s_encoder_in_proj")
+    return q_xp, k_xp, v_vf
+
+
 class _ChainLayer(ctypes.Structure):
     _fields_ = [("w_packed", ctypes.c_void_p), ("bias", ctypes.c_void_p), ("relu", ctypes.c_int)]
 
diff --git a/str2str_amd/ops/packing.py b/str2str_amd/ops/packing.py
--- a/str2str_amd/ops/packing.py
+++ b/str2str_amd/ops/packing.py
@@ -167,6 +167,37 @@
                     w32=lambda d: pack_node_weight_f32(w.float(), tg))
 
 
+ENC_HEAD_DIM, ENC_HEAD_PAD = 80, 96
+
+
+def encoder_qk_order(d_model: int) -> torch.Tensor:
+    t = torch.arange(d_model // 32)[:, None, None, None]
+    u = torch.arange(2)[None, :, None, None]
+    g = torch.arange(2)[None, None, :, None]
+    j = torch.arange(8)[None, None, None, :]
+    col = (32 * t + (j & 3) + 8 * (2 * u + (j >> 2)) + 4 * g).reshape(-1)
+    chan = (32 * t + 16 * u + 8 * g + j).expand(-1, 2, 2, 8).reshape(-1)
+    src = torch.empty(d_model, dtype=torch.long)
+    src[col] = chan
+    return src
+
+
+def pack_encoder_in_proj(in_proj_weight: torch.Tensor, in_proj_bias, n_heads: int) -> dict:
+    w = in_proj_weight.detach().float()
+    D = w.shape[1]
+    if w.shape[0] != 3 * D or D != n_heads * ENC_HEAD_DIM or D % 32 or n_heads % 2:
+        raise HipLibraryError("pack_encoder_in_proj: in_proj_weight must be [3 D, D] with D = n_heads * 80 and an even number of heads")
+    b = w.new_zeros(3 * D) if in_proj_bias is None else in_proj_bias.detach().float()
+    src = encoder_qk_order(D).to(w.device)
+    wv = w.new_zeros(n_heads, ENC_HEAD_PAD, D)
+    wv[:, :ENC_HEAD_DIM] = w[2 * D:].reshape(n_heads, ENC_HEAD_DIM, D)
+    bv = w.new_zeros(n_heads, ENC_HEAD_PAD)
+    bv[:, :ENC_HEAD_DIM] = b[2 * D:].reshape(n_heads, ENC_HEAD_DIM)
+    return {"wq": pack_node_weight(w[:D][src], D // 32), "bq": b[:D][src].contiguous(),
+            "wk": pack_node_weight(w[D:2 * D][src], D // 32), "bk": b[D:2 * D][src].contiguous(),
+            "wv": pack_node_weight(wv.reshape(-1, D), 6), "bv": bv.reshape(-1).contiguous(), "k": D, "heads": n_heads}
+
+
 class LazyDict(dict):
 
     def __init__(self, eager: dict, **lazy):
diff --git a/str2str_amd/ops/torch_ops.py b/str2str_amd/ops/torch_ops.py
--- a/str2str_amd/ops/torch_ops.py
+++ b/str2str_amd/ops/torch_ops.py
@@ -1,9 +1,9 @@
 import torch
 
-from .attention import encoder_attention, ipa_attention, ipa_attention_f16, ipa_prep_points, ipa_prep_points_f16
+from .attention import encoder_attention, encoder_attention_frag, ipa_attention, ipa_attention_f16, ipa_prep_points, ipa_prep_points_f16
 from .binding import _opt_int
 from .geometry import forward_marginal, frames_to_backbone, rigid_compose_update, rigid_scale_trans, se3_step, torsion_head
-from .node import (embed_assemble, ipa_projections, node_chain, node_linear, node_linear_f32, node_linear_multi, node_linear_vfrag, pack_planes,
+from .node import (embed_assemble, encoder_in_proj, ipa_projections, node_chain, node_linear, node_linear_f32, node_linear_multi, node_linear_vfrag, pack_planes,
                    row_layernorm)
 from .packing import PairTiled
 from .pair import edge_embed, edge_embed_f16x3, edge_transition, edge_transition_f16x3, pair_project
@@ -71,6 +71,8 @@
         lambda q, k, v, qp, kp, vp, q2, k2, ab, pz, m, r7, *rest: ipa_attention_f16(q, k, v, (qp, kp, vp, q2, k2), ab, pz, m, r7, *rest),
     "encoder_attention(Tensor qkv, Tensor? key_bias, int n_samples, int n_res, int n_heads=4, bool want_f32=False, bool want_xp=True, "
     "str arith='f32') -> (Tensor?, Tensor?)": lambda *a: encoder_attention(*a),
+    "encoder_attention_frag(Tensor q_xp, Tensor k_xp, Tensor v_vf, Tensor? key_bias, int n_samples, int n_res, int n_heads=4, "
+    "bool want_f32=False, bool want_xp=True) -> (Tensor?, Tensor?)": lambda *a: encoder_attention_frag(*a),
     "node_linear(Tensor xp, Tensor wpk, Tensor? bias, int n_rows, int k_in, int n_out, int tiles, Tensor? pre_scale=None, bool relu=False, "
     "Tensor? pre_mask=None, Tensor? residual=None, Tensor? ln_gamma=None, Tensor? ln_beta=None, float ln_eps=0.0, Tensor? post_mask=None, "
     "Tensor(a!)? out_f32=None, int out_col0=0, bool want_f32=True, Tensor(b!)? out_xp=None, int out_xp_k=-1, int out_xp_k0=0, "
@@ -87,6 +89,8 @@
             s_xp, *[({"w": t[0], "b": t[1], "k": dims[3 * i], "n": dims[3 * i + 1], "tg": dims[3 * i + 2]} if len(t) else None)
                     for i, t in enumerate((q, k, v, qp, kvp))],
             m, mo, (mp, ms) if mp else None),
+    "encoder_in_proj(Tensor xp, Tensor[] pack, int n_heads, int n_samples, int n_res) -> (Tensor, Tensor, Tensor)":
+        lambda xp, pk, heads, b, n: encoder_in_proj(xp, dict(zip(("wq", "bq", "wk", "bk", "wv", "bv"), pk), k=80 * heads, heads=heads), b, n),
     "embed_assemble(Tensor t_img, Tensor node_const, Tensor fa, Tensor fb, int n_samples, int n_res, bool planes, bool b_col_blocked) "
     "-> (Tensor, Tensor, Tensor)": lambda *a: embed_assemble(*a),
     "node_linear_multi(Tensor xp, Tensor[] w, Tensor[] bias, Tensor[] pre_scale, int[] dims, Tensor(a!)[] out_f32, Tensor(b!)[] out_xp) -> ()":
diff --git a/str2str_amd/sampler.py b/str2str_amd/sampler.py
--- a/str2str_amd/sampler.py
+++ b/str2str_amd/sampler.py
@@ -85,7 +85,8 @@
         if k in ("rigids_t", "sc_ca_t", "t_img", "t") or not torch.is_tensor(v):
             continue
         h.update(k.encode()); h.update(str(tuple(v.shape)).encode()); h.update(v.detach().cpu().numpy().tobytes())
-    modes = tuple((type(m).__name__, a, getattr(m, a)) for m in net.modules() for a in getattr(type(m), "launch_switches", ()))
+    modes = tuple((type(m).__name__, a, getattr(m, a)) for m in net.modules()
+                  for a in getattr(type(m), "launch_switches", ()) + getattr(type(m), "ab_switches", ()))
     return (id(net), sum(p._version for p in net.parameters()), b, N, modes, h.hexdigest())
 
 
```

Result: no change. 29.41 conformations/s, median of 6 (+0.4%).
